# giesselmann/STRique

Hardware: AMD Instinct MI355X
Metric: reads/s for STRique 'count' on 50 kb r9.4 signals (higher is better)
Workload: dtype f32

## Files before the change

### strique_amd/csrc/lut_kernels.h

```cpp
#pragma once
#include <hip/hip_runtime.h>
#include <stdint.h>
#include "align_kernels.h"

#define STRQ_LUT_MAX_K 158
#define STRQ_LUT_LOCAL_HARD 64
#define STRQ_TABLE_SLOT_FLOATS(k) ((size_t)(k) * 256)

namespace strq {

struct LutJob {
    const float* level_val;
    const float* cls_val;
    float* table;
    uint8_t* table3;
    int32_t* band_lo;
    int32_t k, pad_;
};
struct LutInfo { int32_t total, n_hard, need, packed; };
struct HardEntry { int32_t job, k, level, index; };

int launch_lut_build(hipStream_t stream, const LutJob* jobs, LutInfo* info, int n_jobs, int max_k,
                     HardEntry* hard, int* hard_count, int hard_cap, const AlignParams& p);
int launch_lut_patch(hipStream_t stream, const LutJob* jobs, const HardEntry* hard, const float* vals, int n);

}
```

### strique_amd/csrc/lut_kernels.hip

```cpp
#include <hip/hip_runtime.h>
#include <stdint.h>
#include "lut_kernels.h"

namespace strq {

#define STRQ_HARD_ULPS 64

static __device__ __forceinline__ float cell_score_dev(const AlignParams& p, float h, float v, bool* hard)
{
    const float d = h > v ? h - v : v - h;
    const double y = pow((double)d, 1.2);
    const uint64_t bits = __builtin_bit_cast(uint64_t, y);
    const int64_t low = (int64_t)(bits & 0x1FFFFFFFull) - 0x10000000ll;
    bool hd = (low >= -STRQ_HARD_ULPS && low <= STRQ_HARD_ULPS);
    const float x = (float)y;
    const float s = p.dist_offset - x;
    if (hd) {
        const uint32_t xb = __builtin_bit_cast(uint32_t, x);
        const float x2 = __builtin_bit_cast(float, (double)x < y ? xb + 1u : (xb ? xb - 1u : 0u));
        const float s2 = p.dist_offset - x2;
        if (!(s > p.dist_min) && !(s2 > p.dist_min)) hd = false;
    }
    *hard = hd;
    return s > p.dist_min ? s : p.dist_min;
}

__global__ void __launch_bounds__(256)
lut_build_kernel(const LutJob* __restrict__ jobs, LutInfo* __restrict__ info, HardEntry* __restrict__ hard,
                 int* __restrict__ hard_count, int hard_cap, AlignParams p)
{
    __shared__ float v[256];
    __shared__ float cls[STRQ_LUT_MAX_K];
    __shared__ int lo[STRQ_LUT_MAX_K], hi[STRQ_LUT_MAX_K + 1];
    __shared__ int width, n_local, plat_lo, plat_hi, rebuild, unpackable;
    __shared__ unsigned char dup[STRQ_LUT_MAX_K];
    __shared__ unsigned short local_hard[STRQ_LUT_LOCAL_HARD][2];
    const LutJob jb = jobs[blockIdx.x];
    const int q = threadIdx.x, lane = q & 63, wave = q >> 6;
    v[q] = jb.level_val[q];
    for (int k = q; k < jb.k; k += 256) cls[k] = jb.cls_val[k];
    if (q == 0) { width = 0; n_local = 0; plat_lo = 255; plat_hi = 0; rebuild = 0; unpackable = 0; }
    __syncthreads();
    {
        const float v0 = v[0], v255 = v[255], vq = v[q];
        if (__builtin_bit_cast(uint32_t, vq) != __builtin_bit_cast(uint32_t, v0)) atomicMin(&plat_lo, q - 1);
        if (__builtin_bit_cast(uint32_t, vq) != __builtin_bit_cast(uint32_t, v255)) atomicMax(&plat_hi, q + 1);
        if (q > 0 && !(v[q - 1] <= vq)) rebuild = 1;
    }
    __syncthreads();
    if (rebuild) { if (q == 0) { info[blockIdx.x].total = 0; info[blockIdx.x].need = 0; info[blockIdx.x].packed = 0; info[blockIdx.x].n_hard = -1; } return; }
    const int plat_lo_r = plat_lo, plat_hi_r = plat_hi < plat_lo ? plat_lo : plat_hi;
    auto in_band = [&](int lv, float c) { bool hd; return cell_score_dev(p, v[lv], c, &hd) > p.dist_min; };
    for (int k = q; k < jb.k; k += 256) {
        const float c = cls[k];
        int a = 0, b = 256;
        while (a < b) { const int m = (a + b) >> 1; if (v[m] < c) a = m + 1; else b = m; }
        int best = a < 256 ? a : 255;
        if (a > 0 && a < 256) { const float dl = c - v[a - 1], dr = v[a] - c; if (dl <= dr) best = a - 1; }
        int l = 256, h = -1;
        bool hd_best;
        const bool best_in = cell_score_dev(p, v[best], c, &hd_best) > p.dist_min;
        if (hd_best) rebuild = 1;
        if (best_in) {
            int x = 0, y = best;
            while (x < y) { const int m = (x + y) >> 1; if (in_band(m, c)) y = m; else x = m + 1; }
            l = x;
            x = best; y = 255;
            while (x < y) { const int m = (x + y + 1) >> 1; if (in_band(m, c)) x = m; else y = m - 1; }
            h = x;
        }
        const bool none = h < l;
        const int el = none ? 0 : (l <= plat_lo_r ? plat_lo_r : l - 1);
        const int er = none ? 0 : (h >= plat_hi_r ? plat_hi_r : h + 1);
        lo[k] = el | (er << 8) | ((!none && l <= plat_lo_r) ? 0 : 1 << 16) | ((!none && h >= plat_hi_r) ? 0 : 1 << 17);
        hi[k] = er - el + 1;
        atomicMax(&width, er - el + 1);
    }
    __syncthreads();
    for (int k = q; k < jb.k; k += 256) {
        int first = k;
        const uint32_t bits = __builtin_bit_cast(uint32_t, cls[k]);
        for (int j = 0; j < k; ++j) if (__builtin_bit_cast(uint32_t, cls[j]) == bits) { first = j; break; }
        dup[k] = (unsigned char)first;
    }
    __syncthreads();
    if (q == 0) {
        int off = 0;
        for (int k = 0; k < jb.k; ++k) {
            if (dup[k] == k) { const int w = hi[k]; hi[k] = off; off += w; }
            else hi[k] = hi[dup[k]];
        }
        hi[jb.k] = off;
    }
    __syncthreads();
    const int* roff = hi;
    for (int k = wave; k < jb.k; k += 4) {
        const int d = lo[k], el = d & 255, er = (d >> 8) & 255;
        const float c = cls[k];
        if (dup[k] != k) {
            if (lane == 0) jb.band_lo[k] = (int32_t)((uint32_t)el | ((uint32_t)(er - el) << 8) | ((uint32_t)roff[k] << 16));
            continue;
        }
        for (int lv = el + lane; lv <= er; lv += 64) {
            bool hd;
            const float s = cell_score_dev(p, v[lv], c, &hd);
            jb.table[roff[k] + lv - el] = s;
            {
                const float r = s * 1048576.0f;
                const uint32_t u = r >= 0.0f && r < 16777216.0f ? (uint32_t)r : 0u;
                if (!((float)u == r) || !(r < 16777216.0f) || __builtin_bit_cast(uint32_t, r) == 0x80000000u) unpackable = 1;
                const int e = roff[k] + lv - el, total = roff[jb.k];
                reinterpret_cast<uint16_t*>(jb.table3)[e] = (uint16_t)(u >> 8);
                jb.table3[((2 * total + 3) & ~3) + e] = (uint8_t)u;
            }
            if (hd) {
                if ((lv == el && (d & (1 << 16))) || (lv == er && (d & (1 << 17)))) rebuild = 1;
                else {
                    const int slot = atomicAdd(&n_local, 1);
                    if (slot < STRQ_LUT_LOCAL_HARD) { local_hard[slot][0] = (unsigned short)k; local_hard[slot][1] = (unsigned short)lv; }
                }
            }
        }
        if (lane == 0) jb.band_lo[k] = (int32_t)((uint32_t)el | ((uint32_t)(er - el) << 8) | ((uint32_t)roff[k] << 16));
    }
    __syncthreads();
    if (q == 0) {
        int nh = n_local;
        if (nh > STRQ_LUT_LOCAL_HARD || rebuild) nh = -1;
        info[blockIdx.x].total = roff[jb.k];
        info[blockIdx.x].need = width;
        info[blockIdx.x].packed = (nh == 0 && !unpackable) ? 1 : 0;
        info[blockIdx.x].n_hard = nh;
        for (int i = 0; i < nh; ++i) {
            const int k = local_hard[i][0], lv = local_hard[i][1];
            const int slot = atomicAdd(hard_count, 1);
            if (slot < hard_cap) {
                HardEntry e;
                e.job = blockIdx.x; e.k = k; e.level = lv;
                e.index = roff[k] + (lv - (lo[k] & 255));
                hard[slot] = e;
            }
        }
    }
}

__global__ void lut_patch_kernel(const LutJob* __restrict__ jobs, const HardEntry* __restrict__ hard,
                                 const float* __restrict__ vals, int n)
{
    const int i = blockIdx.x * blockDim.x + threadIdx.x;
    if (i < n) jobs[hard[i].job].table[hard[i].index] = vals[i];
}

int launch_lut_build(hipStream_t stream, const LutJob* jobs, LutInfo* info, int n_jobs, int max_k,
                     HardEntry* hard, int* hard_count, int hard_cap, const AlignParams& p)
{
    if (max_k > STRQ_LUT_MAX_K) return 2;
    hipLaunchKernelGGL(lut_build_kernel, dim3(n_jobs), dim3(256), 0, stream, jobs, info, hard, hard_count, hard_cap, p);
    return hipGetLastError() == hipSuccess ? 0 : 1;
}

int launch_lut_patch(hipStream_t stream, const LutJob* jobs, const HardEntry* hard, const float* vals, int n)
{
    if (n <= 0) return 0;
    hipLaunchKernelGGL(lut_patch_kernel, dim3((n + 255) / 256), dim3(256), 0, stream, jobs, hard, vals, n);
    return hipGetLastError() == hipSuccess ? 0 : 1;
}

}
```

### strique_amd/csrc/screen_kernels.h

```cpp
#pragma once
#include <hip/hip_runtime.h>
#include <stdint.h>
#include "align_kernels.h"

#define STRQ_SCREEN_R 14
#define STRQ_SCREEN_S 6
#define STRQ_SCREEN_SEG 4
#define STRQ_SCREEN_CHUNK_COLS 128
#define STRQ_SCREEN_MAX_WINDOWS 4
#define STRQ_SCREEN2_CPL 5
#define STRQ_SCREEN2_LPF 29
#define STRQ_SCREEN2_LANE_B 32

namespace strq {

struct ScreenParams {
    int32_t sc;
    int32_t hh, v;
    int32_t cadd;
    int32_t slack;
    int32_t merge_gap;
    int32_t max_cand;
    int32_t margin;
};

struct ScreenTask {
    const uint8_t* levels;
    const float* table;
    const int32_t* band_lo;
    int32_t* out;
    int32_t tsize;
    int32_t n, m, k, col_off;
    int32_t n_chunks;
    int32_t lane_last;
};

struct Screen2Task {
    const uint8_t* levels;
    const float* table[2];
    const int32_t* band_lo[2];
    int32_t* out[2];
    int32_t tsize[2], k[2];
    int32_t n, col_off, n_chunks;
};

struct ScreenWindows {
    int32_t n_win;
    int32_t lo[STRQ_SCREEN_MAX_WINDOWS], hi[STRQ_SCREEN_MAX_WINDOWS];
    float lower_bound;
    float upper_bound;
    int32_t n_cand;
};

int screen_plan(const AlignParams& p, int samples, int max_n, ScreenParams* sp);
static inline bool screen_flank_ok(int m) { return m >= 2 * STRQ_SCREEN_R && m <= 64 * STRQ_SCREEN_R; }
size_t screen_lds_bytes(int tsize);
int launch_screen(hipStream_t stream, const ScreenTask* tasks, int n_groups, int* queue, const ScreenParams& sp,
                  size_t lds_bytes, int tables_per_cu, int n_cu);
int screen2_plan(const AlignParams& p, int samples, int max_n, int merge, ScreenParams* sp);
static inline bool screen2_flank_ok(int m, int k) { return k >= 1 && k <= STRQ_SCREEN2_LPF * STRQ_SCREEN2_CPL && m == k * STRQ_SCREEN_S; }
size_t screen2_lds_bytes(int tsize_a, int tsize_b);
int screen2_lanes_rows(int need_a, int need_b);
bool screen2_lanes_fit(int rows);
size_t screen2_lanes_lds_bytes(int rows);
int launch_screen2(hipStream_t stream, const Screen2Task* tasks, int n_groups, int* queue, const ScreenParams& sp,
                   size_t lds_bytes, int groups_per_cu, int n_cu, int merge, int lanes_rows);
int launch_screen_windows(hipStream_t stream, const ScreenTask* tasks, int n_groups, const ScreenParams& sp,
                          const int32_t* bound_scaled, ScreenWindows* out, const int32_t* list = nullptr, const int32_t* theta_list = nullptr);

}
```

### strique_amd/csrc/screen_kernels.hip

```cpp
#include "strq_opt.h"
#include <hip/hip_runtime.h>
#include <stdint.h>
#include <stdlib.h>
#include <cmath>
#include "screen_kernels.h"
#include "screen_lds_layout.h"

namespace strq {

namespace {

constexpr int R = STRQ_SCREEN_R, S = STRQ_SCREEN_S, SEG = STRQ_SCREEN_SEG;
constexpr int G = 2, C = 3;
static_assert(R == 14 && S == 6, "class expansion below is written for 14 rows per lane, 6 samples per class");

__device__ __forceinline__ int dpp_shr1(int v, int fill)
{
    return __builtin_amdgcn_update_dpp(fill, v, 0x138, 0xF, 0xF, false);
}
__device__ __forceinline__ int dpp_shr1_open(int v)
{
    return __builtin_amdgcn_mov_dpp(v, 0x138, 0xF, 0xF, true);
}
__device__ __forceinline__ int med3i(int a, int lo, int hi)
{
    int r;
    asm("v_med3_i32 %0, %1, %2, %3" : "=v"(r) : "v"(a), "v"(lo), "v"(hi));
    return r;
}
#define STRQ_SCREEN_BIAS 0x00800000
#ifndef STRQ_SCREEN_WPE
#define STRQ_SCREEN_WPE 6
#endif
__device__ __forceinline__ int max3i(int a, int b, int c)
{
    int r;
    asm("v_max3_f32 %0, %1, %2, %3" : "=v"(r) : "v"(a), "v"(b), "v"(c));
    return r;
}
__device__ __forceinline__ int add_uniform(int v, int u)
{
    int r;
    asm("v_add_u32 %0, %2, %1" : "=v"(r) : "v"(v), "s"(u));
    return r;
}
__device__ __forceinline__ int sel_mask(int if0, int if1, uint64_t mask)
{
    int r;
    asm("v_cndmask_b32_e64 %0, %1, %2, %3" : "=v"(r) : "v"(if0), "v"(if1), "s"(mask));
    return r;
}

struct LaneConst { int lo2[C], hi2[C], off[C]; };

struct Screen {
    const char* lds;
    const LaneConst& lc;
    const uint64_t (&pm)[3];
    const int lane, n, hh;
    int T[R], SbotA, upS, potB, cmax;
    int qq;
    int scA[C], scB[C];

    __device__ __forceinline__ void fetch(int q2, int (&sc)[C])
    {
#pragma unroll
        for (int c = 0; c < C; ++c)
            sc[c] = *reinterpret_cast<const uint16_t*>(lds + med3i(q2, lc.lo2[c], lc.hi2[c]) + lc.off[c]);
    }
    __device__ __forceinline__ void advance(int qsrc, int snext, int& qn, int (&nA)[C], int (&nB)[C])
    {
        qn = __builtin_amdgcn_update_dpp(__builtin_amdgcn_readlane(qsrc, snext), qq, 0x138, 0xF, 0xF, false);
        fetch(qn & 0xffff, nA);
        fetch((int)((unsigned)qn >> 16), nB);
    }
    __device__ __forceinline__ void prime(int qcur)
    {
        qq = 0;
        int qn, nA[C], nB[C];
        advance(qcur, 0, qn, nA, nB);
        qq = qn;
#pragma unroll
        for (int c = 0; c < C; ++c) { scA[c] = nA[c]; scB[c] = nB[c]; }
    }
    __device__ __forceinline__ void expand(const int (&sc)[C], int (&rs)[R])
    {
#pragma unroll
        for (int r = 0; r < R; r += G) {
            const int base = r / S, x = (r % S) / G;
            int v;
            if (x == 0 || base + 1 >= C) v = sc[base < C ? base : C - 1];
            else v = sel_mask(sc[base], sc[base + 1], pm[x]);
#pragma unroll
            for (int g = 0; g < G && r + g < R; ++g) rs[r + g] = v;
        }
    }

    template <bool PRED>
    __device__ __forceinline__ void step(int t, int qsrc, int snext)
    {
        const int qn = __builtin_amdgcn_update_dpp(__builtin_amdgcn_readlane(qsrc, snext), qq, 0x138, 0xF, 0xF, false);
        const int potA = potB + hh, potBn = potA + hh;
        const int upA = dpp_shr1(SbotA, potA);
        const int upB = dpp_shr1(T[R - 1], potBn);
        int rsA[R], rsB[R];
        expand(scA, rsA);
        expand(scB, rsB);
        fetch(qn & 0xffff, scA);
        fetch((int)((unsigned)qn >> 16), scB);
        bool act = true, okB = true;
        if constexpr (PRED) { const int jB = 2 * (t - lane), jA = jB - 1; act = (jA >= 1) && (jA <= n); okB = jB <= n; }
        if (act) {
            int ta_prev = upA, ta_prev2 = upS, tb_prev2 = upB;
#pragma unroll
            for (int r = 0; r < R; ++r) {
                const int diagA = r == 0 ? upS : T[r - 1];
                const int ta = max3i(diagA + rsA[r], T[r], ta_prev);
                if (r > 0) {
                    const int tb = max3i(ta_prev2 + rsB[r - 1], ta_prev, tb_prev2);
                    T[r - 1] = tb; tb_prev2 = tb;
                }
                ta_prev2 = ta_prev; ta_prev = ta;
            }
            const int tb = max3i(ta_prev2 + rsB[R - 1], ta_prev, tb_prev2);
            T[R - 1] = tb;
            SbotA = ta_prev;
            upS = upB;
            const int cA = ta_prev - potA + STRQ_SCREEN_BIAS, cB = okB ? tb - potBn + STRQ_SCREEN_BIAS : cA;
            cmax = max3i(cmax, cA, cB);
        }
        potB = potBn;
        qq = qn;
    }
};

__device__ __forceinline__ int load_chunk(const ScreenTask& tk, int chunk, int lane)
{
    const int idx = (chunk * 64 + lane) * 2;
    int a = 0, b = 0;
    if (idx < tk.n) a = tk.levels[idx];
    if (idx + 1 < tk.n) b = tk.levels[idx + 1];
    return (a * 2) | ((b * 2) << 16);
}

}

size_t screen_lds_bytes(int tsize)
{
    return (size_t)((tsize + 1) & ~1) * 2 + 4;
}

__global__ void __attribute__((amdgpu_flat_work_group_size(64 * STRQ_SCREEN_SEG, 64 * STRQ_SCREEN_SEG), amdgpu_waves_per_eu(STRQ_SCREEN_WPE, STRQ_SCREEN_WPE)))
align_screen_kernel(const ScreenTask* __restrict__ tasks, int n_groups, int* __restrict__ queue, ScreenParams sp)
{
    extern __shared__ uint32_t lds_all[];
    __shared__ int next_group;
    const int lane = threadIdx.x & 63, wave = threadIdx.x >> 6;
    const char* ldsb = reinterpret_cast<const char*>(lds_all);
    for (;;) {
        __syncthreads();
        if (threadIdx.x == 0) next_group = atomicAdd(queue, 1);
        __syncthreads();
        const int gi = __builtin_amdgcn_readfirstlane(next_group);
        if (gi >= n_groups) break;
        const ScreenTask& t0 = tasks[(size_t)gi * SEG];
        const int ts = t0.tsize, zero_idx = (ts + 1) & ~1;
        {
            uint16_t* dst = reinterpret_cast<uint16_t*>(lds_all);
            const float scf = (float)sp.sc;
            for (int i = threadIdx.x; i < ts; i += 64 * SEG) dst[i] = (uint16_t)((int)ceilf(t0.table[i] * scf) + sp.cadd);
            if (threadIdx.x == 0) { dst[zero_idx] = 0; dst[zero_idx + 1] = 0; }
        }
        __syncthreads();
        const ScreenTask& tk = tasks[(size_t)gi * SEG + wave];
        if (tk.n <= 0) continue;

        LaneConst lc; uint64_t pm[3];
        {
            const int row0 = lane * R, kbase = row0 / S, phase = row0 % S;
#pragma unroll
            for (int c = 0; c < C; ++c) {
                const int k = kbase + c;
                if (k < tk.k) {
                    const uint32_t d = (uint32_t)tk.band_lo[k];
                    const int lo = (int)(d & 255u), w1 = (int)((d >> 8) & 255u), off = (int)(d >> 16);
                    lc.lo2[c] = lo * 2; lc.hi2[c] = (lo + w1) * 2;
                    lc.off[c] = (off - lo) * 2;
                } else {
                    lc.lo2[c] = 0; lc.hi2[c] = 0; lc.off[c] = zero_idx * 2;
                }
            }
            pm[0] = 0;
#pragma unroll
            for (int x = 1; x < 3; ++x) {
                const uint64_t b = __ballot(phase >= S - x * G);
                const uint32_t lo = __builtin_amdgcn_readfirstlane((int)(uint32_t)b), hi = __builtin_amdgcn_readfirstlane((int)(uint32_t)(b >> 32));
                pm[x] = ((uint64_t)hi << 32) | lo;
            }
        }
        const int lM = (tk.m - 1) / R;
        Screen f{ldsb, lc, pm, lane, tk.n, sp.hh};
        {
#pragma unroll
            for (int r = 0; r < R; ++r) f.T[r] = STRQ_SCREEN_BIAS;
            f.SbotA = STRQ_SCREEN_BIAS; f.upS = STRQ_SCREEN_BIAS;
            f.potB = STRQ_SCREEN_BIAS - 2 * lane * sp.hh;
            f.cmax = STRQ_SCREEN_BIAS;
        }
        const int nsteps = (tk.n + 1) / 2 + 63;
        int qcur = load_chunk(tk, 0, lane);
        f.prime(qcur);
        for (int t0s = 0; t0s < nsteps; t0s += 64) {
            const int qnext = load_chunk(tk, t0s / 64 + 1, lane);
            const bool full = (t0s >= 63) && (2 * (t0s + 64) <= tk.n);
            const int send = nsteps - t0s < 64 ? nsteps - t0s : 64;
            if (full) {
                for (int s = 0; s < 63; ++s) f.template step<false>(t0s + s + 1, qcur, s + 1);
                f.template step<false>(t0s + 64, qnext, 0);
            } else {
                for (int s = 0; s < send; ++s) {
                    const int qsrc = s == 63 ? qnext : qcur, snext = (s + 1) & 63;
                    f.template step<true>(t0s + s + 1, qsrc, snext);
                }
            }
            const int cm = __builtin_amdgcn_readlane(f.cmax, lM) - STRQ_SCREEN_BIAS;
            if (lane == 0) tk.out[t0s / 64] = cm;
            f.cmax = STRQ_SCREEN_BIAS;
            qcur = qnext;
        }
    }
}

namespace {

constexpr int CPL = STRQ_SCREEN2_CPL, LPF = STRQ_SCREEN2_LPF, LB = STRQ_SCREEN2_LANE_B;

struct Lane2Const { int lo2[CPL], hi2[CPL], off[CPL]; };

template <int RPC, int CMG>
struct Screen2 {
    static constexpr int R2 = RPC * CPL;
    static_assert(CMG == 1 || CMG == 2 || CMG == 4, "groups must divide the 64 steps of a chunk");
    const char* lds;
    const Lane2Const& lc;
    const uint64_t top_mask;
    const int lane, n, hh;
    int T[R2], SbotA, upS, potB, cmax;
    int gpot, gmax;
    int qq;
    int scA[CPL], scB[CPL];

    __device__ __forceinline__ int score(int q2, int c) const
    {
        return *reinterpret_cast<const uint16_t*>(lds + med3i(q2, lc.lo2[c], lc.hi2[c]) + lc.off[c]);
    }
    __device__ __forceinline__ void prime(int qcur)
    {
        qq = __builtin_amdgcn_update_dpp(__builtin_amdgcn_readlane(qcur, 0), 0, 0x138, 0xF, 0xF, false);
#pragma unroll
        for (int c = 0; c < CPL; ++c) { scA[c] = score(qq & 0xffff, c); scB[c] = score((int)((unsigned)qq >> 16), c); }
    }

    template <bool PRED>
    __device__ __forceinline__ void step(int t, int qsrc, int snext, bool gfirst = true, bool glast = true)
    {
        const int qn = __builtin_amdgcn_update_dpp(__builtin_amdgcn_readlane(qsrc, snext), qq, 0x138, 0xF, 0xF, false);
        const int qa = qn & 0xffff, qb = (int)((unsigned)qn >> 16);
        const int potA = add_uniform(potB, hh), potBn = add_uniform(potA, hh);
        const int upA = sel_mask(dpp_shr1_open(SbotA), potA, top_mask);
        const int upB = sel_mask(dpp_shr1_open(T[R2 - 1]), potBn, top_mask);
        constexpr bool GROUPED = !PRED && CMG > 1;
        if (GROUPED && gfirst) gpot = potA;
        bool act = true, okB = true;
        if constexpr (PRED) { const int jB = 2 * (t - lane), jA = jB - 1; act = (jA >= 1) && (jA <= n); okB = jB <= n; }
        int ta_prev = upA, ta_prev2 = upS;
        int tb_prev2 = upB;
#pragma unroll
        for (int c = 0; c < CPL; ++c) {
            if (act) {
#pragma unroll
                for (int r = RPC * c; r < RPC * c + RPC; ++r) {
                    const int diagA = r == 0 ? upS : T[r - 1];
                    const int ta = max3i(diagA + scA[c], T[r], ta_prev);
                    if (r > 0) {
                        const int tb = max3i(ta_prev2 + scB[(r - 1) / RPC], ta_prev, tb_prev2);
                        T[r - 1] = tb; tb_prev2 = tb;
                    }
                    ta_prev2 = ta_prev; ta_prev = ta;
                }
                if (c == CPL - 1) {
                    const int tb = max3i(ta_prev2 + scB[c], ta_prev, tb_prev2);
                    T[R2 - 1] = tb;
                    SbotA = ta_prev;
                    upS = upB;
                    if constexpr (GROUPED) {
                        if (glast) { const int d = tb - gpot; gmax = d > gmax ? d : gmax; }
                    } else {
                        const int cA = ta_prev - potA + STRQ_SCREEN_BIAS, cB = okB ? tb - potBn + STRQ_SCREEN_BIAS : cA;
                        cmax = max3i(cmax, cA, cB);
                    }
                }
            }
            scA[c] = score(qa, c);
            if (c > 0) scB[c - 1] = score(qb, c - 1);
            if (c == CPL - 1) scB[c] = score(qb, c);
        }
        potB = potBn;
        qq = qn;
    }
};

template <int SHIFT>
__device__ __forceinline__ int load_chunk2(const Screen2Task& tk, int chunk, int lane)
{
    const int idx = (chunk * 64 + lane) * 2;
    int a = 0, b = 0;
    if (idx < tk.n) a = tk.levels[idx];
    if (idx + 1 < tk.n) b = tk.levels[idx + 1];
    return (a << SHIFT) | (b << (SHIFT + 16));
}

template <int RPC, int CMG, bool LANES>
__device__ __forceinline__ void screen2_body(const Screen2Task* __restrict__ tasks, int n_groups, int* __restrict__ queue, const ScreenParams& sp, int lds_rows)
{
    constexpr int R2 = RPC * CPL, MERGE = S / RPC;
    constexpr int QSHIFT = LANES ? screen_lanes::ROW_SHIFT : 1;
    static_assert(CPL == screen_lanes::CPL, "screen_lds_layout.h stacks the lane's five classes");
    extern __shared__ uint32_t lds_all[];
    __shared__ int next_group;
    const int lane = threadIdx.x & 63, wave = threadIdx.x >> 6;
    const char* ldsb = reinterpret_cast<const char*>(lds_all);
    const int f = lane >= LB ? 1 : 0, lf = lane - f * LB;
    for (;;) {
        __syncthreads();
        if (threadIdx.x == 0) next_group = atomicAdd(queue, 1);
        __syncthreads();
        const int gi = __builtin_amdgcn_readfirstlane(next_group);
        if (gi >= n_groups) break;
        const Screen2Task& t0 = tasks[(size_t)gi * SEG];
        const float scf = (float)sp.sc;
        Lane2Const lc;
        if constexpr (LANES) {
            uint32_t desc[CPL];
            int nc = 0, rowbase[CPL];
#pragma unroll
            for (int c = 0; c < CPL; ++c) {
                const int k = lf * CPL + c;
                const bool in = lf < LPF && k < t0.k[f];
                desc[c] = in ? (uint32_t)t0.band_lo[f][k] : 0u;
                nc += in ? 1 : 0;
            }
            screen_lanes::row_bases(desc, nc, rowbase);
            char* dst = reinterpret_cast<char*>(lds_all);
            if (wave == 0) *reinterpret_cast<uint16_t*>(dst + screen_lanes::slot(lane)) = 0;
#pragma unroll
            for (int c = 0; c < CPL; ++c) {
                const screen_lanes::ClassAddr a = c < nc ? screen_lanes::class_addr(lane, rowbase[c], desc[c]) : screen_lanes::padding_addr(lane);
                lc.lo2[c] = a.lo2; lc.hi2[c] = a.hi2; lc.off[c] = a.off;
                if (c < nc) {
                    const float* src = t0.table[f] + screen_lanes::desc_off(desc[c]);
                    const int w1 = screen_lanes::desc_w1(desc[c]);
                    for (int i = (wave - rowbase[c]) & (SEG - 1); i <= w1; i += SEG)
                        if (rowbase[c] + i < lds_rows)
                            *reinterpret_cast<uint16_t*>(dst + screen_lanes::entry_address(lane, rowbase[c], i)) = (uint16_t)(MERGE * ((int)ceilf(src[i] * scf) + sp.cadd));
                }
            }
        }
        [[maybe_unused]] int base[2], zero_idx[2];
        base[0] = 0; zero_idx[0] = (t0.tsize[0] + 1) & ~1;
        base[1] = zero_idx[0] + 2; zero_idx[1] = base[1] + ((t0.tsize[1] + 1) & ~1);
        if constexpr (!LANES) {
            uint16_t* dst = reinterpret_cast<uint16_t*>(lds_all);
#pragma unroll
            for (int ff = 0; ff < 2; ++ff) {
                for (int i = threadIdx.x; i < t0.tsize[ff]; i += 64 * SEG) dst[base[ff] + i] = (uint16_t)(MERGE * ((int)ceilf(t0.table[ff][i] * scf) + sp.cadd));
                if (threadIdx.x == 0) { dst[zero_idx[ff]] = 0; dst[zero_idx[ff] + 1] = 0; }
            }
        }
        __syncthreads();
        const Screen2Task& tk = tasks[(size_t)gi * SEG + wave];
        if (tk.n <= 0) continue;

        if constexpr (!LANES) {
#pragma unroll
            for (int c = 0; c < CPL; ++c) {
                const int k = lf * CPL + c;
                if (lf < LPF && k < tk.k[f]) {
                    const uint32_t d = (uint32_t)tk.band_lo[f][k];
                    const int lo = (int)(d & 255u), w1 = (int)((d >> 8) & 255u), off = (int)(d >> 16);
                    lc.lo2[c] = lo * 2; lc.hi2[c] = (lo + w1) * 2;
                    lc.off[c] = (base[f] + off - lo) * 2;
                } else {
                    lc.lo2[c] = 0; lc.hi2[c] = 0; lc.off[c] = zero_idx[f] * 2;
                }
            }
        }
        const uint64_t top_mask = 1ull | (1ull << LB);
        const int lMa = (tk.k[0] - 1) / CPL, lMb = LB + (tk.k[1] - 1) / CPL;
        Screen2<RPC, CMG> s2{ldsb, lc, top_mask, lane, tk.n, sp.hh};
        {
#pragma unroll
            for (int r = 0; r < R2; ++r) s2.T[r] = STRQ_SCREEN_BIAS;
            s2.SbotA = STRQ_SCREEN_BIAS; s2.upS = STRQ_SCREEN_BIAS;
            s2.potB = STRQ_SCREEN_BIAS - 2 * lane * sp.hh;
            s2.cmax = STRQ_SCREEN_BIAS; s2.gpot = 0; s2.gmax = 0;
        }
        const int nsteps = (tk.n + 1) / 2 + 63;
        int qcur = load_chunk2<QSHIFT>(tk, 0, lane);
        s2.prime(qcur);
        for (int t0s = 0; t0s < nsteps; t0s += 64) {
            const int qnext = load_chunk2<QSHIFT>(tk, t0s / 64 + 1, lane);
            const bool full = (t0s >= 63) && (2 * (t0s + 64) <= tk.n);
            const int send = nsteps - t0s < 64 ? nsteps - t0s : 64;
            if (full) {
                constexpr int U = CMG > 2 ? CMG : 2;
                s2.gmax = 0;
#pragma unroll 1
                for (int s = 0; s < 64 - U; s += U) {
#pragma unroll
                    for (int u = 0; u < U; ++u) s2.template step<false>(0, qcur, s + u + 1, u % CMG == 0, u % CMG == CMG - 1);
                }
#pragma unroll
                for (int u = 0; u < U - 1; ++u) s2.template step<false>(0, qcur, 64 - U + u + 1, u % CMG == 0, u % CMG == CMG - 1);
                s2.template step<false>(0, qnext, 0, CMG == 1, true);
                if constexpr (CMG > 1) s2.cmax = s2.gmax + STRQ_SCREEN_BIAS;
            } else {
                for (int s = 0; s < send; ++s) {
                    const int qsrc = s == 63 ? qnext : qcur, snext = (s + 1) & 63;
                    s2.template step<true>(t0s + s + 1, qsrc, snext);
                }
            }
            const int cma = __builtin_amdgcn_readlane(s2.cmax, lMa) - STRQ_SCREEN_BIAS;
            const int cmb = __builtin_amdgcn_readlane(s2.cmax, lMb) - STRQ_SCREEN_BIAS;
            if (lane == 0) { tk.out[0][t0s / 64] = cma; tk.out[1][t0s / 64] = cmb; }
            s2.cmax = STRQ_SCREEN_BIAS;
            qcur = qnext;
        }
    }
}

}

size_t screen2_lds_bytes(int tsize_a, int tsize_b)
{
    return (size_t)(((tsize_a + 1) & ~1) + 2 + ((tsize_b + 1) & ~1) + 2) * 2;
}

int screen2_lanes_rows(int need_a, int need_b) { return screen_lanes::rows_bound(need_a, need_b); }
bool screen2_lanes_fit(int rows) { return screen_lanes::fits(rows); }
size_t screen2_lanes_lds_bytes(int rows) { return screen_lanes::bytes(rows); }

#ifndef STRQ_SCREEN3_CMG
#define STRQ_SCREEN3_CMG 2
#endif
#define STRQ_SCREEN2_ATTR(WPE_) __attribute__((amdgpu_flat_work_group_size(64 * STRQ_SCREEN_SEG, 64 * STRQ_SCREEN_SEG), amdgpu_waves_per_eu(WPE_, WPE_)))
#define STRQ_SCREEN2_ARGS const Screen2Task* __restrict__ tasks, int n_groups, int* __restrict__ queue, ScreenParams sp, int lds_rows
__global__ void STRQ_SCREEN2_ATTR(6) align_screen3_kernel(STRQ_SCREEN2_ARGS) { screen2_body<2, STRQ_SCREEN3_CMG, true>(tasks, n_groups, queue, sp, lds_rows); }
__global__ void STRQ_SCREEN2_ATTR(4) align_screen1_kernel(STRQ_SCREEN2_ARGS) { screen2_body<6, 1, true>(tasks, n_groups, queue, sp, lds_rows); }
__global__ void STRQ_SCREEN2_ATTR(6) align_screen3_rows_kernel(STRQ_SCREEN2_ARGS) { screen2_body<2, STRQ_SCREEN3_CMG, false>(tasks, n_groups, queue, sp, lds_rows); }
__global__ void STRQ_SCREEN2_ATTR(4) align_screen1_rows_kernel(STRQ_SCREEN2_ARGS) { screen2_body<6, 1, false>(tasks, n_groups, queue, sp, lds_rows); }
#undef STRQ_SCREEN2_ARGS

__global__ void __launch_bounds__(256)
screen_windows_kernel(const ScreenTask* __restrict__ tasks, int n_groups, ScreenParams sp,
                      const int32_t* __restrict__ bound_scaled, ScreenWindows* __restrict__ out,
                      const int32_t* __restrict__ list, const int32_t* __restrict__ theta_list)
{
    const int lane = threadIdx.x & 63;
    const int idx = blockIdx.x * (blockDim.x >> 6) + (threadIdx.x >> 6);
    if (idx >= n_groups) return;
    const int g = list ? list[idx] : idx;
    const ScreenTask* tg = tasks + (size_t)g * SEG;
    const int m = tg[0].m, lM = tg[0].lane_last;
    const int shift = -m * sp.v;
    int vmax = 0;
    for (int w = 0; w < SEG; ++w) {
        if (tg[w].n <= 0) continue;
        for (int c = lane; c < tg[w].n_chunks; c += 64) { const int v = tg[w].out[c]; vmax = v > vmax ? v : vmax; }
    }
#pragma unroll
    for (int d = 32; d >= 1; d >>= 1) { const int o = __shfl_xor(vmax, d, 64); vmax = o > vmax ? o : vmax; }
    ScreenWindows r;
    r.n_win = 0; r.n_cand = 0;
    for (int k = 0; k < STRQ_SCREEN_MAX_WINDOWS; ++k) { r.lo[k] = 0; r.hi[k] = 0; }
    const int drop = (sp.margin > 0 ? sp.margin : m) + 2 * sp.slack;
    int theta = theta_list ? theta_list[idx] : vmax - drop;
    if (!theta_list && sp.max_cand > 0) {
        auto count_at = [&](int t) {
            int n = 0;
            for (int w = 0; w < SEG; ++w) {
                if (tg[w].n <= 0) continue;
                for (int c = lane; c < tg[w].n_chunks; c += 64) n += tg[w].out[c] >= t;
            }
#pragma unroll
            for (int d = 32; d >= 1; d >>= 1) n += __shfl_xor(n, d, 64);
            return n;
        };
        if (count_at(theta) > sp.max_cand) {
            int lo = theta, hi = vmax;
            while (hi - lo > 1) {
                const int mid = lo + (hi - lo) / 2;
                if (count_at(mid) > sp.max_cand) lo = mid; else hi = mid;
            }
            theta = hi;
        }
    }
    r.upper_bound = (float)(vmax + shift + sp.slack) / (float)sp.sc;
    auto scan = [&](int th, bool store) -> int {
        int nw = 0, last_hi = -(1 << 30), ncand = 0;
        for (int w = 0; w < SEG; ++w) {
            if (tg[w].n <= 0) continue;
            for (int c0 = 0; c0 < tg[w].n_chunks; c0 += 64) {
                const int c1 = c0 + lane;
                const bool cand = c1 < tg[w].n_chunks && tg[w].out[c1] >= th;
                uint64_t mask = __ballot(cand);
                while (mask) {
                    const int bit = __builtin_ctzll(mask); mask &= mask - 1;
                    const int c = c0 + bit;
                    ++ncand;
                    int lo = 128 * c - 2 * lM + 1, hi = 128 * c - 2 * lM + 128;
                    if (lo < 1) lo = 1;
                    if (hi > tg[w].n) hi = tg[w].n;
                    if (hi < lo) continue;
                    lo += tg[w].col_off; hi += tg[w].col_off;
                    if (nw > 0 && lo <= last_hi + sp.merge_gap) {
                        if (hi > last_hi) last_hi = hi;
                        if (store) {
                            const int k = nw <= STRQ_SCREEN_MAX_WINDOWS ? nw - 1 : STRQ_SCREEN_MAX_WINDOWS - 1;
                            if (hi > r.hi[k]) r.hi[k] = hi;
                            if (lo < r.lo[k]) r.lo[k] = lo;
                        }
                    } else {
                        ++nw; last_hi = hi;
                        if (store) {
                            if (nw <= STRQ_SCREEN_MAX_WINDOWS) { r.lo[nw - 1] = lo; r.hi[nw - 1] = hi; }
                            else if (hi > r.hi[STRQ_SCREEN_MAX_WINDOWS - 1]) r.hi[STRQ_SCREEN_MAX_WINDOWS - 1] = hi;
                        }
                    }
                }
            }
        }
        if (store) r.n_cand = ncand;
        return nw;
    };
    if (!theta_list && sp.max_cand > 0 && scan(theta, false) > STRQ_SCREEN_MAX_WINDOWS) {
        int lo = theta, hi = vmax;
        while (hi - lo > 1) {
            const int mid = lo + (hi - lo) / 2;
            if (scan(mid, false) > STRQ_SCREEN_MAX_WINDOWS) lo = mid; else hi = mid;
        }
        theta = hi;
    }
    {
        const double lb = (double)(theta + shift + sp.slack) / (double)sp.sc;
        float lbf = (float)lb;
        if ((double)lbf < lb) {
            int32_t bits = __float_as_int(lbf);
            bits = lbf > 0.0f ? bits + 1 : (lbf < 0.0f ? bits - 1 : 1);
            lbf = __int_as_float(bits);
        }
        r.lower_bound = lbf;
    }
    const bool ok = theta + shift > 0 && theta + shift > bound_scaled[g];
    if (ok) {
        int nw = scan(theta, true);
        if (nw > STRQ_SCREEN_MAX_WINDOWS) nw = STRQ_SCREEN_MAX_WINDOWS;
        for (int a = 1; a < nw; ++a)
            for (int b = a; b > 0 && r.lo[b] < r.lo[b - 1]; --b) {
                const int tl = r.lo[b], th = r.hi[b]; r.lo[b] = r.lo[b - 1]; r.hi[b] = r.hi[b - 1]; r.lo[b - 1] = tl; r.hi[b - 1] = th;
            }
        int kept = nw > 0 ? 1 : 0;
        for (int a = 1; a < nw; ++a) {
            if (r.lo[a] <= r.hi[kept - 1] + 1) { if (r.hi[a] > r.hi[kept - 1]) r.hi[kept - 1] = r.hi[a]; }
            else { r.lo[kept] = r.lo[a]; r.hi[kept] = r.hi[a]; ++kept; }
        }
        for (int a = kept; a < STRQ_SCREEN_MAX_WINDOWS; ++a) { r.lo[a] = 0; r.hi[a] = 0; }
        r.n_win = kept;
    }
    if (lane == 0) out[idx] = r;
}

int screen_plan(const AlignParams& p, int samples, int max_n, ScreenParams* sp)
{
    if (strq::opt("STRQ_NO_SCREEN")) return 0;
    if (samples != S) return 0;
    if (!(p.open_h == p.ext_h && p.open_v == p.ext_v)) return 0;
    if (!(p.dist_min >= 0.0f) || !(p.ext_h < 0.0f) || !(p.ext_v < 0.0f) || !(p.dist_offset > 0.0f) || !(p.dist_min <= p.dist_offset)) return 0;
    for (int sc = 1024; sc >= 16; sc >>= 1) {
        const double hh = -(double)p.ext_h * sc, v = -(double)p.ext_v * sc, smax = std::ceil((double)p.dist_offset * sc);
        if (hh != (double)(long)hh || v != (double)(long)v) continue;
        if (hh < 1 || smax + v + hh > 65000.0) continue;
        const double top = 64.0 * R * (smax + v) + ((double)max_n + 256.0) * hh + smax + v + hh + (double)STRQ_SCREEN_BIAS;
        if (top > 2.0e9) continue;
        sp->sc = sc; sp->hh = (int)hh; sp->v = (int)v; sp->cadd = (int)(hh + v);
        {
            const double rows = 64.0 * R, maxval = rows * (double)p.dist_offset;
            double p2 = 1.0; while (p2 < maxval) p2 *= 2.0;
            const double adds = rows * (1.0 + (double)p.dist_offset / -(double)p.ext_h);
            const double e = adds * p2 / 16777216.0;
            if (!(e < 1.0e4)) continue;
            sp->slack = ((int)std::ceil(e) + 1) * sc;
        }
        sp->merge_gap = 3072; sp->margin = 0; sp->max_cand = 0;
        return 1;
    }
    return 0;
}

int screen2_plan(const AlignParams& p, int samples, int max_n, int merge, ScreenParams* sp)
{
    if (merge != 1 && merge != 3) return 0;
    if (!screen_plan(p, samples, max_n, sp)) return 0;
    while (sp->sc >= 16) {
        const double smax = std::ceil((double)p.dist_offset * sp->sc);
        if ((double)merge * (smax + sp->cadd) <= 65000.0) return 1;
        if ((sp->hh & 1) || (sp->v & 1)) return 0;
        sp->slack = (sp->slack / sp->sc) * (sp->sc / 2);
        sp->sc /= 2; sp->hh /= 2; sp->v /= 2; sp->cadd = sp->hh + sp->v;
    }
    return 0;
}

int launch_screen2(hipStream_t stream, const Screen2Task* tasks, int n_groups, int* queue, const ScreenParams& sp,
                   size_t lds_bytes, int groups_per_cu, int n_cu, int merge, int lanes_rows)
{
    if (n_groups <= 0) return 0;
    if (merge != 3 && merge != 1) return 2;
    const bool lanes = lanes_rows > 0;
    if (lanes && (!screen_lanes::fits(lanes_rows) || lds_bytes < screen_lanes::bytes(lanes_rows))) return 2;
    auto kern = merge == 3 ? (lanes ? align_screen3_kernel : align_screen3_rows_kernel) : (lanes ? align_screen1_kernel : align_screen1_rows_kernel);
    if (merge == 1 && groups_per_cu > 4) groups_per_cu = 4;
    if (groups_per_cu > 6) groups_per_cu = 6;
    (void)hipFuncSetAttribute((const void*)kern, hipFuncAttributeMaxDynamicSharedMemorySize, (int)lds_bytes);
    hipLaunchKernelGGL(kern, dim3(groups_per_cu * n_cu), dim3(64 * SEG), lds_bytes, stream, tasks, n_groups, queue, sp, lanes_rows);
    return hipGetLastError() == hipSuccess ? 0 : 1;
}

int launch_screen(hipStream_t stream, const ScreenTask* tasks, int n_groups, int* queue, const ScreenParams& sp,
                  size_t lds_bytes, int tables_per_cu, int n_cu)
{
    if (n_groups <= 0) return 0;
    (void)hipFuncSetAttribute((const void*)align_screen_kernel, hipFuncAttributeMaxDynamicSharedMemorySize, (int)lds_bytes);
    hipLaunchKernelGGL(align_screen_kernel, dim3(tables_per_cu * n_cu), dim3(64 * SEG), lds_bytes, stream, tasks, n_groups, queue, sp);
    return hipGetLastError() == hipSuccess ? 0 : 1;
}

int launch_screen_windows(hipStream_t stream, const ScreenTask* tasks, int n_groups, const ScreenParams& sp,
                          const int32_t* bound_scaled, ScreenWindows* out, const int32_t* list, const int32_t* theta_list)
{
    if (n_groups <= 0) return 0;
    hipLaunchKernelGGL(screen_windows_kernel, dim3((n_groups + 3) / 4), dim3(256), 0, stream, tasks, n_groups, sp, bound_scaled, out, list, theta_list);
    return hipGetLastError() == hipSuccess ? 0 : 1;
}

}
```

### strique_amd/csrc/strq_align_api.hip

```cpp
#include <hip/hip_runtime.h>
#include <algorithm>
#include <cmath>
#include <climits>
#include <cstring>
#include <cstdlib>
#include <time.h>
#include <unistd.h>
#include <map>
#include <mutex>
#include <string>
#include <tuple>
#include <numeric>
#include <vector>
#include "../../include/strique_hip.h"
#include "strq_ctx.h"
#include "align_kernels.h"
#include "lut_kernels.h"
#include "align_generic.h"

using namespace strq;

#define STRQ_DBG(...) do { if (strq::opt("STRQ_DEBUG")) { fprintf(stderr, "[strq] " __VA_ARGS__); fprintf(stderr, "\n"); fflush(stderr); } } while (0)

namespace strq {

static thread_local const strq_ctx* t_cur_ctx = nullptr;
static std::mutex g_opt_mu;
static std::map<std::string, std::string> g_opts;
CtxScope::CtxScope(const strq_ctx* c) : prev(t_cur_ctx) { t_cur_ctx = c; }
CtxScope::~CtxScope() { t_cur_ctx = prev; }
const char* opt(const char* key)
{
    static thread_local std::string ring[8];
    static thread_local unsigned ring_pos = 0;
    auto keep = [&](const std::string& v) -> const char* {
        if (v.empty()) return nullptr;
        std::string& slot = ring[ring_pos++ & 7u];
        slot = v;
        return slot.c_str();
    };
    if (t_cur_ctx) {
        std::lock_guard<std::mutex> lk(t_cur_ctx->options_mu);
        auto it = t_cur_ctx->options.find(key);
        if (it != t_cur_ctx->options.end()) return keep(it->second);
    }
    {
        std::lock_guard<std::mutex> lk(g_opt_mu);
        auto it = g_opts.find(key);
        if (it != g_opts.end()) return keep(it->second);
    }
    return getenv(key);
}

float host_cell_score(const AlignParams& p, float h, float v)
{
    const float d = h > v ? h - v : v - h;
    const float s = p.dist_offset - (float)std::pow((double)d, 1.2);
    return s > p.dist_min ? s : p.dist_min;
}

void host_col0(const AlignParams& p, int m, float* out)
{
    const float NINF = -3.4028234663852886e38f / 2;
    out[0] = 0.0f;
    float vprev = NINF, sprev = 0.0f;
    for (int i = 1; i <= m; ++i) {
        const float ext = vprev + p.ext_v, opn = sprev + p.open_v;
        const float v = ext >= opn ? ext : opn;
        out[i] = v; vprev = v; sprev = v;
    }
}

struct BatchIn {
    int64_t n_align, n_reads;
    const uint8_t* levels; const int64_t* read_off; const float* level_val;
    const int32_t* align_read; const float* flank; const int64_t* flank_off; int32_t samples;
};
struct BatchOut { float* score; int64_t* j_end; int64_t* j0; int32_t* rec; };


static const int hard_cap = 1 << 16;
static const int trace_wpb = 8;

struct Piece { int col_off, n; size_t ck; };

static int cut(int n, int segs, int ov, Piece* out)
{
    int use = segs;
    while (use > 1 && (ov <= 0 || (long)n < (long)(use + 1) * ov)) --use;
    const long len = use > 1 ? ((long)n + (long)(use - 1) * ov + use - 1) / use : n;
    long o = 0;
    for (int k = 0; k < segs; ++k) {
        if (k >= use) { out[k].col_off = 0; out[k].n = 0; continue; }
        const long start = k == 0 ? 0 : o - ov;
        long end = k == use - 1 ? n : start + len; if (end > n) end = n;
        out[k].col_off = (int)start; out[k].n = (int)(end - start);
        o = end;
    }
    return use;
}

static int packed_dwords(int entries) { return (((2 * entries + 3) & ~3) + entries + 3) / 4; }

struct Launch { int R, NS, tables, first, count, first_task, first_up, lds_floats, packed, segs; bool known_last_row; };

struct CorePlan {
    CorePlan(strq_ctx* c_, const AlignCoreIn& in_, AlignCoreOut& out_) : c(c_), in(in_), out(out_), nb(in_.nb), S(in_.samples), st(c_->stream) {}
    strq_ctx* c;
    const AlignCoreIn& in;
    AlignCoreOut& out;
    const int nb, S;
    const hipStream_t st;

    bool collapsed = false, allow_pack = false, ov_fixed = false, scr_forced = false, mode_fine = false, mode_coarse = false;
    int seg_want = 0, max_tables = 8, max_waves = 16, ov_cap = 8192;
    std::map<std::pair<int, int>, int> ov_of_m;

    std::vector<size_t> cls_off, col0_off, bnd_off;
    std::vector<int> J0, NJ;
    std::vector<int> job_align, job_k0, job_k;
    std::vector<size_t> tab_off, desc_off;
    int nj = 0, max_k = 0;
    std::vector<float> h_cls;
    std::vector<LutJob> jobs;
    std::vector<LutInfo> info;
    std::vector<int> tab_total;

    std::vector<ScreenWindows> wins;
    bool screen2_ran = false;
    std::vector<int> g2_of;
    ScreenTask* d_st2 = nullptr;
    int32_t* d_bound2 = nullptr;
    ScreenParams sp2{};
    double coarse_cols = 0, coarse_all = 0;

    std::vector<char> packed;
    std::vector<int> overlap, segs_of;
    std::vector<Launch> launches;
    int n_up = 0, max_ns = 1, r2_cap = 0, qi = STRQ_QUEUE_FIRST;
    size_t n_tasks = 0, safe0 = 0, r2_0 = 0;
    std::vector<Piece> pieces, safe;
    std::vector<float> min_score;
    std::vector<char> two_round;
    bool any_two_round = false;
    std::vector<size_t> ck_up;
    std::vector<AlignTask> tasks;
    AlignTask *d_tasks = nullptr, *d_heads = nullptr;
    AlignResult *d_seg = nullptr, *d_res = nullptr, *d_seg_safe = nullptr;
    int32_t* d_pick = nullptr;
    float* d_min_score = nullptr;
    int *d_redo = nullptr, *d_redo_count = nullptr;
};

static int overlap_for(CorePlan& p, int m, int ov_worst, int redo_weight = 1)
{
    strq_ctx* c = p.c;
    if (p.ov_fixed || c->score_fracs.size() < 64 || c->mean_n <= 0) return std::min(ov_worst, p.ov_cap);
    auto it = p.ov_of_m.find(std::make_pair(m, redo_weight));
    if (it != p.ov_of_m.end()) return it->second;
    const std::vector<float>& f = c->score_fracs;
    double best_cost = 0; int best_ov = std::min(ov_worst, p.ov_cap);
    for (int ov = 1024; ; ov += 512) {
        if (ov > ov_worst) ov = ov_worst;
        const float need = align_segment_min_score(c->ap, m, ov) / ((float)m * c->ap.dist_offset) + 0.01f;
        const double redo = (double)(std::lower_bound(f.begin(), f.end(), need) - f.begin()) / (double)f.size();
        const double cost = 3.0 * ov / c->mean_n + redo_weight * redo * (1.0 + 3.0 * ov_worst / c->mean_n);
        if (best_cost == 0 || cost < best_cost) { best_cost = cost; best_ov = ov; }
        if (ov >= ov_worst) break;
    }
    p.ov_of_m[std::make_pair(m, redo_weight)] = best_ov;
    STRQ_DBG("overlap for %d-row flanks: %d columns (worst case %d; previous sub-batch: median score fraction %.3f, mean read %.0f samples)", m, best_ov, ov_worst, f[f.size() / 2], c->mean_n);
    return best_ov;
}

static int tables_for(const CorePlan& p, int dwords, int segs)
{
    int t = std::min(p.max_tables, (160 * 1024 - 64) / (std::max(dwords, 1) * 4));
    if (segs > 1) t = std::min(t, p.max_waves / segs);
    return t;
}

static void pause_after_fail(int& pause, int& fail)
{
    pause = std::min(256, 8 << std::min(fail, 5));
    ++fail;
}

static int upload_inputs(CorePlan& p)
{
    strq_ctx* c = p.c; const AlignCoreIn& in = p.in; AlignCoreOut& out = p.out;
    const int nb = p.nb, S = p.S;
    hipStream_t st = p.st;
    size_t cls_tot = 0, col0_tot = 0, rec_tot = 0, tab_tot = 0, bnd_floats = 0, desc_tot = 0;
    p.cls_off.assign(nb, 0); p.col0_off.assign(nb, 0); p.bnd_off.assign(nb, 0);
    std::map<const float*, size_t> cls_of_flank; std::map<int, size_t> col0_of_m;
    std::vector<int> cls_first, col0_first;
    out.rec_off.assign(nb, 0);
    p.J0.assign(nb, 0); p.NJ.assign(nb, 0);
    for (int i = 0; i < nb; ++i) {
        auto fc = cls_of_flank.find(in.flank[i]);
        if (fc == cls_of_flank.end()) { fc = cls_of_flank.emplace(in.flank[i], cls_tot).first; cls_tot += in.k[i]; cls_first.push_back(i); }
        p.cls_off[i] = fc->second;
        auto f0 = col0_of_m.find(in.m[i]);
        if (f0 == col0_of_m.end()) { f0 = col0_of_m.emplace(in.m[i], col0_tot).first; col0_tot += in.m[i] + 1; col0_first.push_back(i); }
        p.col0_off[i] = f0->second;
        p.J0[i] = (int)p.job_align.size();
        p.NJ[i] = in.k[i] > STRQ_LUT_MAX_K ? in.NS[i] : 1;
        for (int sidx = 0; sidx < p.NJ[i]; ++sidx) {
            int k0 = 0, kn = in.k[i];
            if (p.NJ[i] > 1) {
                const int row0 = sidx * 64 * in.R[i], rows = std::min(64 * in.R[i], in.m[i] - row0);
                k0 = row0 / S; kn = (row0 + rows - 1) / S - k0 + 1;
            }
            p.job_align.push_back(i); p.job_k0.push_back(k0); p.job_k.push_back(kn);
            p.desc_off.push_back(desc_tot); desc_tot += kn;
            p.tab_off.push_back(tab_tot); tab_tot += STRQ_TABLE_SLOT_FLOATS(kn);
            p.max_k = std::max(p.max_k, kn);
        }
        out.rec_off[i] = rec_tot; rec_tot += in.m[i];
        p.bnd_off[i] = bnd_floats; if (in.NS[i] > 1) bnd_floats += (size_t)(in.NS[i] - 1) * 2 * ((size_t)in.n[i] + 2);
    }
    const int nj = p.nj = (int)p.job_align.size();
    out.rec_total = rec_tot;
    p.h_cls.assign(cls_tot, 0.0f);
    std::vector<float> h_col0(col0_tot);
    for (int i : cls_first) {
        const float* f = in.flank[i];
        for (int kk = 0; kk < in.k[i]; ++kk) p.h_cls[p.cls_off[i] + kk] = f[(size_t)kk * S];
    }
    for (int i : col0_first) host_col0(c->ap, in.m[i], &h_col0[p.col0_off[i]]);
    STRQ_HIP(c, c->flank_cls.reserve(cls_tot * 4));
    STRQ_HIP(c, c->col0.reserve(col0_tot * 4));
    STRQ_HIP(c, c->band_lo.reserve(desc_tot * 4));
    STRQ_HIP(c, c->tables.reserve(tab_tot * 4));
    STRQ_HIP(c, c->tables3.reserve(tab_tot * 3 + (size_t)nj * 8 + 64));
    STRQ_HIP(c, c->bnd.reserve(bnd_floats * 4 + 256));
    STRQ_HIP(c, c->rec.reserve(rec_tot * 4 + 256));
    STRQ_HIP(c, c->lutinfo.reserve((size_t)nj * (sizeof(LutJob) + sizeof(LutInfo))));
    STRQ_HIP(c, c->hard.reserve((size_t)hard_cap * (sizeof(HardEntry) + 4) + 64));
    STRQ_HIP(c, c->queue.reserve(STRQ_QUEUE_BYTES));
    STRQ_HIP(c, hipMemcpyAsync(c->flank_cls.p, p.h_cls.data(), cls_tot * 4, hipMemcpyHostToDevice, st));
    STRQ_HIP(c, hipMemcpyAsync(c->col0.p, h_col0.data(), col0_tot * 4, hipMemcpyHostToDevice, st));
    STRQ_HIP(c, hipMemsetAsync(c->queue.p, 0, STRQ_QUEUE_BYTES, st));
    return STRQ_OK;
}

struct TableBuild {
    int nj = 0, max_k = 0;
    std::vector<LutJob>* jobs = nullptr;
    const float* d_level_val = nullptr;
    std::vector<int> job_read;
    std::vector<const float*> job_cls;
    std::function<int()> after_tables;
    std::vector<LutInfo>* info = nullptr;
    std::vector<LutInfo>* reported = nullptr;
    std::vector<HardEntry>* handed = nullptr;
    int hard_count = 0;
};

static int run_table_build(strq_ctx* c, hipStream_t st, TableBuild& b)
{
    const int nj = b.nj;
    std::vector<LutJob>& jobs = *b.jobs;
    std::vector<LutInfo>& info = *b.info;
    LutJob* d_jobs = c->lutinfo.as<LutJob>();
    LutInfo* d_info = reinterpret_cast<LutInfo*>(d_jobs + nj);
    STRQ_HIP(c, hipMemcpyAsync(d_jobs, jobs.data(), (size_t)nj * sizeof(LutJob), hipMemcpyHostToDevice, st));
    HardEntry* d_hard = c->hard.as<HardEntry>();
    float* d_hard_vals = reinterpret_cast<float*>(d_hard + hard_cap);
    int* d_hard_count = c->queue.as<int>();
    STRQ_HIP(c, hipEventRecord(c->ev[0], st));
    if (launch_lut_build(st, d_jobs, d_info, nj, b.max_k, d_hard, d_hard_count, hard_cap, c->ap)) { c->err = "lut launch failed"; return STRQ_ERR_DEVICE; }
    STRQ_HIP(c, hipEventRecord(c->ev[1], st));
    if (b.after_tables) { const int arc = b.after_tables(); if (arc) return arc; }
    info.resize(nj);
    int hard_count = 0;
    STRQ_HIP(c, hipMemcpyAsync(info.data(), d_info, (size_t)nj * sizeof(LutInfo), hipMemcpyDeviceToHost, st));
    STRQ_HIP(c, hipMemcpyAsync(&hard_count, d_hard_count, 4, hipMemcpyDeviceToHost, st));
    STRQ_HIP(c, hipStreamSynchronize(st));
    if (b.reported) *b.reported = info;
    STRQ_DBG("lut done jobs=%d hard=%d floats0=%d", nj, hard_count, info[0].total);
    if (strq::opt("STRQ_DEBUG")) { int hist[9] = {0}; for (int i = 0; i < nj; ++i) hist[std::min(8, info[i].need / 8)]++; STRQ_DBG("band need histogram (x8 levels): %d %d %d %d %d %d %d %d %d", hist[0], hist[1], hist[2], hist[3], hist[4], hist[5], hist[6], hist[7], hist[8]); }
    if (strq::opt("STRQ_DEBUG")) { long tot = 0; int mx = 0; for (int i = 0; i < nj; ++i) { tot += info[i].total; mx = std::max(mx, info[i].total); } STRQ_DBG("table floats: mean %.0f max %d (k=%d)", (double)tot / nj, mx, jobs[0].k); }
    if (hard_count > hard_cap) { c->err = "too many borderline table entries"; return STRQ_ERR_DEVICE; }
    bool any_rebuild = false;
    for (int j = 0; j < nj; ++j) any_rebuild |= info[j].n_hard < 0;
    auto level_vals_of = [&](int read, float* dst) -> int {
        STRQ_HIP(c, hipMemcpy(dst, b.d_level_val + (size_t)read * 256, 256 * 4, hipMemcpyDeviceToHost));
        return STRQ_OK;
    };
    if (hard_count > 0) {
        std::vector<HardEntry> he(hard_count); std::vector<float> hv(hard_count);
        STRQ_HIP(c, hipMemcpy(he.data(), d_hard, (size_t)hard_count * sizeof(HardEntry), hipMemcpyDeviceToHost));
        float lv[256]; int last_read = -1;
        for (int i = 0; i < hard_count; ++i) {
            const int rd = b.job_read[he[i].job];
            if (rd != last_read) { const int rc = level_vals_of(rd, lv); if (rc) return rc; last_read = rd; }
            hv[i] = host_cell_score(c->ap, lv[he[i].level], b.job_cls[he[i].job][he[i].k]);
        }
        STRQ_HIP(c, hipMemcpyAsync(d_hard_vals, hv.data(), (size_t)hard_count * 4, hipMemcpyHostToDevice, st));
        if (launch_lut_patch(st, d_jobs, d_hard, d_hard_vals, hard_count)) { c->err = "patch launch failed"; return STRQ_ERR_DEVICE; }
        STRQ_HIP(c, hipStreamSynchronize(st));
        if (b.handed) *b.handed = he;
    } else if (b.handed) b.handed->clear();
    if (any_rebuild) for (int j = 0; j < nj; ++j) if (info[j].n_hard < 0) {
        const int kk = jobs[j].k;
        std::vector<float> tab((size_t)kk * 256); std::vector<int32_t> blo(kk);
        float lv[256];
        { const int rc = level_vals_of(b.job_read[j], lv); if (rc) return rc; }
        for (int x = 0; x < kk; ++x) {
            float* row = &tab[(size_t)x * 256];
            for (int q = 0; q < 256; ++q) row[q] = host_cell_score(c->ap, lv[q], b.job_cls[j][x]);
            blo[x] = (int32_t)((255u << 8) | ((uint32_t)(x * 256) << 16));
        }
        STRQ_HIP(c, hipMemcpy(jobs[j].table, tab.data(), tab.size() * 4, hipMemcpyHostToDevice));
        STRQ_HIP(c, hipMemcpy(jobs[j].band_lo, blo.data(), (size_t)kk * 4, hipMemcpyHostToDevice));
        info[j].total = kk * 256; info[j].need = 256;
    }
    b.hard_count = hard_count;
    return STRQ_OK;
}

static uint8_t* table3_slot(strq_ctx* c, size_t tab_off, int j)
{
    const size_t o = tab_off * 3 + (size_t)j * 8;
    return c->tables3.as<uint8_t>() + o - o % 4;
}

static int build_tables(CorePlan& p)
{
    strq_ctx* c = p.c; const AlignCoreIn& in = p.in;
    const int nb = p.nb, nj = p.nj;
    std::vector<LutJob>& jobs = p.jobs;
    jobs.resize(nj);
    TableBuild b;
    b.nj = nj; b.max_k = p.max_k; b.jobs = &jobs; b.d_level_val = in.d_level_val; b.after_tables = in.after_tables; b.info = &p.info;
    b.job_read.resize(nj); b.job_cls.resize(nj);
    for (int j = 0; j < nj; ++j) {
        const int i = p.job_align[j];
        jobs[j].level_val = in.d_level_val + (size_t)in.read[i] * 256;
        jobs[j].cls_val = c->flank_cls.as<float>() + p.cls_off[i] + p.job_k0[j];
        jobs[j].table = c->tables.as<float>() + p.tab_off[j];
        jobs[j].table3 = table3_slot(c, p.tab_off[j], j);
        jobs[j].band_lo = c->band_lo.as<int32_t>() + p.desc_off[j];
        jobs[j].k = p.job_k[j]; jobs[j].pad_ = 0;
        b.job_read[j] = in.read[i];
        b.job_cls[j] = &p.h_cls[p.cls_off[i] + p.job_k0[j]];
    }
    const int rc = run_table_build(c, p.st, b);
    if (rc) return rc;
    p.tab_total.assign(nb, 0);
    for (int j = 0; j < nj; ++j) p.tab_total[p.job_align[j]] = std::max(p.tab_total[p.job_align[j]], p.info[j].total);
    p.out.n_hard = b.hard_count;
    return STRQ_OK;
}

static void read_switches(CorePlan& p)
{
    const strq_ctx* c = p.c;
    p.collapsed = p.S == 6 && c->ap.open_h == c->ap.ext_h && c->ap.open_v == c->ap.ext_v;
    if (const char* e = strq::opt("STRQ_SEG")) { const int v = atoi(e); if (v >= 1 && v <= 4) p.seg_want = v; }
    if (const char* e = strq::opt("STRQ_TABLES")) { const int v = atoi(e); if (v >= 1 && v <= 8) p.max_tables = v; }
    if (const char* e = strq::opt("STRQ_MAX_WAVES")) { const int v = atoi(e); if (v >= 4 && v <= 16) p.max_waves = v; }
    p.allow_pack = p.collapsed && !strq::opt("STRQ_NO_PACK");
    if (const char* e = strq::opt("STRQ_OVERLAP")) { const int v = atoi(e); p.ov_cap = v > 0 ? v : (1 << 30); p.ov_fixed = true; }
    p.scr_forced = strq::opt("STRQ_SCREEN_ALWAYS") != nullptr;
    const char* mode_opt = strq::opt("STRQ_SCREEN_MODE");
    p.mode_fine = mode_opt && std::strcmp(mode_opt, "fine") == 0;
    p.mode_coarse = mode_opt && std::strcmp(mode_opt, "coarse") == 0;
}


struct ScreenJob {
    int flanks = 1;
    std::vector<int> al;
    std::vector<ScreenTask> views;
    std::vector<Screen2Task> t2;
    std::vector<int32_t> bound;
    std::vector<size_t> out_off;
    size_t out_words = 0, lds_bytes = 0;
    int lanes_rows = 0;
    double steps = 0;
};

struct ScreenRules {
    int merge;
    int groups_per_cu;
    const char* lds_err;
    bool below_bound_free;
    bool count_untaken;
    bool judge;
    double max_cols;
    int* pause; int* fail;
};

static void screen_tasks(CorePlan& p, const ScreenParams& sp, ScreenJob& j)
{
    constexpr int SSEG = STRQ_SCREEN_SEG;
    const AlignCoreIn& in = p.in;
    const int F = j.flanks, ng = (int)j.al.size() / F;
    if (F == 2) j.t2.resize((size_t)ng * SSEG);
    j.views.resize(j.al.size() * SSEG);
    j.bound.resize(j.al.size());
    j.out_off.assign(j.al.size() * SSEG, 0);
    for (int g = 0; g < ng; ++g) {
        const int* a = &j.al[(size_t)g * F];
        const int n = in.n[a[0]];
        const int m_big = F == 2 ? std::max(in.m[a[0]], in.m[a[1]]) : in.m[a[0]];
        const int ov_worst = align_segment_overlap(p.c->ap, m_big), ov_s = overlap_for(p, m_big, ov_worst, 16);
        Piece pc[SSEG];
        const int used = cut(n, SSEG, ov_s, pc);
        j.lds_bytes = std::max(j.lds_bytes, F == 2 ? screen2_lds_bytes(p.info[p.J0[a[0]]].total, p.info[p.J0[a[1]]].total) : screen_lds_bytes(p.info[p.J0[a[0]]].total));
        if (F == 2) j.lanes_rows = std::max(j.lanes_rows, screen2_lanes_rows(p.info[p.J0[a[0]]].need, p.info[p.J0[a[1]]].need));
        for (int f = 0; f < F; ++f)
            j.bound[(size_t)g * F + f] = used <= 1 ? INT32_MIN / 2 : (ov_s >= ov_worst ? 0 : (int32_t)std::ceil((double)align_segment_min_score(p.c->ap, in.m[a[f]], ov_s) * sp.sc));
        for (int w = 0; w < SSEG; ++w) {
            Screen2Task t; std::memset(&t, 0, sizeof(t));
            t.levels = in.d_levels + in.read_off[in.read[a[0]]] + pc[w].col_off;
            t.n = pc[w].n; t.col_off = pc[w].col_off;
            t.n_chunks = pc[w].n > 0 ? (align_num_steps(pc[w].n) + 63) / 64 : 0;
            for (int f = 0; f < F; ++f) {
                const LutJob& job = p.jobs[p.J0[a[f]]];
                t.table[f] = job.table; t.band_lo[f] = job.band_lo; t.tsize[f] = p.info[p.J0[a[f]]].total; t.k[f] = in.k[a[f]];
                ScreenTask v; std::memset(&v, 0, sizeof(v));
                v.n = pc[w].n; v.m = in.m[a[f]]; v.k = in.k[a[f]]; v.col_off = pc[w].col_off; v.n_chunks = t.n_chunks;
                if (F == 2) v.lane_last = f * STRQ_SCREEN2_LANE_B + (in.k[a[f]] - 1) / STRQ_SCREEN2_CPL;
                else { v.levels = t.levels; v.table = t.table[0]; v.band_lo = t.band_lo[0]; v.tsize = t.tsize[0]; v.lane_last = (v.m - 1) / STRQ_SCREEN_R; }
                j.out_off[((size_t)g * F + f) * SSEG + w] = j.out_words; j.out_words += (size_t)t.n_chunks;
                j.views[((size_t)g * F + f) * SSEG + w] = v;
            }
            if (pc[w].n > 0) j.steps += align_num_steps(pc[w].n);
            if (F == 2) j.t2[(size_t)g * SSEG + w] = t;
        }
    }
}

static int run_screen(CorePlan& p, ScreenJob& j, const ScreenParams& sp, const ScreenRules& r)
{
    constexpr int SSEG = STRQ_SCREEN_SEG;
    strq_ctx* c = p.c; const AlignCoreIn& in = p.in;
    hipStream_t st = p.st;
    const int nv = (int)j.al.size();
    int lanes_rows = 0;
    if (j.flanks == 2) {
        const char* e = strq::opt("STRQ_SCREEN_LDS");
        if (!(e && std::strcmp(e, "rows") == 0) && screen2_lanes_fit(j.lanes_rows)) { lanes_rows = j.lanes_rows; j.lds_bytes = screen2_lanes_lds_bytes(lanes_rows); }
    }
    if (j.lds_bytes > 160 * 1024 - 64) { c->err = r.lds_err; return STRQ_ERR_UNSUPPORTED; }
    const int groups = std::max(1, std::min(r.groups_per_cu, (int)((160 * 1024 - 64) / j.lds_bytes)));
    auto aligned = [](size_t bytes) { return (bytes + 255) & ~(size_t)255; };
    const size_t t2_bytes = aligned(j.t2.size() * sizeof(Screen2Task)), task_bytes = aligned(j.views.size() * sizeof(ScreenTask));
    const size_t bound_bytes = aligned((size_t)nv * 4), win_bytes = aligned((size_t)nv * sizeof(ScreenWindows));
    STRQ_HIP(c, c->screen.reserve(t2_bytes + task_bytes + bound_bytes + win_bytes + j.out_words * 4 + 256));
    char* base = c->screen.as<char>();
    Screen2Task* d_t2 = reinterpret_cast<Screen2Task*>(base);
    ScreenTask* d_st = reinterpret_cast<ScreenTask*>(base + t2_bytes);
    int32_t* d_bound = reinterpret_cast<int32_t*>(base + t2_bytes + task_bytes);
    ScreenWindows* d_win = reinterpret_cast<ScreenWindows*>(base + t2_bytes + task_bytes + bound_bytes);
    int32_t* d_out = reinterpret_cast<int32_t*>(base + t2_bytes + task_bytes + bound_bytes + win_bytes);
    for (size_t x = 0; x < j.views.size(); ++x) j.views[x].out = d_out + j.out_off[x];
    if (j.flanks == 2)
        for (int v = 0; v < nv; ++v) for (int w = 0; w < SSEG; ++w) j.t2[(size_t)(v / 2) * SSEG + w].out[v % 2] = j.views[(size_t)v * SSEG + w].out;
    if (j.flanks == 2) STRQ_HIP(c, hipMemcpyAsync(d_t2, j.t2.data(), j.t2.size() * sizeof(Screen2Task), hipMemcpyHostToDevice, st));
    STRQ_HIP(c, hipMemcpyAsync(d_st, j.views.data(), j.views.size() * sizeof(ScreenTask), hipMemcpyHostToDevice, st));
    STRQ_HIP(c, hipMemcpyAsync(d_bound, j.bound.data(), (size_t)nv * 4, hipMemcpyHostToDevice, st));
    STRQ_HIP(c, hipEventRecord(c->ev[5], st));
    int* queue = c->queue.as<int>() + STRQ_QUEUE_FIRST - 1;
    if (j.flanks == 2) {
        if (launch_screen2(st, d_t2, nv / 2, queue, sp, j.lds_bytes, groups, c->n_cu, r.merge, lanes_rows)) { c->err = "coarse screen launch failed"; return STRQ_ERR_DEVICE; }
    } else {
        if (launch_screen(st, d_st, nv, queue, sp, j.lds_bytes, groups, c->n_cu)) { c->err = "screen launch failed"; return STRQ_ERR_DEVICE; }
    }
    STRQ_HIP(c, hipEventRecord(c->ev[6], st));
    if (launch_screen_windows(st, d_st, nv, sp, d_bound, d_win)) { c->err = "screen windows launch failed"; return STRQ_ERR_DEVICE; }
    std::vector<ScreenWindows> hw((size_t)nv);
    STRQ_HIP(c, hipMemcpyAsync(hw.data(), d_win, hw.size() * sizeof(ScreenWindows), hipMemcpyDeviceToHost, st));
    STRQ_HIP(c, hipStreamSynchronize(st));
    c->screen_ran = true; c->screen_mode_last = r.merge > 1 ? 2 : 1; c->coarse_merge_last = r.merge;
    c->screen_lds_last = j.flanks == 2 ? (lanes_rows > 0 ? 1 : 2) : 0;
    if (const char* path = strq::opt("STRQ_SCREEN_DUMP")) {
        std::vector<int32_t> ho(j.out_words);
        STRQ_HIP(c, hipMemcpy(ho.data(), d_out, j.out_words * 4, hipMemcpyDeviceToHost));
        if (FILE* fp = fopen(path, "wb")) {
            const int32_t hdr[8] = {nv, sp.sc, sp.hh, sp.v, j.flanks, SSEG, sp.slack, r.merge};
            fwrite(hdr, 4, 8, fp);
            for (int v = 0; v < nv; ++v) {
                const int32_t gh[4] = {j.al[v], j.al[v], j.bound[v], j.views[(size_t)v * SSEG].lane_last};
                fwrite(gh, 4, 4, fp);
                for (int w = 0; w < SSEG; ++w) {
                    const ScreenTask& t = j.views[(size_t)v * SSEG + w];
                    const int32_t th[4] = {t.col_off, t.n, t.m, t.n_chunks};
                    fwrite(th, 4, 4, fp);
                    fwrite(ho.data() + (t.out - d_out), 4, (size_t)t.n_chunks, fp);
                }
                fwrite(&hw[(size_t)v], sizeof(ScreenWindows), 1, fp);
            }
            fclose(fp);
        }
    }
    if (const char* e = strq::opt("STRQ_SCREEN_TEST_RAISE")) {
        const float up = (float)atof(e);
        for (auto& w : hw) w.lower_bound += up;
    }
    int windowed = 0, heavy = 0, below_bound = 0; double cols = 0, all = 0;
    for (int v = 0; v < nv; ++v) {
        const int al = j.al[v];
        const ScreenWindows& w = hw[(size_t)v];
        c->screen_stats[1] += 1; c->screen_stats[7] += w.n_cand;
        double mine = in.n[al];
        if (w.n_win > 0) {
            p.wins[al] = w; c->screen_stats[2] += 1; ++windowed; mine = 0;
            for (int k = 0; k < w.n_win; ++k) { c->screen_stats[4] += w.hi[k] - w.lo[k] + 1; mine += w.hi[k] - w.lo[k] + 1 + 4096; }
        } else {
            c->screen_stats[3] += 1;
            if (w.n_cand == 0) { ++below_bound; if (r.below_bound_free) mine = 0; }
        }
        all += in.n[al]; cols += mine; heavy += mine > 4 * 32768.0;
    }
    if (r.count_untaken) c->screen_stats[3] += p.nb - nv;
    c->screen_stats[5] += j.steps; c->screen_stats[6] = sp.sc;
    if (j.flanks == 2) {
        p.screen2_ran = true;
        p.d_st2 = d_st; p.d_bound2 = d_bound; p.sp2 = sp;
        for (int v = 0; v < nv; ++v) p.g2_of[j.al[v]] = v;
        p.coarse_cols = cols; p.coarse_all = all;
    }
    if (r.judge && nv >= 64) {
        if (below_bound * 10 > nv && !p.ov_fixed) c->score_fracs.clear();
        else if (windowed < 0.9 * (nv - (p.ov_fixed ? 0 : below_bound)) || cols > r.max_cols * all || (long)heavy * 100 > 2L * nv) pause_after_fail(*r.pause, *r.fail);
        else *r.fail = 0;
    }
    STRQ_DBG("screen (%d flanks per wave, merge %d): %d alignments, scale %d, margin %.0f, %d groups per CU, LDS %zu bytes: %d with windows (%d below the cold-start bound), %.2f %% of the columns, %d heavy -> pause %d",
             j.flanks, r.merge, nv, sp.sc, (double)sp.margin / sp.sc, groups, j.lds_bytes, windowed, below_bound, 100.0 * cols / std::max(1.0, all), heavy, *r.pause);
    return STRQ_OK;
}

static int screen_two_flank(CorePlan& p, int merge, int max_n)
{
    strq_ctx* c = p.c; const AlignCoreIn& in = p.in;
    const int nb = p.nb;
    ScreenParams sp;
    if (!screen2_plan(c->ap, p.S, max_n, merge, &sp)) return STRQ_OK;
    const bool fine_rules = merge == 1;
    int min_n = fine_rules ? 65536 : 28672, groups = 6;
    if (const char* e = strq::opt("STRQ_SCREEN_MIN_N")) min_n = atoi(e);
    if (const char* e = strq::opt("STRQ_SCREEN2_GROUPS")) { const int v = atoi(e); if (v >= 1 && v <= 8) groups = v; }
    std::map<int, std::vector<int>> by_read;
    for (int i = 0; i < nb; ++i)
        if (in.NS[i] == 1 && p.NJ[i] == 1 && in.n[i] >= min_n && screen2_flank_ok(in.m[i], in.k[i])) by_read[in.read[i]].push_back(i);
    std::vector<std::pair<int, int>> pairs;
    for (auto& kv : by_read) {
        const std::vector<int>& v = kv.second;
        if (v.size() == 2) { pairs.emplace_back(v[0], v[1]); continue; }
        for (size_t x = 0; x + 1 < v.size(); ++x)
            if (!(v[x] & 1) && v[x + 1] == v[x] + 1) { pairs.emplace_back(v[x], v[x + 1]); ++x; }
    }
    std::stable_sort(pairs.begin(), pairs.end(), [&](const std::pair<int, int>& x, const std::pair<int, int>& y) { return in.n[x.first] > in.n[y.first]; });
    const int ngr = (int)pairs.size();
    if (ngr == 0 || 2 * ngr < (nb * 9) / 10) return STRQ_OK;
    sp.margin = (int32_t)std::lround((double)c->coarse_margin * (merge == 3 ? 1.3 : 1.0) * sp.sc);
    if (const char* e = strq::opt("STRQ_SCREEN2_MARGIN")) sp.margin = (int32_t)std::lround(atof(e) * sp.sc);
    sp.max_cand = 8;
    if (const char* e = strq::opt("STRQ_SCREEN2_MAX_CAND")) sp.max_cand = atoi(e);
    if (fine_rules) { sp.margin = 0; sp.max_cand = 0; }
    ScreenJob j;
    j.flanks = 2;
    for (const auto& pr : pairs) { j.al.push_back(pr.first); j.al.push_back(pr.second); }
    screen_tasks(p, sp, j);
    ScreenRules r;
    r.merge = merge; r.groups_per_cu = groups;
    r.lds_err = "score tables do not fit LDS (coarse screen)";
    r.below_bound_free = !p.ov_fixed; r.count_untaken = true;
    if (fine_rules) { r.judge = !p.scr_forced; r.max_cols = 0.15; r.pause = &c->screen_pause; r.fail = &c->screen_fail; }
    else { r.judge = !p.mode_coarse && !p.scr_forced; r.max_cols = 0.30; r.pause = &c->coarse_pause; r.fail = &c->coarse_fail; }
    return run_screen(p, j, sp, r);
}

static int screen_one_flank(CorePlan& p, const ScreenParams& sp)
{
    strq_ctx* c = p.c; const AlignCoreIn& in = p.in;
    int min_n = 65536;
    if (const char* e = strq::opt("STRQ_SCREEN_MIN_N")) min_n = atoi(e);
    std::vector<int> sel;
    for (int i = 0; i < p.nb; ++i)
        if (in.NS[i] == 1 && p.NJ[i] == 1 && in.n[i] >= min_n && screen_flank_ok(in.m[i]) && in.k[i] * p.S == in.m[i]) sel.push_back(i);
    std::stable_sort(sel.begin(), sel.end(), [&](int x, int y) { return in.n[x] > in.n[y]; });
    if (sel.empty()) return STRQ_OK;
    ScreenJob j;
    j.al = sel;
    screen_tasks(p, sp, j);
    ScreenRules r;
    r.merge = 0; r.groups_per_cu = 6;
    r.lds_err = "score table does not fit LDS (screen)";
    r.below_bound_free = false; r.count_untaken = false;
    r.judge = true; r.max_cols = 0.10; r.pause = &c->screen_pause; r.fail = &c->screen_fail;
    return run_screen(p, j, sp, r);
}

static int run_screens(CorePlan& p)
{
    strq_ctx* c = p.c; const AlignCoreIn& in = p.in;
    const int nb = p.nb;
    p.wins.resize(nb);
    c->screen_ran = false;
    STRQ_HIP(c, hipEventRecord(c->ev[2], p.st));
    int max_n = 0;
    for (int i = 0; i < nb; ++i) max_n = std::max(max_n, in.n[i]);
    c->screen_mode_last = 0;
    const int coarse_merge = 3;
    p.g2_of.assign(nb, -1);
    for (int attempt = 0; attempt < 2 && !p.screen2_ran; ++attempt) {
        int merge = coarse_merge;
        if (attempt == 0) {
            if (!p.collapsed || p.mode_fine || strq::opt("STRQ_NO_SCREEN")) continue;
            if (c->coarse_pause > 0 && !p.mode_coarse && !p.scr_forced) { --c->coarse_pause; continue; }
        } else {
            if (!p.collapsed || strq::opt("STRQ_NO_SCREEN") || (c->screen_pause > 0 && !p.scr_forced)) continue;
            merge = 1;
        }
        const int rc = screen_two_flank(p, merge, max_n);
        if (rc) return rc;
    }
    if (p.screen2_ran) return STRQ_OK;
    if (p.collapsed && c->screen_pause > 0 && !p.scr_forced) {
        --c->screen_pause; c->screen_stats[3] += nb;
        return STRQ_OK;
    }
    ScreenParams sp;
    if (p.collapsed && screen_plan(c->ap, p.S, max_n, &sp)) return screen_one_flank(p, sp);
    return STRQ_OK;
}

static int plan_launches(CorePlan& p)
{
    strq_ctx* c = p.c; const AlignCoreIn& in = p.in; AlignCoreOut& out = p.out;
    const int nb = p.nb;
    std::vector<ScreenWindows>& wins = p.wins;
    static const double rate[5][2] = {{0, 0}, {1.017, 0.941}, {0.79, 0.862}, {0.85, 0.85}, {0.69, 0.80}};
    p.packed.assign(nb, 0); p.overlap.assign(nb, 0); p.segs_of.assign(nb, 1);
    std::vector<char> segmentable(nb, 0);
    const bool force_pack = strq::opt("STRQ_PACK") != nullptr;
    int class_count[5] = {0, 0, 0, 0, 0};
    for (int i = 0; i < nb; ++i) {
        segmentable[i] = p.collapsed && in.NS[i] == 1;
        p.overlap[i] = segmentable[i] ? align_segment_overlap(c->ap, in.m[i]) : 0;
        const bool can_pack = p.allow_pack && in.NS[i] == 1 && p.info[p.J0[i]].packed && p.info[p.J0[i]].n_hard == 0;
        int best_s = 1, best_p = can_pack ? 1 : 0;
        if (segmentable[i]) {
            const double l = overlap_for(p, in.m[i], p.overlap[i]);
            double best_cost = 0;
            for (int sgs : {1, 2, 3, 4}) {
                if (p.seg_want ? sgs != p.seg_want : sgs == 3) continue;
                if (sgs > 1 && !p.seg_want && (l <= 0 || in.n[i] < (sgs + 1) * l)) continue;
                for (int pk = 0; pk < 2; ++pk) {
                    if ((pk && !can_pack) || (force_pack && can_pack && !pk)) continue;
                    const double cost = (in.n[i] + (sgs - 1) * l) * rate[sgs][pk];
                    if (best_cost == 0 || cost < best_cost) { best_cost = cost; best_s = sgs; best_p = pk; }
                }
            }
        }
        if (wins[i].n_win > 0) {
            ScreenWindows& w = wins[i];
            while (w.n_win < STRQ_SCREEN_MAX_WINDOWS) {
                int widest = 0;
                for (int k2 = 1; k2 < w.n_win; ++k2) if (w.hi[k2] - w.lo[k2] > w.hi[widest] - w.lo[widest]) widest = k2;
                if (w.hi[widest] - w.lo[widest] < 16384) break;
                const int mid = w.lo[widest] + (w.hi[widest] - w.lo[widest]) / 2;
                for (int k2 = w.n_win; k2 > widest + 1; --k2) { w.lo[k2] = w.lo[k2 - 1]; w.hi[k2] = w.hi[k2 - 1]; }
                w.lo[widest + 1] = mid + 1; w.hi[widest + 1] = w.hi[widest]; w.hi[widest] = mid;
                ++w.n_win;
            }
            const int nw = w.n_win;
            best_s = p.seg_want >= nw ? p.seg_want : (nw <= 2 ? nw : 4); best_p = 0;
        }
        p.segs_of[i] = best_s; p.packed[i] = (char)best_p;
        ++class_count[best_s];
    }
    std::vector<int>& segs_of = p.segs_of;
    if (!p.seg_want && !c->screen_ran) {
        int few = 2 * c->n_cu;
        if (const char* e = strq::opt("STRQ_CLASS_MIN")) few = atoi(e);
        if (class_count[4] && class_count[4] < few) { for (int i = 0; i < nb; ++i) if (segs_of[i] == 4) { segs_of[i] = 2; if (wins[i].n_win > 2) wins[i].n_win = 0; } class_count[2] += class_count[4]; class_count[4] = 0; }
        if (class_count[2] && class_count[2] < few && class_count[1]) { for (int i = 0; i < nb; ++i) if (segs_of[i] == 2) { segs_of[i] = 1; if (wins[i].n_win > 1) wins[i].n_win = 0; } class_count[1] += class_count[2]; class_count[2] = 0; }
    }
    std::map<std::tuple<int, int, int, int, int>, std::vector<int>> groups;
    for (int i = 0; i < nb; ++i) {
        const int w = tables_for(p, p.packed[i] ? packed_dwords(p.tab_total[i]) : p.tab_total[i], segs_of[i]);
        if (w < 1) { c->err = "score table does not fit LDS"; return STRQ_ERR_UNSUPPORTED; }
        groups[std::make_tuple(in.R[i], in.NS[i], -segs_of[i], -w, p.packed[i] ? 0 : 1)].push_back(i);
    }
    const int min_rounds = 4;
    for (auto it = groups.begin(); it != groups.end();) {
        auto nx = std::next(it);
        const int w = -std::get<3>(it->first);
        const bool same_kind = nx != groups.end() && std::get<0>(nx->first) == std::get<0>(it->first) && std::get<1>(nx->first) == std::get<1>(it->first)
                               && std::get<2>(nx->first) == std::get<2>(it->first)
                               && !(std::get<4>(it->first) == 1 && std::get<4>(nx->first) == 0);
        if (same_kind && (long)it->second.size() < (long)min_rounds * w * c->n_cu) {
            nx->second.insert(nx->second.end(), it->second.begin(), it->second.end());
            it = groups.erase(it);
        } else ++it;
    }
    out.order.clear(); out.order.reserve(nb);
    for (auto& g : groups) {
        auto& v = g.second;
        auto work = [&](int x) {
            if (wins[x].n_win <= 0) return (long)in.n[x];
            long w = 0;
            for (int k = 0; k < wins[x].n_win; ++k) w += wins[x].hi[k] - wins[x].lo[k] + 1 + 4096;
            return w;
        };
        std::stable_sort(v.begin(), v.end(), [&](int x, int y) { return work(x) > work(y); });
        const int NS = std::get<1>(g.first);
        const int pk = std::get<4>(g.first) == 0;
        int lds_floats = 0;
        for (int i : v) lds_floats = std::max(lds_floats, pk ? packed_dwords(p.tab_total[i]) : p.tab_total[i]);
        const int segs = -std::get<2>(g.first);
        const int tables = std::min(-std::get<3>(g.first), tables_for(p, lds_floats, segs));
        if (tables < 1) { c->err = "score table does not fit LDS"; return STRQ_ERR_UNSUPPORTED; }
        bool known = std::get<0>(g.first) == 14;
        for (int i : v) known = known && in.m[i] == 870;
        p.launches.push_back({std::get<0>(g.first), NS, tables, (int)out.order.size(), (int)v.size(), (int)p.n_tasks, 0, lds_floats, pk, segs, known});
        out.order.insert(out.order.end(), v.begin(), v.end());
        p.n_tasks += (size_t)v.size() * segs;
        if (NS > 1) p.n_up += (int)v.size() * (NS - 1);
    }
    { size_t up = p.n_tasks; for (auto& L : p.launches) if (L.NS > 1) { L.first_up = (int)up; up += (size_t)L.count * (L.NS - 1); } }
    return STRQ_OK;
}

static int cut_pieces(CorePlan& p)
{
    strq_ctx* c = p.c; const AlignCoreIn& in = p.in; const AlignCoreOut& out = p.out;
    const int nb = p.nb;
    const size_t n_tasks = p.n_tasks;
    p.safe0 = n_tasks + p.n_up + (size_t)nb;
    p.pieces.resize(n_tasks); p.safe.resize(n_tasks);
    p.min_score.assign(nb, -INFINITY);
    p.two_round.assign(p.launches.size(), 0);
    p.ck_up.assign(nb, 0);
    size_t ck_floats = 0;
    for (size_t li = 0; li < p.launches.size(); ++li) {
        auto& L = p.launches[li];
        for (int x = 0; x < L.count; ++x) {
            const int pos = L.first + x, i = out.order[pos];
            const int n = in.n[i], R = in.R[i], ov = p.overlap[i];
            const size_t per_ckpt = (size_t)STRQ_CKPT_FIELDS(R) * 64;
            Piece* pf = &p.pieces[(size_t)L.first_task + (size_t)x * L.segs];
            Piece* ps = &p.safe[(size_t)L.first_task + (size_t)x * L.segs];
            cut(n, L.segs, ov, ps);
            const int ov_fast = overlap_for(p, in.m[i], ov);
            if (p.wins[i].n_win > 0) {
                const ScreenWindows& w = p.wins[i];
                const int ov_w = std::min(ov > 0 ? ov : (1 << 30), align_overlap_for_score(c->ap, in.m[i], w.lower_bound));
                for (int k = 0; k < L.segs; ++k) {
                    if (k < w.n_win) { const int start = std::max(0, w.lo[k] - 1 - ov_w); pf[k].col_off = start; pf[k].n = w.hi[k] - start; }
                    else { pf[k].col_off = 0; pf[k].n = 0; }
                }
                p.min_score[pos] = std::max(w.lower_bound, align_segment_min_score(c->ap, in.m[i], ov_w));
                p.two_round[li] = 1;
            } else if (L.segs > 1 && ov_fast < ov && cut(n, L.segs, ov_fast, pf) > 1) {
                p.min_score[pos] = align_segment_min_score(c->ap, in.m[i], ov_fast);
                p.two_round[li] = 1;
            } else {
                for (int k = 0; k < L.segs; ++k) pf[k] = ps[k];
            }
            for (int k = 0; k < L.segs; ++k) {
                pf[k].ck = ps[k].ck = ck_floats;
                ck_floats += (size_t)align_num_ckpts(std::max(pf[k].n, ps[k].n)) * per_ckpt;
            }
            if (L.NS > 1) { p.ck_up[i] = ck_floats; ck_floats += (size_t)(L.NS - 1) * align_num_ckpts(n) * per_ckpt; }
        }
    }
    for (char t : p.two_round) p.any_two_round |= t != 0;
    const size_t n_all_tasks = p.safe0 + (p.any_two_round ? n_tasks : 0);
    STRQ_HIP(c, c->ckpt.reserve(ck_floats * 4 + 256));
    p.r2_cap = p.screen2_ran ? std::max(1024, std::min(nb, 8192)) : 0;
    p.r2_0 = n_all_tasks;
    STRQ_HIP(c, c->tasks.reserve((n_all_tasks + (size_t)p.r2_cap * 4) * sizeof(AlignTask)));
    STRQ_HIP(c, c->results.reserve((2 * n_tasks + nb) * sizeof(AlignResult) + (size_t)nb * 12 + p.launches.size() * 4 + 256));
    p.tasks.resize(n_all_tasks);
    p.d_tasks = c->tasks.as<AlignTask>();
    p.d_heads = p.d_tasks + n_tasks + p.n_up;
    p.d_seg = c->results.as<AlignResult>();
    p.d_res = p.d_seg + n_tasks;
    p.d_seg_safe = p.d_res + nb;
    p.d_pick = reinterpret_cast<int32_t*>(p.d_seg_safe + n_tasks);
    p.d_min_score = reinterpret_cast<float*>(p.d_pick + nb);
    p.d_redo = reinterpret_cast<int*>(p.d_min_score + nb);
    p.d_redo_count = p.d_redo + nb;
    return STRQ_OK;
}

static int write_tasks(CorePlan& p)
{
    strq_ctx* c = p.c; const AlignCoreIn& in = p.in; AlignCoreOut& out = p.out;
    const int nb = p.nb, S = p.S;
    hipStream_t st = p.st;
    const size_t n_tasks = p.n_tasks, n_up = p.n_up, safe0 = p.safe0;
    std::vector<AlignTask>& tasks = p.tasks;
    for (auto& L : p.launches) {
        for (int x = 0; x < L.count; ++x) {
            const int pos = L.first + x, i = out.order[pos];
            const int R = in.R[i], M = in.m[i];
            AlignTask base; std::memset(&base, 0, sizeof(base));
            base.levels = in.d_levels + in.read_off[in.read[i]];
            base.rec = c->rec.as<int32_t>() + out.rec_off[i];
            base.n = in.n[i]; base.n_full = in.n[i]; base.m_total = M;
            auto strip = [&](int row0, int rows, size_t ck, int sidx) {
                AlignTask t = base;
                const int j = p.NJ[i] > 1 ? p.J0[i] + sidx : p.J0[i];
                const int k0 = row0 / S, k1 = (row0 + rows - 1) / S;
                t.row0 = row0; t.m = rows; t.k = k1 - k0 + 1; t.tsize = p.info[j].total;
                t.table = p.jobs[j].table; t.table3 = p.jobs[j].table3; t.band_lo = p.jobs[j].band_lo + (k0 - p.job_k0[j]);
                t.col0 = c->col0.as<float>() + p.col0_off[i] + row0;
                t.ckpt = c->ckpt.as<float>() + ck;
                return t;
            };
            tasks[n_tasks + n_up + pos] = strip(0, M, 0, 0);
            if (L.NS == 1) {
                for (int k = 0; k < L.segs; ++k) {
                    const size_t ti = (size_t)L.first_task + (size_t)x * L.segs + k;
                    AlignTask t = strip(0, M, p.pieces[ti].ck, 0);
                    t.levels += p.pieces[ti].col_off; t.n = p.pieces[ti].n; t.col_off = p.pieces[ti].col_off;
                    tasks[ti] = t;
                    if (p.any_two_round) {
                        AlignTask u = strip(0, M, p.safe[ti].ck, 0);
                        u.levels += p.safe[ti].col_off; u.n = p.safe[ti].n; u.col_off = p.safe[ti].col_off;
                        tasks[safe0 + ti] = u;
                    }
                }
            } else {
                const int rows_s = 64 * R;
                const size_t ck_strip = (size_t)align_num_ckpts(in.n[i]) * STRQ_CKPT_FIELDS(R) * 64;
                float* bnd = c->bnd.as<float>() + p.bnd_off[i];
                const size_t bnd_stride = 2 * ((size_t)in.n[i] + 2);
                for (int sidx = 0; sidx < L.NS; ++sidx) {
                    const bool last = sidx == L.NS - 1;
                    const int row0 = sidx * rows_s, rows = last ? M - row0 : rows_s;
                    const size_t slot = last ? (size_t)L.first_task + x : (size_t)L.first_up + (size_t)sidx * L.count + x;
                    AlignTask t = strip(row0, rows, last ? p.pieces[(size_t)L.first_task + x].ck : p.ck_up[i] + (size_t)sidx * ck_strip, sidx);
                    if (sidx > 0) { t.bnd_in = bnd + (size_t)(sidx - 1) * bnd_stride; t.up = p.d_tasks + L.first_up + (size_t)(sidx - 1) * L.count + x; }
                    if (!last) t.bnd_out = bnd + (size_t)sidx * bnd_stride;
                    tasks[slot] = t;
                    if (last && p.any_two_round) tasks[safe0 + slot] = t;
                }
            }
        }
    }
    STRQ_HIP(c, hipMemcpyAsync(p.d_tasks, tasks.data(), tasks.size() * sizeof(AlignTask), hipMemcpyHostToDevice, st));
    STRQ_HIP(c, hipMemsetAsync(p.d_seg, 0, (2 * n_tasks + nb) * sizeof(AlignResult), st));
    if (p.any_two_round) {
        STRQ_HIP(c, hipMemcpyAsync(p.d_min_score, p.min_score.data(), (size_t)nb * 4, hipMemcpyHostToDevice, st));
        STRQ_HIP(c, hipMemsetAsync(p.d_redo_count, 0, p.launches.size() * 4, st));
    }
    size_t scratch_words = 0;
    for (auto& L : p.launches) scratch_words = std::max(scratch_words, align_trace_scratch_words_per_wave(L.R));
    STRQ_HIP(c, c->scratch.reserve(scratch_words * 8 * (size_t)c->n_cu * trace_wpb));
    out.n_launches = 0; out.wave_steps = 0; out.columns = 0;
    for (size_t t = 0; t < n_tasks + n_up; ++t) if (tasks[t].n > 0) { out.wave_steps += align_num_steps(tasks[t].n); out.columns += tasks[t].n; }
    if (!p.launches.empty()) {
        const Launch& L = p.launches.back(); out.segs = L.segs; out.tables = L.tables; out.packed = L.packed; out.rows_per_lane = L.R;
        const int i = out.order[L.first];
        out.overlap_worst = p.overlap[i]; out.overlap_first = L.segs > 1 ? overlap_for(p, in.m[i], p.overlap[i]) : 0;
        const bool seg_kernel = L.NS == 1 && p.collapsed;
        const int32_t g[8] = {L.segs, L.tables, seg_kernel ? align_segments_wpe(L.segs, L.tables) : 0, L.R, L.packed, out.overlap_first, out.overlap_worst, (int32_t)p.launches.size()};
        std::memcpy(c->geometry, g, sizeof(g));
    }
    return STRQ_OK;
}
// ... 299 lines not shown
    float ms;
    STRQ_HIP(c, hipEventElapsedTime(&ms, c->ev[0], c->ev[1])); *t_lut += ms;
    STRQ_HIP(c, hipEventElapsedTime(&ms, c->ev[2], c->ev[3])); *t_fwd += ms + c->aborted_fwd_ms;
    c->screen_stats[0] += c->aborted_screen_ms;
    c->aborted_fwd_ms = c->aborted_screen_ms = 0;
    STRQ_HIP(c, hipEventElapsedTime(&ms, c->ev[3], c->ev[4])); *t_tr += ms;
    if (c->screen_ran) { STRQ_HIP(c, hipEventElapsedTime(&ms, c->ev[5], c->ev[6])); c->screen_stats[0] += ms; }
    return STRQ_OK;
}

size_t align_workspace_bytes(int n, int m, int R, int NS)
{
    size_t b = (size_t)NS * (align_num_ckpts(n) + align_num_ckpts(n) / 4 + 300) * STRQ_CKPT_FIELDS(R) * 64 * 4;
    if (NS > 1) b += (size_t)(NS - 1) * ((size_t)n + 2) * 8;
    (void)m;
    return b;
}

int align_validate_flank(strq_ctx* c, const float* f, int64_t mm, int samples, int* k_out, int* R_out, int* NS_out)
{
    if (mm < 1 || samples < 1 || mm % samples != 0) { c->err = "flank length must be a positive multiple of `samples`"; return STRQ_ERR_UNSUPPORTED; }
    for (int64_t i = 0; i < mm; ++i)
        if (std::memcmp(&f[i], &f[i - i % samples], 4) != 0) { c->err = "flank is not made of runs of `samples` equal values"; return STRQ_ERR_UNSUPPORTED; }
    const int S = align_effective_samples(samples);
    int R = 0, NS = 0;
    if (mm > (1 << 20) || !align_plan((int)mm, S, &R, &NS)) { c->err = "flank shape not covered by the compiled kernels"; return STRQ_ERR_UNSUPPORTED; }
    if (S == 6 && mm / S > STRQ_LUT_MAX_K && NS == 1) { R = 12; NS = (int)((mm + 64 * 12 - 1) / (64 * 12)); }
    *k_out = (int)(mm / S); *R_out = R; *NS_out = NS;
    return STRQ_OK;
}

static int run_align_batch(strq_ctx* c, const BatchIn& in, const BatchOut& out)
{
    const int S = align_effective_samples(in.samples);
    const int64_t NA = in.n_align;
    std::fill(c->timing, c->timing + 8, 0.0f);
    for (double& v : c->screen_stats) v = 0;
    if (NA == 0) return STRQ_OK;
    std::vector<int> m(NA), k(NA), R(NA), n(NA), NS(NA);
    for (int64_t a = 0; a < NA; ++a) {
        const int64_t mm = in.flank_off[a + 1] - in.flank_off[a];
        const int rd = in.align_read[a];
        if (rd < 0 || rd >= in.n_reads) { c->err = "align_read out of range"; return STRQ_ERR_ARG; }
        const int64_t nn = in.read_off[rd + 1] - in.read_off[rd];
        if (nn < 0 || nn > (int64_t)1 << 30) { c->err = "bad read length"; return STRQ_ERR_ARG; }
        const int rc = align_validate_flank(c, in.flank + in.flank_off[a], mm, in.samples, &k[a], &R[a], &NS[a]);
        if (rc) return rc;
        m[a] = (int)mm; n[a] = (int)nn;
    }
    hipStream_t st = c->stream;
    c->second_round[0] = 0; c->second_round[1] = NA; c->look2_served = 0;
    STRQ_HIP(c, c->redo_total.reserve(64));
    STRQ_HIP(c, hipMemsetAsync(c->redo_total.p, 0, 64, st));
    const int64_t tot_levels = in.read_off[in.n_reads];
    STRQ_HIP(c, c->levels.reserve((size_t)tot_levels + 64));
    STRQ_HIP(c, c->level_val.reserve((size_t)in.n_reads * 256 * 4));
    STRQ_HIP(c, hipMemcpyAsync(c->levels.p, in.levels, (size_t)tot_levels, hipMemcpyHostToDevice, st));
    STRQ_HIP(c, hipMemcpyAsync(c->level_val.p, in.level_val, (size_t)in.n_reads * 256 * 4, hipMemcpyHostToDevice, st));
    int64_t a0 = 0;
    float t_lut = 0, t_fwd = 0, t_tr = 0, n_hard = 0, n_launch = 0;
    std::fill(c->counters, c->counters + 8, 0.0);
    while (a0 < NA) {
        int64_t a1 = a0; size_t ck_bytes = 0;
        while (a1 < NA) {
            const size_t need = align_workspace_bytes(n[a1], m[a1], R[a1], NS[a1]);
            if (a1 > a0 && ck_bytes + need > c->max_ws_bytes) break;
            ck_bytes += need; ++a1;
        }
        const int nb = (int)(a1 - a0);
        AlignCoreIn ci; AlignCoreOut co;
        ci.nb = nb; ci.samples = S; ci.d_levels = c->levels.as<uint8_t>(); ci.read_off = in.read_off;
        ci.d_level_val = c->level_val.as<float>();
        std::vector<const float*> fl(nb);
        for (int i = 0; i < nb; ++i) fl[i] = in.flank + in.flank_off[a0 + i];
        ci.read = in.align_read + a0; ci.n = &n[a0]; ci.m = &m[a0]; ci.k = &k[a0]; ci.R = &R[a0]; ci.NS = &NS[a0]; ci.flank = fl.data();
        int rc = align_core(c, ci, co);
        if (rc) return rc;
        std::vector<AlignResult> res(nb);
        std::vector<int32_t> h_rec(co.rec_total);
        STRQ_HIP(c, hipMemcpyAsync(res.data(), co.d_results, (size_t)nb * sizeof(AlignResult), hipMemcpyDeviceToHost, st));
        if (out.rec) STRQ_HIP(c, hipMemcpyAsync(h_rec.data(), co.d_rec, co.rec_total * 4, hipMemcpyDeviceToHost, st));
        STRQ_HIP(c, hipStreamSynchronize(st));
        for (int pos = 0; pos < nb; ++pos) {
            const int i = co.order[pos]; const int64_t a = a0 + i;
            if (out.score) out.score[a] = res[pos].best;
            if (out.j_end) out.j_end[a] = res[pos].j_end;
            if (out.j0) out.j0[a] = res[pos].j0;
            if (out.rec) std::memcpy(out.rec + in.flank_off[a], &h_rec[co.rec_off[i]], (size_t)m[a] * 4);
        }
        rc = align_core_times(c, &t_lut, &t_fwd, &t_tr);
        if (rc) return rc;
        n_hard += co.n_hard; n_launch += co.n_launches;
        c->counters[0] += co.wave_steps; c->counters[1] += co.columns; c->counters[2] += nb;
        c->counters[3] = co.segs; c->counters[4] = co.tables; c->counters[5] = co.packed; c->counters[6] = co.rows_per_lane;
        a0 = a1;
    }
    c->timing[0] = t_lut; c->timing[1] = t_fwd; c->timing[2] = t_tr; c->timing[3] = t_lut + t_fwd + t_tr; c->timing[4] = n_hard; c->timing[7] = n_launch;
    {
        unsigned int redo = 0;
        STRQ_HIP(c, hipMemcpy(&redo, c->redo_total.p, 4, hipMemcpyDeviceToHost));
        c->second_round[0] = (int64_t)redo - c->look2_served;
    }
    return STRQ_OK;
}

}

extern "C" {

int strq_abi_version(void) { return 13; }

int strq_set_option(strq_ctx* c, const char* key, const char* value)
{
    if (!key || std::strncmp(key, "STRQ_", 5) != 0) { if (c) c->err = "option keys start with STRQ_"; return STRQ_ERR_ARG; }
    if (c) { std::lock_guard<std::mutex> lk(c->options_mu); if (value) c->options[key] = value; else c->options.erase(key); return STRQ_OK; }
    std::lock_guard<std::mutex> lk(g_opt_mu);
    if (value) g_opts[key] = value; else g_opts.erase(key);
    return STRQ_OK;
}

int strq_get_option(const strq_ctx* c, const char* key, char* out, int32_t cap)
{
    if (!key || !out || cap < 1) return STRQ_ERR_ARG;
    CtxScope scope(c);
    const char* v = opt(key);
    out[0] = 0;
    if (!v) return STRQ_OK;
    std::strncpy(out, v, (size_t)cap - 1); out[cap - 1] = 0;
    return STRQ_OK;
}

int strq_ctx_create(int device_id, strq_ctx** out)
{
    if (!out) return STRQ_ERR_ARG;
    *out = nullptr;
    int ndev = 0;
    if (hipGetDeviceCount(&ndev) != hipSuccess || ndev <= 0 || device_id < 0 || device_id >= ndev) return STRQ_ERR_DEVICE;
    if (hipSetDevice(device_id) != hipSuccess) return STRQ_ERR_DEVICE;
    strq_ctx* c = new strq_ctx();
    c->device = device_id;
    hipDeviceProp_t prop;
    if (hipGetDeviceProperties(&prop, device_id) != hipSuccess) { delete c; return STRQ_ERR_DEVICE; }
    c->n_cu = prop.multiProcessorCount;
    if (hipStreamCreateWithFlags(&c->stream, hipStreamNonBlocking) != hipSuccess) { delete c; return STRQ_ERR_DEVICE; }
    for (auto& e : c->ev) if (hipEventCreate(&e) != hipSuccess) { delete c; return STRQ_ERR_DEVICE; }
    *out = c;
    return STRQ_OK;
}

void strq_ctx_destroy(strq_ctx* c)
{
    if (!c) return;
    (void)hipSetDevice(c->device);
    if (c->stream) (void)hipStreamSynchronize(c->stream);
    detect_state_free(c);
    for (HostModel* m : c->models) delete m;
    for (auto& e : c->ev) if (e) (void)hipEventDestroy(e);
    if (c->ev_fork) (void)hipEventDestroy(c->ev_fork);
    if (c->side_join) (void)hipEventDestroy(c->side_join);
    if (c->side_stream) (void)hipStreamDestroy(c->side_stream);
    if (c->stream) (void)hipStreamDestroy(c->stream);
    delete c;
}

int strq_debug_live_allocations(int64_t out[2])
{
    if (!out) return STRQ_ERR_ARG;
    out[0] = live_allocations[0].load(); out[1] = live_allocations[1].load();
    return STRQ_OK;
}

const char* strq_last_error(const strq_ctx* c) { return c ? c->err.c_str() : "null context"; }

int strq_set_align_params(strq_ctx* c, const float p[6])
{
    if (!c || !p) return STRQ_ERR_ARG;
    c->ap = AlignParams{p[0], p[1], p[2], p[3], p[4], p[5]};
    return STRQ_OK;
}
int strq_get_align_params(const strq_ctx* c, float p[6])
{
    if (!c || !p) return STRQ_ERR_ARG;
    p[0] = c->ap.open_h; p[1] = c->ap.ext_h; p[2] = c->ap.open_v; p[3] = c->ap.ext_v;
    p[4] = c->ap.dist_offset; p[5] = c->ap.dist_min;
    return STRQ_OK;
}

int strq_device_synchronize(strq_ctx* c)
{
    if (!c) return STRQ_ERR_ARG;
    STRQ_HIP(c, hipSetDevice(c->device));
    STRQ_HIP(c, hipDeviceSynchronize());
    return STRQ_OK;
}

int strq_last_timing(const strq_ctx* c, float ms[8])
{
    if (!c || !ms) return STRQ_ERR_ARG;
    std::memcpy(ms, c->timing, sizeof(c->timing));
    return STRQ_OK;
}

int strq_last_counters(const strq_ctx* c, double out[8])
{
    if (!c || !out) return STRQ_ERR_ARG;
    std::memcpy(out, c->counters, sizeof(c->counters));
    return STRQ_OK;
}

int strq_debug_screen_plan(const float params[6], int32_t samples, int32_t max_n, int32_t out[6])
{
    if (!params || !out) return 0;
    const AlignParams p{params[0], params[1], params[2], params[3], params[4], params[5]};
    ScreenParams sp;
    if (!screen_plan(p, samples, max_n, &sp)) return 0;
    out[0] = sp.sc; out[1] = sp.hh; out[2] = sp.v; out[3] = sp.cadd; out[4] = sp.slack; out[5] = sp.merge_gap;
    return 1;
}

int strq_debug_score_tables(strq_ctx* c, int32_t n_jobs, const float* level_val, const float* cls_val, const int64_t* cls_off,
                            int32_t* info_out, int32_t* band_lo, float* table, uint8_t* planes,
                            int32_t* handed, int32_t handed_cap, int32_t* n_handed)
{
    strq::CtxScope scope_(c);
    if (!c) return STRQ_ERR_ARG;
    if (n_jobs < 1 || n_jobs > 4096 || !level_val || !cls_val || !cls_off || !info_out || !band_lo || !table || !planes || !n_handed ||
        handed_cap < 0 || (handed_cap > 0 && !handed) || cls_off[0] != 0) { c->err = "bad argument"; return STRQ_ERR_ARG; }
    int max_k = 0;
    for (int j = 0; j < n_jobs; ++j) {
        const int64_t k = cls_off[j + 1] - cls_off[j];
        if (k < 1 || k > STRQ_LUT_MAX_K) { c->err = "a score table has 1 to 158 classes"; return STRQ_ERR_ARG; }
        max_k = std::max(max_k, (int)k);
    }
    STRQ_HIP(c, hipSetDevice(c->device));
    hipStream_t st = c->stream;
    const size_t cls_tot = (size_t)cls_off[n_jobs], tab_tot = STRQ_TABLE_SLOT_FLOATS(cls_tot);
    STRQ_HIP(c, c->level_val.reserve((size_t)n_jobs * 256 * 4));
    STRQ_HIP(c, c->flank_cls.reserve(cls_tot * 4));
    STRQ_HIP(c, c->band_lo.reserve(cls_tot * 4));
    STRQ_HIP(c, c->tables.reserve(tab_tot * 4));
    STRQ_HIP(c, c->tables3.reserve(tab_tot * 3 + (size_t)n_jobs * 8 + 64));
    STRQ_HIP(c, c->lutinfo.reserve((size_t)n_jobs * (sizeof(LutJob) + sizeof(LutInfo))));
    STRQ_HIP(c, c->hard.reserve((size_t)hard_cap * (sizeof(HardEntry) + 4) + 64));
    STRQ_HIP(c, c->queue.reserve(STRQ_QUEUE_BYTES));
    STRQ_HIP(c, hipMemcpyAsync(c->level_val.p, level_val, (size_t)n_jobs * 256 * 4, hipMemcpyHostToDevice, st));
    STRQ_HIP(c, hipMemcpyAsync(c->flank_cls.p, cls_val, cls_tot * 4, hipMemcpyHostToDevice, st));
    STRQ_HIP(c, hipMemsetAsync(c->queue.p, 0, STRQ_QUEUE_BYTES, st));
    STRQ_HIP(c, hipMemsetAsync(c->tables3.p, 0, tab_tot * 3 + (size_t)n_jobs * 8, st));
    std::vector<LutJob> jobs(n_jobs);
    std::vector<LutInfo> info, reported;
    std::vector<HardEntry> he;
    TableBuild b;
    b.nj = n_jobs; b.max_k = max_k; b.jobs = &jobs; b.d_level_val = c->level_val.as<float>(); b.info = &info; b.reported = &reported; b.handed = &he;
    b.job_read.resize(n_jobs); b.job_cls.resize(n_jobs);
    for (int j = 0; j < n_jobs; ++j) {
        const size_t tab_off = STRQ_TABLE_SLOT_FLOATS(cls_off[j]);
        jobs[j].level_val = c->level_val.as<float>() + (size_t)j * 256;
        jobs[j].cls_val = c->flank_cls.as<float>() + cls_off[j];
        jobs[j].table = c->tables.as<float>() + tab_off;
        jobs[j].table3 = table3_slot(c, tab_off, j);
        jobs[j].band_lo = c->band_lo.as<int32_t>() + cls_off[j];
        jobs[j].k = (int32_t)(cls_off[j + 1] - cls_off[j]); jobs[j].pad_ = 0;
        b.job_read[j] = j;
        b.job_cls[j] = cls_val + cls_off[j];
    }
    const int rc = run_table_build(c, st, b);
    if (rc) return rc;
    for (int j = 0; j < n_jobs; ++j) {
        info_out[5 * j] = reported[j].total; info_out[5 * j + 1] = reported[j].need; info_out[5 * j + 2] = reported[j].packed;
        info_out[5 * j + 3] = reported[j].n_hard; info_out[5 * j + 4] = info[j].total;
    }
    STRQ_HIP(c, hipMemcpy(band_lo, c->band_lo.p, cls_tot * 4, hipMemcpyDeviceToHost));
    STRQ_HIP(c, hipMemcpy(table, c->tables.p, tab_tot * 4, hipMemcpyDeviceToHost));
    for (int j = 0; j < n_jobs; ++j)
        STRQ_HIP(c, hipMemcpy(planes + (size_t)cls_off[j] * 768 + (size_t)j * 8, jobs[j].table3, (size_t)jobs[j].k * 768 + 8, hipMemcpyDeviceToHost));
    *n_handed = (int32_t)he.size();
    for (size_t i = 0; i < he.size() && (int64_t)i < handed_cap; ++i) {
        handed[4 * i] = he[i].job; handed[4 * i + 1] = he[i].k; handed[4 * i + 2] = he[i].level; handed[4 * i + 3] = he[i].index;
    }
    return STRQ_OK;
}

int strq_last_overlap(const strq_ctx* c, double out[4])
{
    if (!c || !out) return STRQ_ERR_ARG;
    for (int i = 0; i < 4; ++i) out[i] = c->overlap[i];
    return STRQ_OK;
}
int strq_last_screen(const strq_ctx* c, double out[8])
{
    if (!c || !out) return STRQ_ERR_ARG;
    for (int i = 0; i < 8; ++i) out[i] = c->screen_stats[i];
    return STRQ_OK;
}

int strq_last_screen_mode(const strq_ctx* c, int32_t out[8])
{
    if (!c || !out) return STRQ_ERR_ARG;
    for (int i = 0; i < 8; ++i) out[i] = 0;
    out[0] = c->screen_mode_last; out[1] = c->coarse_pause; out[2] = c->screen_pause; out[3] = (int32_t)c->coarse_margin;
    out[5] = (int32_t)std::min<int64_t>(c->look2_served, INT32_MAX);
    out[4] = c->screen_mode_last ? c->coarse_merge_last : 0;
    out[6] = c->screen_mode_last ? c->screen_lds_last : 0;
    return STRQ_OK;
}

int strq_last_second_round(const strq_ctx* c, int64_t out[2])
{
    if (!c || !out) return STRQ_ERR_ARG;
    out[0] = c->second_round[0]; out[1] = c->second_round[1];
    return STRQ_OK;
}

int strq_last_viterbi_launches(const strq_ctx* c, int32_t out[4])
{
    if (!c || !out) return STRQ_ERR_ARG;
    std::memcpy(out, c->vit_launches, sizeof(c->vit_launches));
    return STRQ_OK;
}

int strq_last_geometry(const strq_ctx* c, int32_t out[8])
{
    if (!c || !out) return STRQ_ERR_ARG;
    std::memcpy(out, c->geometry, sizeof(c->geometry));
    return STRQ_OK;
}

int strq_align_batch(strq_ctx* c, int64_t n_align, int64_t n_reads, const uint8_t* levels,
                     const int64_t* read_off, const float* level_val, const int32_t* align_read,
                     const float* flank, const int64_t* flank_off, int32_t samples,
                     float* score, int64_t* j_end, int64_t* j0, int32_t* rec)
{
    strq::CtxScope scope_(c);
    if (!c) return STRQ_ERR_ARG;
    if (n_align < 0 || n_reads < 0 || (n_align > 0 && (!levels || !read_off || !level_val || !align_read || !flank || !flank_off)) || samples < 1) {
        c->err = "bad argument"; return STRQ_ERR_ARG;
    }
    STRQ_HIP(c, hipSetDevice(c->device));
    BatchIn in{n_align, n_reads, levels, read_off, level_val, align_read, flank, flank_off, samples};
    BatchOut out{score, j_end, j0, rec};
    return run_align_batch(c, in, out);
}

static int align_overlap_generic(strq_ctx* c, const float* a, int64_t n, const float* b, int64_t m, float* score,
                                 std::vector<int32_t>& rec, int64_t* je, int64_t* j0)
{
    if (n > ((int64_t)1 << 30) || m > ((int64_t)1 << 24) || (double)(n + 1) * (double)(m + 1) > 1.7e10) {
        c->err = "align_overlap: (n + 1) x (m + 1) exceeds the 16 GiB trace limit of the generic path"; return STRQ_ERR_UNSUPPORTED;
    }
    hipStream_t st = c->stream;
    auto encode = [](const float* x, int64_t len, std::vector<float>& vals, std::vector<uint32_t>& code) {
        std::vector<uint32_t> bits((size_t)len);
        std::memcpy(bits.data(), x, (size_t)len * 4);
        std::vector<uint32_t> uniq(bits);
        std::sort(uniq.begin(), uniq.end());
        uniq.erase(std::unique(uniq.begin(), uniq.end()), uniq.end());
        code.resize((size_t)len);
        for (int64_t i = 0; i < len; ++i) code[(size_t)i] = (uint32_t)(std::lower_bound(uniq.begin(), uniq.end(), bits[(size_t)i]) - uniq.begin());
        vals.resize(uniq.size());
        std::memcpy(vals.data(), uniq.data(), uniq.size() * 4);
    };
    std::vector<float> va, vb; std::vector<uint32_t> ca, cb;
    encode(a, n, va, ca); encode(b, m, vb, cb);
    const size_t na = va.size(), nbv = vb.size();
    if ((double)na * (double)nbv > 2.0e9) { c->err = "align_overlap: more than 2e9 distinct (a, b) value pairs"; return STRQ_ERR_UNSUPPORTED; }
    const size_t tab = std::max<size_t>(1, na * nbv);
    const int hard_cap = 1 << 20;
    STRQ_HIP(c, c->gen_codes.reserve(((size_t)n + (size_t)m + na + nbv) * 4 + 64));
    STRQ_HIP(c, c->gen_table.reserve(tab * 4 + 64));
    STRQ_HIP(c, c->gen_bnd.reserve(((size_t)n + 1) * 16 + ((size_t)m + 1) * 4 + 256));
    STRQ_HIP(c, c->gen_trace.reserve(((size_t)n + 1) * ((size_t)m + 1) + 64));
    STRQ_HIP(c, c->gen_hard.reserve((size_t)hard_cap * (sizeof(GenericHard) + 4) + 64));
    STRQ_HIP(c, c->results.reserve(sizeof(AlignResult) + 64));
    STRQ_HIP(c, c->queue.reserve(STRQ_QUEUE_BYTES));
    uint32_t* d_ca = c->gen_codes.as<uint32_t>(); uint32_t* d_cb = d_ca + n;
    float* d_va = reinterpret_cast<float*>(d_cb + m); float* d_vb = d_va + na;
    float* d_tab = c->gen_table.as<float>();
    float* d_bnd = c->gen_bnd.as<float>();
    GenericHard* d_hard = c->gen_hard.as<GenericHard>(); float* d_hvals = reinterpret_cast<float*>(d_hard + hard_cap);
    int* d_count = c->queue.as<int>();
    if (n) STRQ_HIP(c, hipMemcpyAsync(d_ca, ca.data(), (size_t)n * 4, hipMemcpyHostToDevice, st));
    STRQ_HIP(c, hipMemcpyAsync(d_cb, cb.data(), (size_t)m * 4, hipMemcpyHostToDevice, st));
    if (na) STRQ_HIP(c, hipMemcpyAsync(d_va, va.data(), na * 4, hipMemcpyHostToDevice, st));
    STRQ_HIP(c, hipMemcpyAsync(d_vb, vb.data(), nbv * 4, hipMemcpyHostToDevice, st));
    STRQ_HIP(c, hipMemsetAsync(d_count, 0, 4, st));
    int hard_count = 0;
    if (na) {
        if (launch_generic_table(st, d_va, (int)na, d_vb, (int)nbv, d_tab, d_hard, d_count, hard_cap, c->ap)) { c->err = "table launch failed"; return STRQ_ERR_DEVICE; }
        STRQ_HIP(c, hipMemcpyAsync(&hard_count, d_count, 4, hipMemcpyDeviceToHost, st));
        STRQ_HIP(c, hipStreamSynchronize(st));
        if (hard_count > hard_cap) {
            std::vector<float> full(tab);
            for (size_t y = 0; y < nbv; ++y) for (size_t x = 0; x < na; ++x) full[y * na + x] = host_cell_score(c->ap, va[x], vb[y]);
            STRQ_HIP(c, hipMemcpy(d_tab, full.data(), tab * 4, hipMemcpyHostToDevice));
        } else if (hard_count > 0) {
            std::vector<GenericHard> he((size_t)hard_count); std::vector<float> hv((size_t)hard_count);
            STRQ_HIP(c, hipMemcpy(he.data(), d_hard, (size_t)hard_count * sizeof(GenericHard), hipMemcpyDeviceToHost));
            for (int i = 0; i < hard_count; ++i) hv[(size_t)i] = host_cell_score(c->ap, va[(size_t)he[(size_t)i].ia], vb[(size_t)he[(size_t)i].ib]);
            STRQ_HIP(c, hipMemcpyAsync(d_hvals, hv.data(), (size_t)hard_count * 4, hipMemcpyHostToDevice, st));
            if (launch_generic_patch(st, d_tab, (int)na, d_hard, d_hvals, hard_count)) { c->err = "patch launch failed"; return STRQ_ERR_DEVICE; }
        }
    }
    c->timing[4] = (float)hard_count;
    std::vector<float> col0((size_t)m + 1);
    host_col0(c->ap, (int)m, col0.data());
    GenericAlignArgs ga;
    ga.code_a = d_ca; ga.code_b = d_cb; ga.table = d_tab;
    ga.bnd_S[0] = d_bnd; ga.bnd_V[0] = d_bnd + (n + 1); ga.bnd_S[1] = d_bnd + 2 * (n + 1); ga.bnd_V[1] = d_bnd + 3 * (n + 1);
    float* d_col0 = d_bnd + 4 * (n + 1);
    STRQ_HIP(c, hipMemcpyAsync(d_col0, col0.data(), ((size_t)m + 1) * 4, hipMemcpyHostToDevice, st));
    ga.col0 = d_col0; ga.trace = c->gen_trace.as<uint8_t>(); ga.result = c->results.as<AlignResult>();
    ga.p = c->ap; ga.n = (int32_t)n; ga.m = (int32_t)m; ga.na = (int32_t)na; ga.nb = (int32_t)nbv;
    if (launch_generic_align(st, ga)) { c->err = "generic align launch failed"; return STRQ_ERR_DEVICE; }
    AlignResult res;
    std::vector<uint8_t> trace(((size_t)n + 1) * ((size_t)m + 1));
    STRQ_HIP(c, hipMemcpyAsync(&res, ga.result, sizeof(res), hipMemcpyDeviceToHost, st));
    STRQ_HIP(c, hipMemcpyAsync(trace.data(), ga.trace, trace.size(), hipMemcpyDeviceToHost, st));
    STRQ_HIP(c, hipStreamSynchronize(st));
    rec.assign((size_t)m, 0);
    int64_t i = m, j = res.j_end; int state = 0;
    const size_t W = (size_t)n + 1;
    while (i > 0 && j > 0) {
        const uint8_t tr = trace[(size_t)i * W + (size_t)j];
        if (state == 0) {
            const unsigned dsel = tr & 3u;
            if (dsel == 0) { rec[(size_t)i - 1] = (int32_t)(j << 1); --i; --j; }
            else state = (int)dsel;
        } else if (state == 1) { --j; if (!(tr & 4u)) state = 0; }
        else { rec[(size_t)i - 1] = (int32_t)((j << 1) | 1); --i; if (!(tr & 8u)) state = 0; }
    }
    for (; i > 0; --i) rec[(size_t)i - 1] = (int32_t)((j << 1) | 1);
    *score = res.best; *je = res.j_end; *j0 = j;
    return STRQ_OK;
}

int strq_align_overlap(strq_ctx* c, const float* a, int64_t n, const float* b, int64_t m, float* score,
                       uint64_t* a_idx, uint64_t* b_idx, int32_t* rec_out, int64_t* j_end_out, int64_t* j0_out)
{
    strq::CtxScope scope_(c);
    if (!c) return STRQ_ERR_ARG;
    if ((!a && n > 0) || !b || n < 0 || m < 1 || !score) { c->err = "bad argument"; return STRQ_ERR_ARG; }
    STRQ_HIP(c, hipSetDevice(c->device));
    std::fill(c->timing, c->timing + 8, 0.0f);
    std::vector<int32_t> rec((size_t)m);
    int64_t je = 0, j0 = 0;
    std::vector<float> vals(a, a + n);
    std::sort(vals.begin(), vals.end(), [](float x, float y) { return __builtin_bit_cast(uint32_t, x) < __builtin_bit_cast(uint32_t, y); });
    vals.erase(std::unique(vals.begin(), vals.end(), [](float x, float y) { return std::memcmp(&x, &y, 4) == 0; }), vals.end());
    int run = 0;
    { int64_t start = 0;
      for (int64_t i = 1; i <= m; ++i)
          if (i == m || std::memcmp(&b[i], &b[start], 4) != 0) { int len = (int)std::min<int64_t>(i - start, 1 << 20); run = run ? std::__gcd(run, len) : len; start = i; } }
    bool fast = vals.size() <= 256 && run >= 1 && !strq::opt("STRQ_GENERIC_ALIGN");
    for (float v : vals) if (v != v) fast = false;
    if (fast) {
        std::sort(vals.begin(), vals.end());
        for (size_t x = 1; x < vals.size(); ++x) if (vals[x] == vals[x - 1]) fast = false;
        int kk, RR, NN;
        if (fast && align_validate_flank(c, b, m, run, &kk, &RR, &NN) != STRQ_OK) fast = false;
    }
    if (fast) {
        std::vector<uint8_t> lv((size_t)n);
        for (int64_t i = 0; i < n; ++i) lv[(size_t)i] = (uint8_t)(std::lower_bound(vals.begin(), vals.end(), a[i]) - vals.begin());
        std::vector<float> lval(256, INFINITY);
        std::copy(vals.begin(), vals.end(), lval.begin());
        const int64_t roff[2] = {0, n}, foff[2] = {0, m};
        const int32_t ar = 0;
        BatchIn in{1, 1, lv.data(), roff, lval.data(), &ar, b, foff, run};
        BatchOut out{score, &je, &j0, rec.data()};
        const int rc = run_align_batch(c, in, out);
        if (rc) return rc;
    } else {
        const int rc = align_overlap_generic(c, a, n, b, m, score, rec, &je, &j0);
        if (rc) return rc;
    }
    if (rec_out) std::memcpy(rec_out, rec.data(), (size_t)m * 4);
    if (j_end_out) *j_end_out = je;
    if (j0_out) *j0_out = j0;
    if (a_idx || b_idx) {
        if (a_idx) for (int64_t x = 0; x < j0; ++x) a_idx[x] = (uint64_t)x;
        int64_t ai = j0, col = j0;
        for (int64_t kk = 0; kk < m; ++kk) {
            const int64_t j = rec[(size_t)kk] >> 1; const bool vert = rec[(size_t)kk] & 1;
            const int64_t upto = vert ? j : j - 1;
            for (; ai < upto; ++ai, ++col) if (a_idx) a_idx[ai] = (uint64_t)col;
            if (b_idx) b_idx[kk] = (uint64_t)col;
            if (!vert) { if (a_idx) a_idx[ai] = (uint64_t)col; ++ai; }
            ++col;
        }
        for (; ai < n; ++ai, ++col) if (a_idx) a_idx[ai] = (uint64_t)col;
    }
    return STRQ_OK;
}

}
```

### strique_amd/csrc/strq_ctx.h

```cpp
#pragma once
#include <hip/hip_runtime.h>
#include <stdint.h>
#include <string>
#include <vector>
#include <map>
#include <cstdio>
#include <functional>
#include <mutex>
#include <atomic>
#include <utility>
#include "align_kernels.h"
#include "viterbi_kernels.h"
#include "forward_kernels.h"
#include "mod_llr_kernels.h"
#include "variant_kernels.h"
#include "screen_kernels.h"
#include "strq_opt.h"

namespace strq {

inline std::atomic<int64_t> live_allocations[2];

template <bool PINNED> struct OwnedBuf {
    void* p = nullptr;
    size_t cap = 0;
    OwnedBuf() = default;
    OwnedBuf(const OwnedBuf&) = delete;
    OwnedBuf& operator=(const OwnedBuf&) = delete;
    ~OwnedBuf() { release(); }
    hipError_t reserve(size_t bytes)
    {
        if (bytes <= cap) return hipSuccess;
        release();
        const size_t want = bytes + bytes / 8 + (PINNED ? 0 : 256);
        const hipError_t e = PINNED ? hipHostMalloc(&p, want, hipHostMallocDefault) : hipMalloc(&p, want);
        if (e != hipSuccess) { p = nullptr; return e; }
        cap = want; ++live_allocations[PINNED];
        return e;
    }
    void release()
    {
        if (p) { (void)(PINNED ? hipHostFree(p) : hipFree(p)); --live_allocations[PINNED]; }
        p = nullptr; cap = 0;
    }
    void swap(OwnedBuf& o) { std::swap(p, o.p); std::swap(cap, o.cap); }
    template <class T> T* as() const { return reinterpret_cast<T*>(p); }
};
using DevBuf = OwnedBuf<false>;
using PinBuf = OwnedBuf<true>;

#define STRQ_QUEUE_BYTES 65536
#define STRQ_QUEUE_FIRST 8
#define STRQ_QUEUE_SLOTS (STRQ_QUEUE_BYTES / 4)

struct AlignCoreIn {
    int nb = 0, samples = 6;
    const uint8_t* d_levels = nullptr;
    const int64_t* read_off = nullptr;
    const float* d_level_val = nullptr;
    const int32_t* read = nullptr;
    const int* n = nullptr; const int* m = nullptr; const int* k = nullptr; const int* R = nullptr;
    const int* NS = nullptr;
    const float* const* flank = nullptr;
    std::function<int()> after_tables;
};
struct AlignCoreOut {
    std::vector<int> order;
    std::vector<size_t> rec_off;
    size_t rec_total = 0;
    AlignTask* d_tasks = nullptr; AlignResult* d_results = nullptr; int32_t* d_rec = nullptr;
    int n_hard = 0;
    int n_launches = 0;
    double wave_steps = 0, columns = 0;
    int segs = 1, tables = 0, packed = 0, rows_per_lane = 0;
    int overlap_first = 0, overlap_worst = 0;
};

struct HostModel {
    VitModel h;
    const VitModel* dev = nullptr;
    DevBuf blob;
    DevBuf g2_blob;
    int32_t n_states = 0, silent_start = 0, start = 0, end = 0;
    std::vector<int32_t> in_ptr, in_src, emis_kind, count_inc, state_tag;
    std::vector<double> in_logp, emis_a, emis_b, emis_c;
    std::vector<int32_t> edge_csr, chain_csr;
    int32_t fwd_stages = 1;
    std::vector<double> fwd_logp;
    DevBuf fwd_blob;
    const FwdModel* fwd_dev = nullptr;
    DevBuf llr_blob;
    const LlrModel* llr_dev = nullptr;
    int32_t llr_mode = -1;
    DevBuf var_blob;
    const VarModel* var_dev = nullptr;
    int32_t var_mode = -1, var_nb = 0;
    DevBuf tract_blob;
    int32_t n_tracts = 0;
};

}

struct strq_ctx {
    std::map<std::string, std::string> options;
    mutable std::mutex options_mu;
    int device = 0;
    int n_cu = 0;
    hipStream_t stream = nullptr;
    hipStream_t side_stream = nullptr;
    hipEvent_t ev_fork = nullptr, side_join = nullptr;
    hipEvent_t ev[8] = {};
    strq::AlignParams ap{-2.0f, -8.0f, -2.0f, -8.0f, 8.0f, -16.0f};
    std::string err;
    float timing[8] = {};
    double counters[8] = {};
    int32_t geometry[8] = {};
    int32_t vit_launches[4] = {};
    int32_t tract_shape_last = -1;
    int64_t second_round[2] = {};
    strq::DevBuf redo_total;
    int64_t look2_served = 0;
    double screen_stats[8] = {};
    double overlap[4] = {};
    bool screen_ran = false;
    int screen_pause = 0;
    int coarse_pause = 0;
    int coarse_fail = 0, screen_fail = 0;
    float coarse_margin = 384.0f;
    float aborted_fwd_ms = 0, aborted_screen_ms = 0;
    int screen_mode_last = 0;
    int coarse_merge_last = 0;
    int screen_lds_last = 0;
    
    strq::DevBuf levels, level_val, flank_cls, tables, tables3, band_lo, col0, ckpt, rec, tasks, results,
        queue, scratch, lutinfo, hard, misc, vit_x, vit_tasks, vit_bp, vit_path, bnd,
        gen_codes, gen_table, gen_bnd, gen_trace, gen_hard,
        screen,
        ckpt2;
    std::vector<strq::HostModel*> models;
    void* detect = nullptr;
    size_t max_ws_bytes = (size_t)96 << 30;
    std::vector<float> score_fracs; double mean_n = 0;
};

namespace strq {
struct CtxScope { const strq_ctx* prev; explicit CtxScope(const strq_ctx* c); ~CtxScope(); };
int align_core(strq_ctx* c, const AlignCoreIn& in, AlignCoreOut& out);
int align_core_times(strq_ctx* c, float* t_lut, float* t_fwd, float* t_tr);
int align_validate_flank(strq_ctx* c, const float* f, int64_t m, int samples, int* k_out, int* R_out, int* NS_out);
size_t align_workspace_bytes(int n, int m, int R, int NS);
float host_cell_score(const AlignParams& p, float h, float v);
void detect_state_free(strq_ctx* c);
int detect_drain(strq_ctx* c);
int viterbi_launch_status(int vrc);
int forward_model(strq_ctx* c, HostModel* hm);
struct TractPosWindow { VitTask task; const HostModel* hm; int64_t base; int64_t n[3]; };
struct TractPosOut { std::vector<int32_t> status; std::vector<std::vector<int64_t>> pos; };
int tract_positions(strq_ctx* c, const std::vector<TractPosWindow>& w, TractPosOut& out, double* stats);
void host_stats_batch(const double* signals, const int64_t* offsets, int64_t n_reads, bool want_raw, double* out,
                      const double* const* reads = nullptr);
}

#define STRQ_ENTER(ctx)                                                                        \
    if (!(ctx)) return STRQ_ERR_ARG;                                                           \
    strq::CtxScope scope_(ctx);                                                                \
    STRQ_HIP(ctx, hipSetDevice((ctx)->device))

#define STRQ_HIP(ctx, call)                                                                    \
    do {                                                                                       \
        hipError_t e_ = (call);                                                                \
        if (e_ != hipSuccess) {                                                                \
            (ctx)->err = std::string(#call) + ": " + hipGetErrorString(e_);                    \
            return STRQ_ERR_DEVICE;                                                            \
        }                                                                                      \
    } while (0)

namespace strq {
inline int reset_queue_heads(strq_ctx* c, hipStream_t st)
{
    STRQ_HIP(c, c->queue.reserve(1024));
    STRQ_HIP(c, hipMemsetAsync(c->queue.p, 0, 1024, st));
    return STRQ_OK;
}
}
```

### strique_amd/ffi.py

```python
import ctypes
import os

import numpy as np

_HERE = os.path.dirname(os.path.abspath(__file__))
LIB_PATH = os.environ.get("STRQ_LIB") or os.path.join(_HERE, "lib", "libstrique_hip.so")

STRQ_OK, STRQ_ERR_ARG, STRQ_ERR_DEVICE, STRQ_ERR_UNSUPPORTED, STRQ_ERR_NOMEM = 0, 1, 2, 3, 4

SCAN_SYMBOLS = ("strq_scan_batch_reads", "strq_scan_set", "strq_scan_clear", "strq_batch_fetch_scan")

_lib = None


class StriqueHipError(RuntimeError):
    def __init__(self, code, message):
        RuntimeError.__init__(self, "libstrique_hip error %d: %s" % (code, message))
        self.code = code


def _torch_hip_runtime():
    import importlib.util
    try:
        spec = importlib.util.find_spec("torch")
    except (ImportError, ValueError):
        spec = None
    if spec is None or not spec.submodule_search_locations:
        return None
    cand = os.path.join(list(spec.submodule_search_locations)[0], "lib", "libamdhip64.so")
    return cand if os.path.exists(cand) else None


def mapped_hip_runtimes():
    seen = set()
    try:
        for line in open("/proc/self/maps"):
            f = line.split()[-1]
            if "libamdhip64" in os.path.basename(f):
                seen.add(os.path.realpath(f))
    except OSError:
        pass
    return sorted(seen)


def _pin_hip_runtime():
    choice = os.environ.get("STRQ_HIP_RUNTIME", "auto")
    if choice == "system" or mapped_hip_runtimes():
        return None
    path = _torch_hip_runtime() if choice in ("auto", "torch") else choice
    if path is None:
        if choice == "torch":
            raise ImportError("STRQ_HIP_RUNTIME=torch: no torch wheel with a bundled libamdhip64.so found")
        return None
    ctypes.CDLL(path, mode=ctypes.RTLD_GLOBAL)
    return path


def load_library(path=None):
    global _lib
    if _lib is None:
        path = path or LIB_PATH
        if not os.path.exists(path):
            raise ImportError("%s not found: run `python -m strique_amd.build` (hipcc, gfx950) first" % path)
        _pin_hip_runtime()
        lib = ctypes.CDLL(path)
        lib.strq_last_error.restype = ctypes.c_char_p
        lib.strq_last_error.argtypes = [ctypes.c_void_p]
        lib.strq_ctx_destroy.restype = None
        lib.strq_ctx_destroy.argtypes = [ctypes.c_void_p]
        lib.strq_set_option.argtypes = [ctypes.c_void_p, ctypes.c_char_p, ctypes.c_char_p]
        lib.strq_get_option.argtypes = [ctypes.c_void_p, ctypes.c_char_p, ctypes.c_char_p, ctypes.c_int32]
        for name in SCAN_SYMBOLS:
            getattr(lib, name).restype = ctypes.c_int
        _lib = lib
    return _lib


def _ptr(a):
    return None if a is None else a.ctypes.data_as(ctypes.c_void_p)


def _c(a, dtype):
    return np.ascontiguousarray(a, dtype=dtype)


def host_stats(signals, offsets, want_raw=False):
    lib = load_library()
    signals = _c(signals, np.float64); offsets = _c(offsets, np.int64)
    out = np.zeros((len(offsets) - 1, 6), np.float64)
    rc = lib.strq_host_stats(_ptr(signals), _ptr(offsets), ctypes.c_int64(len(offsets) - 1), ctypes.c_int32(1 if want_raw else 0), _ptr(out))
    if rc != STRQ_OK:
        raise StriqueHipError(rc, "strq_host_stats: bad argument")
    return out


def live_allocations():
    out = np.zeros(2, np.int64)
    rc = load_library().strq_debug_live_allocations(_ptr(out))
    if rc != STRQ_OK:
        raise StriqueHipError(rc, "strq_debug_live_allocations: bad argument")
    return int(out[0]), int(out[1])


def _offsets(arrays, dtype):
    off = np.zeros(len(arrays) + 1, np.int64)
    for i, a in enumerate(arrays):
        off[i + 1] = off[i] + len(a)
    flat = np.concatenate([_c(a, dtype).ravel() for a in arrays] + [np.zeros(1, dtype)])
    return flat, off


_IMAGE_ORDER = ("src", "lp", "src2", "lp2", "start_lp", "kind", "hub", "ea", "eb", "ec", "end_src", "end_lp")
VARIANT_IMAGE_SHAPES = {"src": (np.int32, (2, 8, 64)), "lp": (np.float64, (2, 8, 64)), "src2": (np.int32, (3, 2, 4, 64)), "lp2": (np.float64, (3, 2, 4, 64)),
                        "start_lp": (np.float64, (2, 64)), "kind": (np.int32, (2, 64)), "hub": (np.int32, (2, 64)), "ea": (np.float64, (2, 64)),
                        "eb": (np.float64, (2, 64)), "ec": (np.float64, (2, 64)), "end_src": (np.int32, (4, 8)), "end_lp": (np.float64, (4, 8))}
MOD_LLR_IMAGE_SHAPES = dict(VARIANT_IMAGE_SHAPES, src2=(np.int32, (2, 4, 64)), lp2=(np.float64, (2, 4, 64)), start_lp=(np.float64, (2, 2, 64)),
                            end_src=(np.int32, (2, 8)), end_lp=(np.float64, (2, 8)))


def _debug_image(entry, shapes, baked, extra):
    lib = load_library()
    arrs = [_c(baked.in_ptr, np.int32), _c(baked.in_src, np.int32), _c(baked.in_logp, np.float64), _c(baked.emis_kind, np.int32),
            _c(baked.emis_a, np.float64), _c(baked.emis_b, np.float64), _c(baked.emis_c, np.float64),
            None if baked.tag is None else _c(baked.tag, np.int32)]
    brc = ctypes.c_int32(-1); head = np.zeros(10, np.int32); offs = np.zeros(12, np.int64); nbytes = ctypes.c_int64(0)
    image = np.zeros(1 << 16, np.uint8); why = ctypes.create_string_buffer(512)
    rc = getattr(lib, entry)(ctypes.c_int32(baked.n_states), ctypes.c_int32(baked.silent_start), ctypes.c_int32(baked.start), ctypes.c_int32(baked.end),
                             *([_ptr(a) for a in arrs] + extra + [ctypes.byref(brc), _ptr(head), _ptr(offs), _ptr(image), ctypes.c_int64(len(image)),
                                                                ctypes.byref(nbytes), why, ctypes.c_int32(512)]))
    if rc != STRQ_OK:
        raise StriqueHipError(rc, "%s: bad argument" % entry)
    out = {"rc": int(brc.value), "why": why.value.decode()}
    if brc.value:
        return out
    if nbytes.value > len(image):
        raise StriqueHipError(STRQ_ERR_NOMEM, "%s: an image of %d bytes" % (entry, nbytes.value))
    out.update(n_emit=int(head[0]), n_branch=int(head[1]), mode=int(head[2]), deg=int(head[3]), deg2=int(head[4]),
               end_deg=[int(v) for v in head[5:5 + int(head[1])]])
    for name, at in zip(_IMAGE_ORDER, offs):
        dtype, shape = shapes[name]
        count = int(np.prod(shape))
        out[name] = np.frombuffer(image.tobytes(), dtype, count, int(at)).reshape(shape).copy()
    return out


def debug_variant_image(baked, n_alt):
    return _debug_image("strq_debug_variant_image", VARIANT_IMAGE_SHAPES, baked, [ctypes.c_int32(n_alt)])


def debug_mod_llr_image(baked):
    return _debug_image("strq_debug_mod_llr_image", MOD_LLR_IMAGE_SHAPES, baked, [])


VIT_COUNT, VIT_BACKPTR, VIT_MARK, VIT_HUB, VIT_UNIT = range(5)
VIT_SHAPE_CSR, VIT_SHAPE_G2, VIT_SHAPE_SS = 8, 9, 16
VIT_SRC_F64, VIT_SRC_F64_AFFINE, VIT_SRC_I16_AFFINE = 0, 1, 2


def debug_viterbi_plan(baked):
    lib = load_library()
    hints = getattr(baked, 'hint_slot', None) is not None and (np.asarray(baked.hint_slot)[:baked.silent_start] >= 0).all()
    arrs = [_c(baked.in_ptr, np.int32), _c(baked.in_src, np.int32), _c(baked.in_logp, np.float64), _c(baked.emis_kind, np.int32),
            _c(baked.emis_a, np.float64), _c(baked.emis_b, np.float64), _c(baked.emis_c, np.float64), _c(baked.count_inc, np.int32),
            None if baked.tag is None else _c(baked.tag, np.int32),
            _c(baked.hint_slot, np.int32) if hints else None, _c(baked.hint_lane, np.int32) if hints else None]
    out = np.zeros(48, np.int32); why = ctypes.create_string_buffer(256)
    rc = lib.strq_debug_viterbi_plan(ctypes.c_int32(baked.n_states), ctypes.c_int32(baked.silent_start), ctypes.c_int32(baked.start),
                                     ctypes.c_int32(baked.end), *([_ptr(a) for a in arrs] + [_ptr(out), why, ctypes.c_int32(256)]))
    if rc != STRQ_OK:
        raise StriqueHipError(rc, "strq_debug_viterbi_plan: " + why.value.decode())
    shape = int(out[0])
    epl, spl = int(out[10]), int(out[11])
    return {"shape": shape, "row": shape & ~VIT_SHAPE_SS if shape >= 0 else -1, "ss": bool(shape >= 0 and shape & VIT_SHAPE_SS),
            "shapes": [int(v) for v in out[0:5]], "modes": [m for m in range(5) if out[5 + m]], "epl": epl, "spl": spl,
            "e_deg": [int(v) for v in out[12:12 + epl]], "s_deg": [int(v) for v in out[20:20 + spl]], "e_flat": [int(v) for v in out[28:28 + epl]],
            "single_stage": int(out[36]), "silent_counted": int(out[37]), "rec_state": int(out[38]),
            "unit_state": (int(out[39]), int(out[40])), "csr": int(out[41])}


class Context(object):

    def __init__(self, device=0):
        self._lib = load_library()
        self._h = ctypes.c_void_p()
        rc = self._lib.strq_ctx_create(ctypes.c_int(device), ctypes.byref(self._h))
        if rc != STRQ_OK:
            self._h = None
            raise StriqueHipError(rc, "cannot create a context on HIP device %d (no GPU?)" % device)
        self.device = device

    def close(self):
        if getattr(self, "_h", None):
            self._lib.strq_ctx_destroy(self._h)
            self._h = None

    def __del__(self):
        try:
            self.close()
        except Exception:
            pass

    def _check(self, rc):
        if rc != STRQ_OK:
            raise StriqueHipError(rc, self._lib.strq_last_error(self._h).decode())

    def device_synchronize(self):
        self._check(self._lib.strq_device_synchronize(self._h))

    def set_option(self, key, value):
        v = None if value is None else str(value).encode()
        self._check(self._lib.strq_set_option(self._h, key.encode(), v))

    def get_option(self, key):
        buf = ctypes.create_string_buffer(256)
        self._check(self._lib.strq_get_option(self._h, key.encode(), buf, ctypes.c_int32(256)))
        return buf.value.decode()

    def set_align_params(self, open_h, ext_h, open_v, ext_v, dist_offset, dist_min):
        p = np.array([open_h, ext_h, open_v, ext_v, dist_offset, dist_min], dtype=np.float32)
        self._check(self._lib.strq_set_align_params(self._h, _ptr(p)))

    def get_align_params(self):
        p = np.zeros(6, np.float32)
        self._check(self._lib.strq_get_align_params(self._h, _ptr(p)))
        return p

    def align_overlap(self, a, b, want_idx=True):
        a = _c(a, np.float32); b = _c(b, np.float32)
        n, m = len(a), len(b)
        score = ctypes.c_float(); j_end = ctypes.c_int64(); j0 = ctypes.c_int64()
        rec = np.zeros(m, np.int32)
        a_idx = np.zeros(n, np.uint64) if want_idx else None
        b_idx = np.zeros(m, np.uint64) if want_idx else None
        self._check(self._lib.strq_align_overlap(self._h, _ptr(a), ctypes.c_int64(n), _ptr(b), ctypes.c_int64(m),
                                                 ctypes.byref(score), _ptr(a_idx), _ptr(b_idx), _ptr(rec),
                                                 ctypes.byref(j_end), ctypes.byref(j0)))
        return score.value, a_idx, b_idx, rec, j_end.value, j0.value

    def align_batch(self, levels, read_off, level_val, align_read, flank, flank_off, samples=6, want_rec=True):
        levels = _c(levels, np.uint8); read_off = _c(read_off, np.int64); level_val = _c(level_val, np.float32)
        align_read = _c(align_read, np.int32); flank = _c(flank, np.float32); flank_off = _c(flank_off, np.int64)
        na, nr = len(align_read), len(read_off) - 1
        score = np.zeros(na, np.float32); j_end = np.zeros(na, np.int64); j0 = np.zeros(na, np.int64)
        rec = np.zeros(len(flank), np.int32) if want_rec else None
        self._check(self._lib.strq_align_batch(self._h, ctypes.c_int64(na), ctypes.c_int64(nr), _ptr(levels), _ptr(read_off),
                                               _ptr(level_val), _ptr(align_read), _ptr(flank), _ptr(flank_off),
                                               ctypes.c_int32(samples), _ptr(score), _ptr(j_end), _ptr(j0), _ptr(rec)))
        return score, j_end, j0, rec

    def last_timing(self):
        t = np.zeros(8, np.float32)
        self._check(self._lib.strq_last_timing(self._h, _ptr(t)))
        return t

    def last_counters(self):
        t = np.zeros(8, np.float64)
        self._check(self._lib.strq_last_counters(self._h, _ptr(t)))
        return t

    def last_viterbi_launches(self):
        g = np.zeros(4, np.int32)
        self._check(self._lib.strq_last_viterbi_launches(self._h, _ptr(g)))
        return dict(zip(("launches", "register_resident", "lane_layout", "general"), (int(v) for v in g)))

    def last_second_round(self):
        g = np.zeros(2, np.int64)
        self._check(self._lib.strq_last_second_round(self._h, _ptr(g)))
        return int(g[0]), int(g[1])

    def last_screen(self):
        g = np.zeros(8, np.float64)
        self._check(self._lib.strq_last_screen(self._h, _ptr(g)))
        keys = ("ms", "screened", "windowed", "whole_read", "window_columns", "wave_steps", "scale", "candidate_chunks")
        out = dict(zip(keys, (float(v) for v in g)))
        m = np.zeros(8, np.int32)
        self._check(self._lib.strq_last_screen_mode(self._h, _ptr(m)))
        out["mode"] = {0: None, 1: "fine", 2: "coarse"}.get(int(m[0]))
        out["coarse_pause"], out["fine_pause"], out["coarse_margin"], out["merge"] = int(m[1]), int(m[2]), int(m[3]), int(m[4])
        out["second_look"] = int(m[5])
        out["lds_layout"] = {0: None, 1: "lanes", 2: "rows"}.get(int(m[6]))
        return out

    def last_overlap(self):
        g = np.zeros(4, np.float64)
        self._check(self._lib.strq_last_overlap(self._h, _ptr(g)))
        return dict(zip(("viterbi_ms", "under_screen_ms", "under_alignment_stage_ms", "sub_batches"), (float(v) for v in g)))

    def last_geometry(self):
        g = np.zeros(8, np.int32)
        self._check(self._lib.strq_last_geometry(self._h, _ptr(g)))
        keys = ("waves_per_alignment", "tables_per_cu", "wpe", "rows_per_lane", "packed", "overlap_first", "overlap_worst", "launch_groups")
        return dict(zip(keys, (int(v) for v in g)))

    def model_create(self, baked):
        mid = ctypes.c_int32(-1)
        arrs = [_c(baked.in_ptr, np.int32), _c(baked.in_src, np.int32), _c(baked.in_logp, np.float64),
                _c(baked.emis_kind, np.int32), _c(baked.emis_a, np.float64), _c(baked.emis_b, np.float64),
                _c(baked.emis_c, np.float64), _c(baked.count_inc, np.int32), _c(baked.tag, np.int32)]
        hints = getattr(baked, 'hint_slot', None) is not None and (np.asarray(baked.hint_slot)[:baked.silent_start] >= 0).all()
        arrs += [_c(baked.hint_slot, np.int32) if hints else None, _c(baked.hint_lane, np.int32) if hints else None]
        self._check(self._lib.strq_model_create(self._h, ctypes.c_int32(baked.n_states), ctypes.c_int32(baked.silent_start),
                                                ctypes.c_int32(baked.start), ctypes.c_int32(baked.end),
                                                *[_ptr(a) for a in arrs], ctypes.byref(mid)))
        psum = getattr(baked, 'in_logp_sum', None)
        if psum is not None and len(psum) == len(baked.in_logp) and np.all(psum >= baked.in_logp) and not np.array_equal(psum, baked.in_logp):
            self._check(self._lib.strq_model_set_forward_logp(self._h, mid, _ptr(_c(baked.in_logp_sum, np.float64))))
        self.last_positions_rc = self.last_positions_error = None
        if getattr(baked, 'pos_kind', None) is not None:
            rc = self._lib.strq_model_set_positions(self._h, mid, _ptr(_c(baked.pos_kind, np.int32)), _ptr(_c(baked.pos_index, np.int32)))
            self.last_positions_rc = rc
            self.last_positions_error = self._lib.strq_last_error(self._h).decode() if rc == STRQ_ERR_UNSUPPORTED else None
            if rc not in (STRQ_OK, STRQ_ERR_UNSUPPORTED):
                self._check(rc)
        return mid.value

    def viterbi_batch(self, model_id, seqs, want_path=False):
        off = np.zeros(len(seqs) + 1, np.int64)
        for i, s in enumerate(seqs):
            off[i + 1] = off[i] + len(s)
        x = np.concatenate([_c(s, np.float64) for s in seqs]) if len(seqs) else np.zeros(0)
        n = len(seqs)
        logp = np.zeros(n); counted = np.zeros(n, np.int64); status = np.zeros(n, np.int32)
        paths = np.zeros(len(x), np.int32) if want_path else None
        self._check(self._lib.strq_viterbi_batch(self._h, ctypes.c_int32(model_id), ctypes.c_int64(n), _ptr(x), _ptr(off),
                                                 _ptr(logp), _ptr(counted), _ptr(status), _ptr(paths)))
        if want_path:
            paths = [paths[off[i]:off[i + 1]] for i in range(n)]
        return logp, counted, status, paths

    def debug_viterbi_mode(self, model_id, mode, seqs):
        return self._debug_viterbi(model_id, mode, seqs, VIT_SRC_F64, None, False, False)

    def debug_viterbi_sourced(self, model_id, mode, kind, samples, consts, tracts=False):
        consts = _c(consts, np.float64).reshape(-1, 6)
        if len(consts) != len(samples):
            raise ValueError("consts must have one row per window")
        return self._debug_viterbi(model_id, mode, samples, kind, consts, tracts, True)

    def _debug_viterbi(self, model_id, mode, seqs, kind, consts, tracts, sourced):
        n = len(seqs)
        x, x_off = _offsets(seqs, np.int16 if kind == VIT_SRC_I16_AFFINE else np.float64)
        logp = np.zeros(n); counted = np.zeros(n, np.int64); status = np.zeros(n, np.int32); dbg = np.zeros((n, 4), np.uint32)
        launched = np.full(1, -1, np.int32)
        rec = rec_off = None
        if mode in (VIT_HUB, VIT_UNIT):
            rec_off = np.zeros(n + 1, np.int64)
            for i, s in enumerate(seqs):
                rec_off[i + 1] = rec_off[i] + (8 * (len(s) + 1) if mode == VIT_HUB else 8 * len(s))
            rec = np.full(int(rec_off[-1]) + 8, 0xA5, np.uint8)
        tcounts = np.zeros((n, 3), np.int64) if tracts else None
        if not sourced:
            self._check(self._lib.strq_debug_viterbi_mode(self._h, ctypes.c_int32(model_id), ctypes.c_int32(mode), ctypes.c_int64(n), _ptr(x), _ptr(x_off),
                                                          _ptr(logp), _ptr(counted), _ptr(status), _ptr(dbg), _ptr(rec), _ptr(rec_off), _ptr(launched)))
        else:
            self._check(self._lib.strq_debug_viterbi_sourced(self._h, ctypes.c_int32(model_id), ctypes.c_int32(mode), ctypes.c_int32(kind),
                                                             ctypes.c_int32(1 if tracts else 0), ctypes.c_int64(n), _ptr(x), _ptr(x_off), _ptr(consts),
                                                             _ptr(logp), _ptr(counted), _ptr(status), _ptr(dbg), _ptr(rec), _ptr(rec_off), _ptr(tcounts),
                                                             _ptr(launched)))
        records = [None] * n
        if rec is not None:
            for i in range(n):
                raw = rec[int(rec_off[i]):int(rec_off[i + 1])]
                records[i] = raw.view(np.uint64).copy() if mode == VIT_HUB else raw.view(np.uint32).reshape(-1, 2).copy()
        out = {"logp": logp, "counted": counted, "status": status, "dbg": dbg, "records": records, "launched": int(launched[0])}
        if tracts:
            out["tract_counts"] = tcounts
        return out

    def forward_batch(self, model_id, xs, c0=None):
        n = len(xs)
        off = np.zeros(n + 1, np.int64)
        for i, s in enumerate(xs):
            off[i + 1] = off[i] + len(s)
        x = np.concatenate([_c(s, np.float64) for s in xs]) if n else np.zeros(0)
        if len(x) == 0:
            x = np.zeros(1)
        ll = np.zeros(n); mean = np.zeros(n); var = np.zeros(n); status = np.zeros(n, np.int32)
        c0a = None if c0 is None else _c(c0, np.int64)
        if c0a is not None and len(c0a) != n:
            raise ValueError("c0 must have one entry per window")
        self._check(self._lib.strq_forward_batch(self._h, ctypes.c_int32(model_id), ctypes.c_int64(n), _ptr(x), _ptr(off), _ptr(c0a),
                                                 _ptr(ll), _ptr(mean), _ptr(var), _ptr(status)))
        return ll, mean, var, status

    def model_set_tracts(self, model_id, n_tracts, tract_of):
        self._check(self._lib.strq_model_set_tracts(self._h, ctypes.c_int32(model_id), ctypes.c_int32(n_tracts), _ptr(_c(tract_of, np.int32))))

    def viterbi_tracts(self, model_id, xs):
        n = len(xs)
        x, off = _offsets(xs, np.float64)
        logp = np.zeros(n); counts = np.zeros((n, 3), np.int64); status = np.zeros(n, np.int32)
        self._check(self._lib.strq_viterbi_tracts(self._h, ctypes.c_int32(model_id), ctypes.c_int64(n), _ptr(x), _ptr(off),
                                                  _ptr(logp), _ptr(counts), _ptr(status)))
        return logp, counts, status

    def viterbi_tract_positions(self, model_id, xs):
        n = len(xs)
        x, off = _offsets(xs, np.float64)
        logp = np.zeros(n); counts = np.zeros((n, 3), np.int64); status = np.zeros(max(1, n), np.int32)
        pos_off = np.zeros(3 * n + 1, np.int64); pool = np.zeros(max(1, int(off[-1])), np.int64)
        self._check(self._lib.strq_viterbi_tract_positions(self._h, ctypes.c_int32(model_id), ctypes.c_int64(n), _ptr(x), _ptr(off), _ptr(logp), _ptr(counts),
                                                           _ptr(status), _ptr(pos_off), _ptr(pool), ctypes.c_int64(len(pool))))
        return logp, counts, status[:n], [tuple(pool[pos_off[3 * i + j]:pos_off[3 * i + j + 1]].copy() for j in range(3)) for i in range(n)]

    def debug_tract_shape(self):
        shape = ctypes.c_int32(-1)
        self._check(self._lib.strq_debug_tract_shape(self._h, ctypes.byref(shape)))
        return int(shape.value)

    def viterbi(self, model_id, x, want_path=True):
        logp, counted, status, paths = self.viterbi_batch(model_id, [x], want_path)
        return logp[0], int(counted[0]), int(status[0]), (paths[0] if want_path else None)

    def set_pore_stats(self, tail_lo, tail_hi, model_min, model_max):
        self._check(self._lib.strq_set_pore_stats(self._h, ctypes.c_double(tail_lo), ctypes.c_double(tail_hi),
                                                  ctypes.c_double(model_min), ctypes.c_double(model_max)))

    def target_add(self, prefix_ext, suffix_ext, trim_prefix, trim_suffix, samples, model_id, count_bias):
        pe = _c(prefix_ext, np.float32); se = _c(suffix_ext, np.float32)
        tid = ctypes.c_int32(-1)
        self._check(self._lib.strq_target_add(self._h, _ptr(pe), ctypes.c_int64(len(pe)), _ptr(se), ctypes.c_int64(len(se)),
                                              ctypes.c_int32(trim_prefix), ctypes.c_int32(trim_suffix), ctypes.c_int32(samples),
                                              ctypes.c_int32(model_id), ctypes.c_int32(count_bias), ctypes.byref(tid)))
        return tid.value

    def target_set_mod(self, target_id, mod_model_id, mod_min, mod_max):
        self._check(self._lib.strq_target_set_mod(self._h, ctypes.c_int32(target_id), ctypes.c_int32(mod_model_id),
                                                  ctypes.c_double(mod_min), ctypes.c_double(mod_max)))

    def batch_fetch_mod(self):
        off = np.zeros(self._n_batch + 1, np.int64)
        self._check(self._lib.strq_batch_fetch_mod(self._h, None, ctypes.c_int64(0), _ptr(off)))
        pool = np.zeros(max(1, int(off[-1])), np.uint8)
        self._check(self._lib.strq_batch_fetch_mod(self._h, _ptr(pool), ctypes.c_int64(len(pool)), _ptr(off)))
        raw = pool.tobytes()
        return [raw[off[i]:off[i + 1]].decode() for i in range(self._n_batch)]

    def _last(self, entry, keys, floats=("ms",)):
        out = np.zeros(len(keys))
        self._check(getattr(self._lib, "strq_last_" + entry)(self._h, _ptr(out)))
        return {k: float(v) if k in floats else int(v) for k, v in zip(keys, out)}

    def _fetch_records(self, entry, dtype):
        n = getattr(self, '_n_batch', 0)
        out = np.zeros(max(1, n), dtype=dtype)
        self._check(getattr(self._lib, "strq_batch_fetch_" + entry)(self._h, _ptr(out), ctypes.c_int64(n)))
        return out[:n]

    def _switch(self, entry, on, level=None):
        args = [ctypes.c_int32(1 if on else 0)] + ([] if level is None else [ctypes.c_double(level if on else 0.0)])
        self._check(getattr(self._lib, "strq_set_" + entry)(self._h, *args))

    def set_units(self, on):
        self._switch("units", on)

    def batch_fetch_units(self):
        n = getattr(self, '_n_batch', 0)
        off = np.zeros(n + 1, np.int64); dec = np.zeros(max(1, n), np.int32)
        self._check(self._lib.strq_batch_fetch_units(self._h, None, ctypes.c_int64(0), _ptr(off), _ptr(dec)))
        pool = np.zeros(max(1, int(off[-1])), np.int64)
        self._check(self._lib.strq_batch_fetch_units(self._h, _ptr(pool), ctypes.c_int64(len(pool)), _ptr(off), _ptr(dec)))
        return [pool[off[i]:off[i + 1]].copy() if dec[i] else None for i in range(n)]

    def last_units(self):
        return self._last("units", ("ms", "ws_bytes", "windows", "positions"), floats=("ms", "ws_bytes"))

    def set_confidence(self, on):
        self._switch("confidence", on)

    def batch_fetch_confidence(self):
        n = getattr(self, '_n_batch', 0)
        out = np.zeros((max(1, n), 3), np.float64); dec = np.zeros(max(1, n), np.int32)
        self._check(self._lib.strq_batch_fetch_confidence(self._h, _ptr(out), _ptr(dec)))
        return [(float(out[i, 0]), float(out[i, 1]), float(out[i, 2])) if dec[i] else None for i in range(n)]

    def last_confidence(self):
        return self._last("confidence", ("ms", "windows", "no_path", "max_exponent"))

    def set_mod_llr(self, on):
        self._switch("mod_llr", on)

    def batch_fetch_mod_llr(self):
        n = getattr(self, '_n_batch', 0)
        off = np.zeros(n + 1, np.int64)
        self._check(self._lib.strq_batch_fetch_mod_llr(self._h, None, ctypes.c_int64(0), _ptr(off)))
        pool = np.zeros((max(1, int(off[-1])), 2), np.float64)
        self._check(self._lib.strq_batch_fetch_mod_llr(self._h, _ptr(pool), ctypes.c_int64(len(pool)), _ptr(off)))
        return [pool[off[i]:off[i + 1]].copy() if off[i + 1] > off[i] else None for i in range(n)]

    def last_mod_llr(self):
        return self._last("mod_llr", ("ms", "units", "reads", "launches"))

    def target_set_variants(self, target_id, model_id, lo, hi, n_alt, context_units):
        self._check(self._lib.strq_target_set_variants(self._h, ctypes.c_int32(target_id), ctypes.c_int32(model_id), ctypes.c_double(lo), ctypes.c_double(hi),
                                                       ctypes.c_int32(n_alt), ctypes.c_int32(context_units)))

    def set_variants(self, on):
        self._switch("variants", on)

    def batch_fetch_variants(self):
        n = getattr(self, '_n_batch', 0)
        count_v = np.zeros(max(1, n), np.int32); dec = np.zeros(max(1, n), np.int32); off = np.zeros(n + 1, np.int64)
        vt = ctypes.c_int64(0)
        self._check(self._lib.strq_batch_fetch_variants(self._h, _ptr(count_v), _ptr(dec), _ptr(off), None, None, ctypes.c_int64(0),
                                                        None, None, ctypes.c_int64(0), ctypes.byref(vt)))
        npass = int(off[-1])
        branch = np.zeros(max(1, npass), np.int8); end = np.zeros(max(1, npass), np.int64)
        vpool = np.zeros(max(1, vt.value), np.float64); voff = np.zeros(npass + 1, np.int64)
        self._check(self._lib.strq_batch_fetch_variants(self._h, _ptr(count_v), _ptr(dec), _ptr(off), _ptr(branch), _ptr(end), ctypes.c_int64(len(branch)),
                                                        _ptr(vpool), _ptr(voff), ctypes.c_int64(len(vpool)), None))
        out = []
        for i in range(n):
            if not dec[i]:
                out.append(None)
                continue
            a, b = int(off[i]), int(off[i + 1])
            nb = int(voff[a + 1] - voff[a]) if b > a else 0
            V = vpool[voff[a]:voff[b]].reshape(b - a, nb).copy() if b > a else np.zeros((0, 0))
            out.append((int(count_v[i]), branch[a:b].copy(), end[a:b].copy(), V))
        return out

    def last_variants(self):
        return self._last("variants", ("launches", "passages", "ms", "reads"))

    def target_set_anchored(self, target_id, end_model_id, end_bias, start_model_id, start_bias):
        self._check(self._lib.strq_target_set_anchored(self._h, ctypes.c_int32(target_id), ctypes.c_int32(end_model_id), ctypes.c_int32(end_bias),
                                                       ctypes.c_int32(start_model_id), ctypes.c_int32(start_bias)))

    def set_anchored(self, on, min_score=0.0):
        self._switch("anchored", on, min_score)

    def batch_fetch_anchored(self):
        return self._fetch_records("anchored", ANCHORED_DTYPE)

    def last_anchored(self):
        d = self._last("anchored", ("ms", 0, 1, 2, 3, "launches", "register_resident", "lane_layout"))
        return {'ms': d['ms'], 'kinds': tuple(d[k] for k in range(4)), **{k: d[k] for k in ('launches', 'register_resident', 'lane_layout')}}

    def target_set_tracts(self, target_id, model_id, n_tracts=0, bias=()):
        b = np.zeros(3, np.int32)
        b[:len(bias)] = bias
        self._check(self._lib.strq_target_set_tracts(self._h, ctypes.c_int32(target_id), ctypes.c_int32(model_id), ctypes.c_int32(n_tracts), _ptr(b)))

    def set_tracts(self, on):
        self._switch("tracts", on)

    def batch_fetch_tracts(self):
        return self._fetch_records("tracts", TRACTS_DTYPE)

    def last_tracts(self):
        return self._last("tracts", ("ms", "windows", "launches", "failed"))

    def set_tract_positions(self, on):
        self._switch("tract_positions", on)

    def batch_fetch_tract_positions(self):
        n = getattr(self, '_n_batch', 0)
        off = np.zeros(3 * n + 1, np.int64); ps = np.zeros(max(1, n), np.int32)
        self._check(self._lib.strq_batch_fetch_tract_positions(self._h, _ptr(ps), _ptr(off), None, ctypes.c_int64(0)))
        pool = np.zeros(max(1, int(off[-1])), np.int64)
        self._check(self._lib.strq_batch_fetch_tract_positions(self._h, _ptr(ps), _ptr(off), _ptr(pool), ctypes.c_int64(len(pool))))
        return [(int(ps[i]), tuple(pool[off[3 * i + j]:off[3 * i + j + 1]].copy() for j in range(3)) if ps[i] == 0 else None) for i in range(n)]

    def last_tract_positions(self):
        return self._last("tract_positions", ("ms", "windows", "launches", "bp_bytes"), floats=("ms", "bp_bytes"))

    def target_set_flank_mod(self, target_id, which, profile_model_id, flank_len, column_of, groups):
        col = _c(column_of, np.int32)
        g = _c(groups if len(groups) else np.zeros((0, 6)), np.int32).reshape(-1, 6)
        self._check(self._lib.strq_target_set_flank_mod(self._h, ctypes.c_int32(target_id), ctypes.c_int32(which), ctypes.c_int32(profile_model_id),
                                                        ctypes.c_int32(flank_len), _ptr(col), ctypes.c_int32(len(g)), _ptr(g) if len(g) else None))

    def set_flank_mod(self, on):
        self._switch("flank_mod", on)

    def batch_fetch_flank_mod(self):
        n = getattr(self, '_n_batch', 0)
        called = np.zeros(max(1, n), np.int32); off = np.zeros(n + 1, np.int64)
        self._check(self._lib.strq_batch_fetch_flank_mod(self._h, _ptr(called), _ptr(off), None, ctypes.c_int64(0)))
        pool = np.zeros(max(1, int(off[-1])), FLANK_MOD_DTYPE)
        self._check(self._lib.strq_batch_fetch_flank_mod(self._h, _ptr(called), _ptr(off), _ptr(pool), ctypes.c_int64(len(pool))))
        return [pool[int(off[i]):int(off[i + 1])].copy() if called[i] else None for i in range(n)]

# ... 282 lines not shown
```

Measured before the change: 24930.

## Add level-indexed byte LDS image layout for the coarse flank-pair screen

Adds a third LDS layout for the two-flank coarse screen (merge 3). Each lane's class scores are stored as one byte per signal level, over the level range the LUT build now reports, instead of as 16-bit band entries. The kernel rescales levels into byte-row addresses, requantizes scores to a byte scale, and maps chunk maxima back to the original scale. It also allows 8 pieces per group instead of 4. The goal is a smaller LDS footprint and cheaper score lookups, which raises occupancy and parallelism. In exchange there is coarser quantization, some saturation at 255, and extra overlap work from more pieces, all gated by a host-side heuristic.

```diff
diff --git a/strique_amd/csrc/lut_kernels.h b/strique_amd/csrc/lut_kernels.h
--- a/strique_amd/csrc/lut_kernels.h
+++ b/strique_amd/csrc/lut_kernels.h
@@ -17,7 +17,7 @@
     int32_t* band_lo;
     int32_t k, pad_;
 };
-struct LutInfo { int32_t total, n_hard, need, packed; };
+struct LutInfo { int32_t total, n_hard, need, packed, lvl; };
 struct HardEntry { int32_t job, k, level, index; };
 
 int launch_lut_build(hipStream_t stream, const LutJob* jobs, LutInfo* info, int n_jobs, int max_k,
diff --git a/strique_amd/csrc/lut_kernels.hip b/strique_amd/csrc/lut_kernels.hip
--- a/strique_amd/csrc/lut_kernels.hip
+++ b/strique_amd/csrc/lut_kernels.hip
@@ -33,13 +33,14 @@
     __shared__ float cls[STRQ_LUT_MAX_K];
     __shared__ int lo[STRQ_LUT_MAX_K], hi[STRQ_LUT_MAX_K + 1];
     __shared__ int width, n_local, plat_lo, plat_hi, rebuild, unpackable;
+    __shared__ int lvl_lo, lvl_hi;
     __shared__ unsigned char dup[STRQ_LUT_MAX_K];
     __shared__ unsigned short local_hard[STRQ_LUT_LOCAL_HARD][2];
     const LutJob jb = jobs[blockIdx.x];
     const int q = threadIdx.x, lane = q & 63, wave = q >> 6;
     v[q] = jb.level_val[q];
     for (int k = q; k < jb.k; k += 256) cls[k] = jb.cls_val[k];
-    if (q == 0) { width = 0; n_local = 0; plat_lo = 255; plat_hi = 0; rebuild = 0; unpackable = 0; }
+    if (q == 0) { width = 0; n_local = 0; plat_lo = 255; plat_hi = 0; rebuild = 0; unpackable = 0; lvl_lo = 255; lvl_hi = 0; }
     __syncthreads();
     {
         const float v0 = v[0], v255 = v[255], vq = v[q];
@@ -48,7 +49,7 @@
         if (q > 0 && !(v[q - 1] <= vq)) rebuild = 1;
     }
     __syncthreads();
-    if (rebuild) { if (q == 0) { info[blockIdx.x].total = 0; info[blockIdx.x].need = 0; info[blockIdx.x].packed = 0; info[blockIdx.x].n_hard = -1; } return; }
+    if (rebuild) { if (q == 0) { info[blockIdx.x].total = 0; info[blockIdx.x].need = 0; info[blockIdx.x].packed = 0; info[blockIdx.x].n_hard = -1; info[blockIdx.x].lvl = 255 << 8; } return; }
     const int plat_lo_r = plat_lo, plat_hi_r = plat_hi < plat_lo ? plat_lo : plat_hi;
     auto in_band = [&](int lv, float c) { bool hd; return cell_score_dev(p, v[lv], c, &hd) > p.dist_min; };
     for (int k = q; k < jb.k; k += 256) {
@@ -75,6 +76,7 @@
         lo[k] = el | (er << 8) | ((!none && l <= plat_lo_r) ? 0 : 1 << 16) | ((!none && h >= plat_hi_r) ? 0 : 1 << 17);
         hi[k] = er - el + 1;
         atomicMax(&width, er - el + 1);
+        if (!none) { atomicMin(&lvl_lo, el); atomicMax(&lvl_hi, er); }
     }
     __syncthreads();
     for (int k = q; k < jb.k; k += 256) {
@@ -131,6 +133,7 @@
         info[blockIdx.x].need = width;
         info[blockIdx.x].packed = (nh == 0 && !unpackable) ? 1 : 0;
         info[blockIdx.x].n_hard = nh;
+        info[blockIdx.x].lvl = lvl_lo <= lvl_hi ? lvl_lo | (lvl_hi << 8) : 0;
         for (int i = 0; i < nh; ++i) {
             const int k = local_hard[i][0], lv = local_hard[i][1];
             const int slot = atomicAdd(hard_count, 1);
diff --git a/strique_amd/csrc/screen_kernels.h b/strique_amd/csrc/screen_kernels.h
--- a/strique_amd/csrc/screen_kernels.h
+++ b/strique_amd/csrc/screen_kernels.h
@@ -6,6 +6,8 @@
 #define STRQ_SCREEN_R 14
 #define STRQ_SCREEN_S 6
 #define STRQ_SCREEN_SEG 4
+#define STRQ_SCREEN_SEG_LEVELS 8
+#define STRQ_SCREEN_SEG_MAX 8
 #define STRQ_SCREEN_CHUNK_COLS 128
 #define STRQ_SCREEN_MAX_WINDOWS 4
 #define STRQ_SCREEN2_CPL 5
@@ -22,6 +24,8 @@
     int32_t merge_gap;
     int32_t max_cand;
     int32_t margin;
+    int32_t seg;
+    int32_t byte_sc;
 };
 
 struct ScreenTask {
@@ -42,6 +46,7 @@
     int32_t* out[2];
     int32_t tsize[2], k[2];
     int32_t n, col_off, n_chunks;
+    uint32_t lvl;
 };
 
 struct ScreenWindows {
@@ -63,8 +68,17 @@
 int screen2_lanes_rows(int need_a, int need_b);
 bool screen2_lanes_fit(int rows);
 size_t screen2_lanes_lds_bytes(int rows);
+#define STRQ_SCREEN_LDS_LANES 1
+#define STRQ_SCREEN_LDS_ROWS 2
+#define STRQ_SCREEN_LDS_LEVELS 3
+int screen2_levels_plan(const AlignParams& p, int samples, int max_n, int merge, ScreenParams* sp);
+ScreenParams screen2_byte_frame(const ScreenParams& sp);
+uint32_t screen2_levels_range(uint32_t lvl_a, uint32_t lvl_b);
+int screen2_levels_rows(uint32_t range);
+bool screen2_levels_fit(int rows);
+size_t screen2_levels_lds_bytes(int rows);
 int launch_screen2(hipStream_t stream, const Screen2Task* tasks, int n_groups, int* queue, const ScreenParams& sp,
-                   size_t lds_bytes, int groups_per_cu, int n_cu, int merge, int lanes_rows);
+                   size_t lds_bytes, int groups_per_cu, int n_cu, int merge, int layout, int rows);
 int launch_screen_windows(hipStream_t stream, const ScreenTask* tasks, int n_groups, const ScreenParams& sp,
                           const int32_t* bound_scaled, ScreenWindows* out, const int32_t* list = nullptr, const int32_t* theta_list = nullptr);
 
diff --git a/strique_amd/csrc/screen_kernels.hip b/strique_amd/csrc/screen_kernels.hip
--- a/strique_amd/csrc/screen_kernels.hip
+++ b/strique_amd/csrc/screen_kernels.hip
@@ -5,6 +5,7 @@
 #include <cmath>
 #include "screen_kernels.h"
 #include "screen_lds_layout.h"
+#include "screen_levels_layout.h"
 
 namespace strq {
 
@@ -49,6 +50,25 @@
     int r;
     asm("v_cndmask_b32_e64 %0, %1, %2, %3" : "=v"(r) : "v"(if0), "v"(if1), "s"(mask));
     return r;
+}
+
+__device__ __forceinline__ int mad3_lo16(int q, int add)
+{
+    int r;
+    asm("v_mad_u32_u16 %0, %1, 3, %2" : "=v"(r) : "v"(q), "v"(add));
+    return r;
+}
+__device__ __forceinline__ int mad3_hi16(int q, int add)
+{
+    int r;
+    asm("v_mad_u32_u16 %0, %1, 3, %2 op_sel:[1,0,0,0]" : "=v"(r) : "v"(q), "v"(add));
+    return r;
+}
+__device__ __forceinline__ int ceil_scaled(float s, float scf)
+{
+    float c = ceilf(s * scf);
+    if (fmaf(s, scf, -c) > 0.0f) c += 1.0f;
+    return (int)c;
 }
 
 struct LaneConst { int lo2[C], hi2[C], off[C]; };
@@ -237,9 +257,10 @@
 
 struct Lane2Const { int lo2[CPL], hi2[CPL], off[CPL]; };
 
-template <int RPC, int CMG>
+template <int RPC, int CMG, int LAYOUT>
 struct Screen2 {
     static constexpr int R2 = RPC * CPL;
+    static constexpr bool LEVELS = LAYOUT == STRQ_SCREEN_LDS_LEVELS;
     static_assert(CMG == 1 || CMG == 2 || CMG == 4, "groups must divide the 64 steps of a chunk");
     const char* lds;
     const Lane2Const& lc;
@@ -250,22 +271,30 @@
     int qq;
     int scA[CPL], scB[CPL];
 
+    template <bool HI>
+    __device__ __forceinline__ int column(int qpair) const
+    {
+        if constexpr (LEVELS) return HI ? mad3_hi16(qpair, lc.off[0]) : mad3_lo16(qpair, lc.off[0]);
+        else return HI ? (int)((unsigned)qpair >> 16) : (qpair & 0xffff);
+    }
     __device__ __forceinline__ int score(int q2, int c) const
     {
-        return *reinterpret_cast<const uint16_t*>(lds + med3i(q2, lc.lo2[c], lc.hi2[c]) + lc.off[c]);
+        if constexpr (LEVELS) return *reinterpret_cast<const uint8_t*>(lds + q2 + screen_levels::class_offset(c));
+        else return *reinterpret_cast<const uint16_t*>(lds + med3i(q2, lc.lo2[c], lc.hi2[c]) + lc.off[c]);
     }
     __device__ __forceinline__ void prime(int qcur)
     {
         qq = __builtin_amdgcn_update_dpp(__builtin_amdgcn_readlane(qcur, 0), 0, 0x138, 0xF, 0xF, false);
-#pragma unroll
-        for (int c = 0; c < CPL; ++c) { scA[c] = score(qq & 0xffff, c); scB[c] = score((int)((unsigned)qq >> 16), c); }
+        const int qa = column<false>(qq), qb = column<true>(qq);
+#pragma unroll
+        for (int c = 0; c < CPL; ++c) { scA[c] = score(qa, c); scB[c] = score(qb, c); }
     }
 
     template <bool PRED>
     __device__ __forceinline__ void step(int t, int qsrc, int snext, bool gfirst = true, bool glast = true)
     {
         const int qn = __builtin_amdgcn_update_dpp(__builtin_amdgcn_readlane(qsrc, snext), qq, 0x138, 0xF, 0xF, false);
-        const int qa = qn & 0xffff, qb = (int)((unsigned)qn >> 16);
+        const int qa = column<false>(qn), qb = column<true>(qn);
         const int potA = add_uniform(potB, hh), potBn = add_uniform(potA, hh);
         const int upA = sel_mask(dpp_shr1_open(SbotA), potA, top_mask);
         const int upB = sel_mask(dpp_shr1_open(T[R2 - 1]), potBn, top_mask);
@@ -310,21 +339,26 @@
     }
 };
 
-template <int SHIFT>
-__device__ __forceinline__ int load_chunk2(const Screen2Task& tk, int chunk, int lane)
+template <int SHIFT, bool LEVELS>
+__device__ __forceinline__ int load_chunk2(const Screen2Task& tk, int chunk, int lane, int lvl0, int lvl1)
 {
     const int idx = (chunk * 64 + lane) * 2;
     int a = 0, b = 0;
     if (idx < tk.n) a = tk.levels[idx];
     if (idx + 1 < tk.n) b = tk.levels[idx + 1];
-    return (a << SHIFT) | (b << (SHIFT + 16));
-}
-
-template <int RPC, int CMG, bool LANES>
+    if constexpr (LEVELS) return screen_levels::scaled_level(a, lvl0, lvl1) | (screen_levels::scaled_level(b, lvl0, lvl1) << 16);
+    else return (a << SHIFT) | (b << (SHIFT + 16));
+}
+
+template <int RPC, int CMG, int LAYOUT, int SEGW>
 __device__ __forceinline__ void screen2_body(const Screen2Task* __restrict__ tasks, int n_groups, int* __restrict__ queue, const ScreenParams& sp, int lds_rows)
 {
     constexpr int R2 = RPC * CPL, MERGE = S / RPC;
+    constexpr bool LANES = LAYOUT == STRQ_SCREEN_LDS_LANES, LEVELS = LAYOUT == STRQ_SCREEN_LDS_LEVELS;
     constexpr int QSHIFT = LANES ? screen_lanes::ROW_SHIFT : 1;
+    constexpr int UNIT = LEVELS ? MERGE : 1;
+    static_assert(!LEVELS || (MERGE == screen_levels::MERGE && SEGW == screen_levels::SEG && CPL == screen_levels::CPL), "the level image is the coarse screen's");
+    static_assert((SEGW & (SEGW - 1)) == 0, "the prologue deals rows to waves by a mask");
     static_assert(CPL == screen_lanes::CPL, "screen_lds_layout.h stacks the lane's five classes");
     extern __shared__ uint32_t lds_all[];
     __shared__ int next_group;
@@ -337,9 +371,44 @@
         __syncthreads();
         const int gi = __builtin_amdgcn_readfirstlane(next_group);
         if (gi >= n_groups) break;
-        const Screen2Task& t0 = tasks[(size_t)gi * SEG];
-        const float scf = (float)sp.sc;
+        const Screen2Task& t0 = tasks[(size_t)gi * SEGW];
+        const int ksc = LEVELS ? sp.byte_sc : sp.sc;
+        const int khh = LEVELS ? sp.hh * ksc / sp.sc : sp.hh, kcadd = LEVELS ? khh + sp.v * ksc / sp.sc : sp.cadd;
+        const float scf = (float)ksc;
         Lane2Const lc;
+        [[maybe_unused]] int lvl0 = 0, lvl1 = 0;
+        if constexpr (LEVELS) {
+            lvl0 = screen_levels::range_lo(t0.lvl); lvl1 = screen_levels::range_hi(t0.lvl);
+            uint32_t desc[CPL];
+            int nc = 0;
+#pragma unroll
+            for (int c = 0; c < CPL; ++c) {
+                const int k = lf * CPL + c;
+                const bool in = lf < LPF && k < t0.k[f];
+                desc[c] = in ? (uint32_t)t0.band_lo[f][k] : 0u;
+                nc += in ? 1 : 0;
+            }
+            char* dst = reinterpret_cast<char*>(lds_all) + screen_levels::slot(lane);
+            const float* src = t0.table[f];
+            const int rows = lvl1 - lvl0 + 1 < lds_rows ? lvl1 - lvl0 + 1 : lds_rows;
+            for (int r = wave; r < rows; r += SEGW) {
+                int e[CPL];
+#pragma unroll
+                for (int c = 0; c < CPL; ++c) {
+                    e[c] = 0;
+                    if (c < nc) {
+                        const int v = ceil_scaled(src[screen_levels::desc_off(desc[c]) + screen_levels::band_index(desc[c], lvl0 + r)], scf) + kcadd;
+                        e[c] = v < 255 ? v : 255;
+                    }
+                }
+                char* row = dst + r * screen_levels::ROW_BYTES;
+                *reinterpret_cast<uint16_t*>(row + screen_levels::class_offset(0)) = (uint16_t)(e[0] | (e[1] << 8));
+                *reinterpret_cast<uint16_t*>(row + screen_levels::class_offset(2)) = (uint16_t)(e[2] | (e[3] << 8));
+                *reinterpret_cast<uint16_t*>(row + screen_levels::class_offset(4)) = (uint16_t)e[4];
+            }
+#pragma unroll
+            for (int c = 0; c < CPL; ++c) { lc.lo2[c] = 0; lc.hi2[c] = 0; lc.off[c] = screen_levels::slot(lane); }
+        }
         if constexpr (LANES) {
             uint32_t desc[CPL];
             int nc = 0, rowbase[CPL];
@@ -360,28 +429,28 @@
                 if (c < nc) {
                     const float* src = t0.table[f] + screen_lanes::desc_off(desc[c]);
                     const int w1 = screen_lanes::desc_w1(desc[c]);
-                    for (int i = (wave - rowbase[c]) & (SEG - 1); i <= w1; i += SEG)
+                    for (int i = (wave - rowbase[c]) & (SEGW - 1); i <= w1; i += SEGW)
                         if (rowbase[c] + i < lds_rows)
-                            *reinterpret_cast<uint16_t*>(dst + screen_lanes::entry_address(lane, rowbase[c], i)) = (uint16_t)(MERGE * ((int)ceilf(src[i] * scf) + sp.cadd));
+                            *reinterpret_cast<uint16_t*>(dst + screen_lanes::entry_address(lane, rowbase[c], i)) = (uint16_t)(MERGE * (ceil_scaled(src[i], scf) + sp.cadd));
                 }
             }
         }
         [[maybe_unused]] int base[2], zero_idx[2];
         base[0] = 0; zero_idx[0] = (t0.tsize[0] + 1) & ~1;
         base[1] = zero_idx[0] + 2; zero_idx[1] = base[1] + ((t0.tsize[1] + 1) & ~1);
-        if constexpr (!LANES) {
+        if constexpr (!LANES && !LEVELS) {
             uint16_t* dst = reinterpret_cast<uint16_t*>(lds_all);
 #pragma unroll
             for (int ff = 0; ff < 2; ++ff) {
-                for (int i = threadIdx.x; i < t0.tsize[ff]; i += 64 * SEG) dst[base[ff] + i] = (uint16_t)(MERGE * ((int)ceilf(t0.table[ff][i] * scf) + sp.cadd));
+                for (int i = threadIdx.x; i < t0.tsize[ff]; i += 64 * SEGW) dst[base[ff] + i] = (uint16_t)(MERGE * (ceil_scaled(t0.table[ff][i], scf) + sp.cadd));
                 if (threadIdx.x == 0) { dst[zero_idx[ff]] = 0; dst[zero_idx[ff] + 1] = 0; }
             }
         }
         __syncthreads();
-        const Screen2Task& tk = tasks[(size_t)gi * SEG + wave];
+        const Screen2Task& tk = tasks[(size_t)gi * SEGW + wave];
         if (tk.n <= 0) continue;
 
-        if constexpr (!LANES) {
+        if constexpr (!LANES && !LEVELS) {
 #pragma unroll
             for (int c = 0; c < CPL; ++c) {
                 const int k = lf * CPL + c;
@@ -397,19 +466,20 @@
         }
         const uint64_t top_mask = 1ull | (1ull << LB);
         const int lMa = (tk.k[0] - 1) / CPL, lMb = LB + (tk.k[1] - 1) / CPL;
-        Screen2<RPC, CMG> s2{ldsb, lc, top_mask, lane, tk.n, sp.hh};
+        const int hh = khh / UNIT;
+        Screen2<RPC, CMG, LAYOUT> s2{ldsb, lc, top_mask, lane, tk.n, hh};
         {
 #pragma unroll
             for (int r = 0; r < R2; ++r) s2.T[r] = STRQ_SCREEN_BIAS;
             s2.SbotA = STRQ_SCREEN_BIAS; s2.upS = STRQ_SCREEN_BIAS;
-            s2.potB = STRQ_SCREEN_BIAS - 2 * lane * sp.hh;
+            s2.potB = STRQ_SCREEN_BIAS - 2 * lane * hh;
             s2.cmax = STRQ_SCREEN_BIAS; s2.gpot = 0; s2.gmax = 0;
         }
         const int nsteps = (tk.n + 1) / 2 + 63;
-        int qcur = load_chunk2<QSHIFT>(tk, 0, lane);
+        int qcur = load_chunk2<QSHIFT, LEVELS>(tk, 0, lane, lvl0, lvl1);
         s2.prime(qcur);
         for (int t0s = 0; t0s < nsteps; t0s += 64) {
-            const int qnext = load_chunk2<QSHIFT>(tk, t0s / 64 + 1, lane);
+            const int qnext = load_chunk2<QSHIFT, LEVELS>(tk, t0s / 64 + 1, lane, lvl0, lvl1);
             const bool full = (t0s >= 63) && (2 * (t0s + 64) <= tk.n);
             const int send = nsteps - t0s < 64 ? nsteps - t0s : 64;
             if (full) {
@@ -432,7 +502,12 @@
             }
             const int cma = __builtin_amdgcn_readlane(s2.cmax, lMa) - STRQ_SCREEN_BIAS;
             const int cmb = __builtin_amdgcn_readlane(s2.cmax, lMb) - STRQ_SCREEN_BIAS;
-            if (lane == 0) { tk.out[0][t0s / 64] = cma; tk.out[1][t0s / 64] = cmb; }
+            if (lane == 0) {
+                if constexpr (LEVELS) {
+                    tk.out[0][t0s / 64] = (int)(((long long)cma * UNIT * sp.sc + ksc - 1) / ksc);
+                    tk.out[1][t0s / 64] = (int)(((long long)cmb * UNIT * sp.sc + ksc - 1) / ksc);
+                } else { tk.out[0][t0s / 64] = cma; tk.out[1][t0s / 64] = cmb; }
+            }
             s2.cmax = STRQ_SCREEN_BIAS;
             qcur = qnext;
         }
@@ -453,12 +528,14 @@
 #ifndef STRQ_SCREEN3_CMG
 #define STRQ_SCREEN3_CMG 2
 #endif
-#define STRQ_SCREEN2_ATTR(WPE_) __attribute__((amdgpu_flat_work_group_size(64 * STRQ_SCREEN_SEG, 64 * STRQ_SCREEN_SEG), amdgpu_waves_per_eu(WPE_, WPE_)))
+#define STRQ_SCREEN2_ATTR_SEG(WPE_, SEG_) __attribute__((amdgpu_flat_work_group_size(64 * SEG_, 64 * SEG_), amdgpu_waves_per_eu(WPE_, WPE_)))
+#define STRQ_SCREEN2_ATTR(WPE_) STRQ_SCREEN2_ATTR_SEG(WPE_, STRQ_SCREEN_SEG)
 #define STRQ_SCREEN2_ARGS const Screen2Task* __restrict__ tasks, int n_groups, int* __restrict__ queue, ScreenParams sp, int lds_rows
-__global__ void STRQ_SCREEN2_ATTR(6) align_screen3_kernel(STRQ_SCREEN2_ARGS) { screen2_body<2, STRQ_SCREEN3_CMG, true>(tasks, n_groups, queue, sp, lds_rows); }
-__global__ void STRQ_SCREEN2_ATTR(4) align_screen1_kernel(STRQ_SCREEN2_ARGS) { screen2_body<6, 1, true>(tasks, n_groups, queue, sp, lds_rows); }
-__global__ void STRQ_SCREEN2_ATTR(6) align_screen3_rows_kernel(STRQ_SCREEN2_ARGS) { screen2_body<2, STRQ_SCREEN3_CMG, false>(tasks, n_groups, queue, sp, lds_rows); }
-__global__ void STRQ_SCREEN2_ATTR(4) align_screen1_rows_kernel(STRQ_SCREEN2_ARGS) { screen2_body<6, 1, false>(tasks, n_groups, queue, sp, lds_rows); }
+__global__ void STRQ_SCREEN2_ATTR_SEG(6, STRQ_SCREEN_SEG_LEVELS) align_screen3_kernel(STRQ_SCREEN2_ARGS) { screen2_body<2, STRQ_SCREEN3_CMG, STRQ_SCREEN_LDS_LEVELS, STRQ_SCREEN_SEG_LEVELS>(tasks, n_groups, queue, sp, lds_rows); }
+__global__ void STRQ_SCREEN2_ATTR(6) align_screen3_lanes_kernel(STRQ_SCREEN2_ARGS) { screen2_body<2, STRQ_SCREEN3_CMG, STRQ_SCREEN_LDS_LANES, STRQ_SCREEN_SEG>(tasks, n_groups, queue, sp, lds_rows); }
+__global__ void STRQ_SCREEN2_ATTR(4) align_screen1_kernel(STRQ_SCREEN2_ARGS) { screen2_body<6, 1, STRQ_SCREEN_LDS_LANES, STRQ_SCREEN_SEG>(tasks, n_groups, queue, sp, lds_rows); }
+__global__ void STRQ_SCREEN2_ATTR(6) align_screen3_rows_kernel(STRQ_SCREEN2_ARGS) { screen2_body<2, STRQ_SCREEN3_CMG, STRQ_SCREEN_LDS_ROWS, STRQ_SCREEN_SEG>(tasks, n_groups, queue, sp, lds_rows); }
+__global__ void STRQ_SCREEN2_ATTR(4) align_screen1_rows_kernel(STRQ_SCREEN2_ARGS) { screen2_body<6, 1, STRQ_SCREEN_LDS_ROWS, STRQ_SCREEN_SEG>(tasks, n_groups, queue, sp, lds_rows); }
 #undef STRQ_SCREEN2_ARGS
 
 __global__ void __launch_bounds__(256)
@@ -470,6 +547,7 @@
     const int idx = blockIdx.x * (blockDim.x >> 6) + (threadIdx.x >> 6);
     if (idx >= n_groups) return;
     const int g = list ? list[idx] : idx;
+    const int SEG = sp.seg;
     const ScreenTask* tg = tasks + (size_t)g * SEG;
     const int m = tg[0].m, lM = tg[0].lane_last;
     const int shift = -m * sp.v;
@@ -601,7 +679,7 @@
             if (!(e < 1.0e4)) continue;
             sp->slack = ((int)std::ceil(e) + 1) * sc;
         }
-        sp->merge_gap = 3072; sp->margin = 0; sp->max_cand = 0;
+        sp->merge_gap = 3072; sp->margin = 0; sp->max_cand = 0; sp->seg = STRQ_SCREEN_SEG; sp->byte_sc = 0;
         return 1;
     }
     return 0;
@@ -621,18 +699,51 @@
     return 0;
 }
 
+int screen2_levels_plan(const AlignParams& p, int samples, int max_n, int merge, ScreenParams* sp)
+{
+    if (merge != screen_levels::MERGE) return 0;
+    if (!screen2_plan(p, samples, max_n, merge, sp)) return 0;
+    const int bsc = screen_levels::byte_scale((double)p.ext_h, (double)p.ext_v, (double)p.dist_offset);
+    if (bsc <= 0) return 0;
+    const double hhb = -(double)p.ext_h * bsc;
+    if ((double)(max_n + 256) * hhb / screen_levels::MERGE + 64.0 * CPL * 2 * 255.0 + (double)STRQ_SCREEN_BIAS > 2.0e9) return 0;
+    sp->byte_sc = bsc; sp->seg = STRQ_SCREEN_SEG_LEVELS;
+    return 1;
+}
+
+ScreenParams screen2_byte_frame(const ScreenParams& sp)
+{
+    ScreenParams b = sp;
+    const int bsc = sp.byte_sc;
+    b.hh = (int)((long long)sp.hh * bsc / sp.sc); b.v = (int)((long long)sp.v * bsc / sp.sc); b.cadd = b.hh + b.v;
+    b.slack = sp.slack / sp.sc * bsc; b.sc = bsc; b.seg = STRQ_SCREEN_SEG; b.byte_sc = 0;
+    return b;
+}
+
+uint32_t screen2_levels_range(uint32_t lvl_a, uint32_t lvl_b) { return screen_levels::join_ranges(lvl_a, lvl_b); }
+int screen2_levels_rows(uint32_t range) { return screen_levels::rows_of(range); }
+bool screen2_levels_fit(int rows) { return screen_levels::fits(rows); }
+size_t screen2_levels_lds_bytes(int rows) { return screen_levels::bytes(rows); }
+
 int launch_screen2(hipStream_t stream, const Screen2Task* tasks, int n_groups, int* queue, const ScreenParams& sp,
-                   size_t lds_bytes, int groups_per_cu, int n_cu, int merge, int lanes_rows)
+                   size_t lds_bytes, int groups_per_cu, int n_cu, int merge, int layout, int rows)
 {
     if (n_groups <= 0) return 0;
     if (merge != 3 && merge != 1) return 2;
-    const bool lanes = lanes_rows > 0;
-    if (lanes && (!screen_lanes::fits(lanes_rows) || lds_bytes < screen_lanes::bytes(lanes_rows))) return 2;
-    auto kern = merge == 3 ? (lanes ? align_screen3_kernel : align_screen3_rows_kernel) : (lanes ? align_screen1_kernel : align_screen1_rows_kernel);
+    const bool lanes = layout == STRQ_SCREEN_LDS_LANES, levels = layout == STRQ_SCREEN_LDS_LEVELS;
+    if (!lanes && !levels && layout != STRQ_SCREEN_LDS_ROWS) return 2;
+    if (lanes && (!screen_lanes::fits(rows) || lds_bytes < screen_lanes::bytes(rows))) return 2;
+    if (levels) {
+        if (merge != screen_levels::MERGE || !screen_levels::fits(rows) || lds_bytes < screen_levels::bytes(rows) || sp.seg != STRQ_SCREEN_SEG_LEVELS || sp.byte_sc <= 0) return 2;
+        const ScreenParams b = screen2_byte_frame(sp);
+        if (b.hh < screen_levels::MERGE || b.hh % screen_levels::MERGE != 0 || b.cadd > 255 || (long long)b.hh * sp.sc != (long long)sp.hh * b.sc) return 2;
+    }
+    if (!levels && sp.seg != SEG) return 2;
+    auto kern = merge == 3 ? (levels ? align_screen3_kernel : lanes ? align_screen3_lanes_kernel : align_screen3_rows_kernel) : (lanes ? align_screen1_kernel : align_screen1_rows_kernel);
     if (merge == 1 && groups_per_cu > 4) groups_per_cu = 4;
     if (groups_per_cu > 6) groups_per_cu = 6;
     (void)hipFuncSetAttribute((const void*)kern, hipFuncAttributeMaxDynamicSharedMemorySize, (int)lds_bytes);
-    hipLaunchKernelGGL(kern, dim3(groups_per_cu * n_cu), dim3(64 * SEG), lds_bytes, stream, tasks, n_groups, queue, sp, lanes_rows);
+    hipLaunchKernelGGL(kern, dim3(groups_per_cu * n_cu), dim3(64 * sp.seg), lds_bytes, stream, tasks, n_groups, queue, sp, lanes || levels ? rows : 0);
     return hipGetLastError() == hipSuccess ? 0 : 1;
 }
 
diff --git a/strique_amd/csrc/screen_levels_layout.h b/strique_amd/csrc/screen_levels_layout.h
--- /dev/null
+++ b/strique_amd/csrc/screen_levels_layout.h
@@ -0,0 +1,74 @@
+#pragma once
+#include <stddef.h>
+#include <stdint.h>
+
+#if defined(__HIPCC__) || defined(__CUDACC__)
+#define STRQ_LEVELS_HD __host__ __device__ __forceinline__
+#else
+#define STRQ_LEVELS_HD inline
+#endif
+
+namespace strq {
+namespace screen_levels {
+
+constexpr int SUB_BYTES = 128;
+constexpr int SUBS = 3;
+constexpr int ROW_BYTES = SUBS * SUB_BYTES;
+constexpr int Q_SHIFT = 7;
+constexpr int CPL = 5;
+constexpr int MERGE = 3;
+constexpr int SEG = 8;
+static_assert(SUB_BYTES == 1 << Q_SHIFT && 255 * SUB_BYTES < 65536, "a scaled level has to fit the 16-bit half of the level pair");
+
+constexpr int MAX_ROWS = 183;
+constexpr size_t MAX_BYTES = (size_t)MAX_ROWS * ROW_BYTES;
+
+STRQ_LEVELS_HD int desc_lo(uint32_t d) { return (int)(d & 255u); }
+STRQ_LEVELS_HD int desc_w1(uint32_t d) { return (int)((d >> 8) & 255u); }
+STRQ_LEVELS_HD int desc_off(uint32_t d) { return (int)(d >> 16); }
+
+STRQ_LEVELS_HD uint32_t pack_range(int lvl0, int lvl1) { return (uint32_t)lvl0 | ((uint32_t)lvl1 << 8); }
+STRQ_LEVELS_HD int range_lo(uint32_t r) { return (int)(r & 255u); }
+STRQ_LEVELS_HD int range_hi(uint32_t r) { return (int)((r >> 8) & 255u); }
+STRQ_LEVELS_HD uint32_t join_ranges(uint32_t a, uint32_t b)
+{
+    const int lo = range_lo(a) < range_lo(b) ? range_lo(a) : range_lo(b), hi = range_hi(a) > range_hi(b) ? range_hi(a) : range_hi(b);
+    return pack_range(lo, hi < lo ? lo : hi);
+}
+STRQ_LEVELS_HD int rows_of(uint32_t r) { return range_hi(r) - range_lo(r) + 1; }
+
+STRQ_LEVELS_HD int slot(int lane) { return (lane & 31) * 4 + (lane >> 5) * 2; }
+STRQ_LEVELS_HD int class_offset(int c) { return (c >> 1) * SUB_BYTES + (c & 1); }
+
+STRQ_LEVELS_HD int scaled_level(int level, int lvl0, int lvl1)
+{
+    const int l = level < lvl0 ? lvl0 : (level > lvl1 ? lvl1 : level);
+    return (l - lvl0) << Q_SHIFT;
+}
+STRQ_LEVELS_HD int column_address(int scaled, int lane) { return scaled * SUBS + slot(lane); }
+STRQ_LEVELS_HD int address(int lane, int c, int level, int lvl0, int lvl1) { return column_address(scaled_level(level, lvl0, lvl1), lane) + class_offset(c); }
+STRQ_LEVELS_HD int band_index(uint32_t desc, int level)
+{
+    const int lo = desc_lo(desc), w1 = desc_w1(desc);
+    return level < lo ? 0 : (level > lo + w1 ? w1 : level - lo);
+}
+
+STRQ_LEVELS_HD size_t bytes(int rows) { return (size_t)rows * ROW_BYTES; }
+STRQ_LEVELS_HD bool fits(int rows) { return rows >= 1 && rows <= MAX_ROWS; }
+
+inline int byte_scale(double ext_h, double ext_v, double dist_offset)
+{
+    for (int sc = 255; sc >= 1; --sc) {
+        const double hh = -ext_h * sc, v = -ext_v * sc;
+        if (hh != (double)(long)hh || v != (double)(long)v || hh < MERGE) continue;
+        if ((long)hh % MERGE != 0) continue;
+        const double top = dist_offset * sc;
+        const long smax = (long)top + ((double)(long)top < top ? 1 : 0);
+        if ((double)smax + hh + v > 255.0) continue;
+        return sc;
+    }
+    return 0;
+}
+
+}
+}
diff --git a/strique_amd/csrc/strq_align_api.hip b/strique_amd/csrc/strq_align_api.hip
--- a/strique_amd/csrc/strq_align_api.hip
+++ b/strique_amd/csrc/strq_align_api.hip
@@ -315,7 +315,7 @@
         }
         STRQ_HIP(c, hipMemcpy(jobs[j].table, tab.data(), tab.size() * 4, hipMemcpyHostToDevice));
         STRQ_HIP(c, hipMemcpy(jobs[j].band_lo, blo.data(), (size_t)kk * 4, hipMemcpyHostToDevice));
-        info[j].total = kk * 256; info[j].need = 256;
+        info[j].total = kk * 256; info[j].need = 256; info[j].lvl = 255 << 8;
     }
     b.hard_count = hard_count;
     return STRQ_OK;
@@ -380,6 +380,8 @@
     std::vector<size_t> out_off;
     size_t out_words = 0, lds_bytes = 0;
     int lanes_rows = 0;
+    int levels_rows = 0;
+    int layout = 0;
     double steps = 0;
 };
 
@@ -396,7 +398,7 @@
 
 static void screen_tasks(CorePlan& p, const ScreenParams& sp, ScreenJob& j)
 {
-    constexpr int SSEG = STRQ_SCREEN_SEG;
+    const int SSEG = sp.seg;
     const AlignCoreIn& in = p.in;
     const int F = j.flanks, ng = (int)j.al.size() / F;
     if (F == 2) j.t2.resize((size_t)ng * SSEG);
@@ -408,16 +410,18 @@
         const int n = in.n[a[0]];
         const int m_big = F == 2 ? std::max(in.m[a[0]], in.m[a[1]]) : in.m[a[0]];
         const int ov_worst = align_segment_overlap(p.c->ap, m_big), ov_s = overlap_for(p, m_big, ov_worst, 16);
-        Piece pc[SSEG];
+        Piece pc[STRQ_SCREEN_SEG_MAX];
         const int used = cut(n, SSEG, ov_s, pc);
         j.lds_bytes = std::max(j.lds_bytes, F == 2 ? screen2_lds_bytes(p.info[p.J0[a[0]]].total, p.info[p.J0[a[1]]].total) : screen_lds_bytes(p.info[p.J0[a[0]]].total));
         if (F == 2) j.lanes_rows = std::max(j.lanes_rows, screen2_lanes_rows(p.info[p.J0[a[0]]].need, p.info[p.J0[a[1]]].need));
+        const uint32_t lvl = F == 2 ? screen2_levels_range((uint32_t)p.info[p.J0[a[0]]].lvl, (uint32_t)p.info[p.J0[a[1]]].lvl) : 0u;
+        if (F == 2) j.levels_rows = std::max(j.levels_rows, screen2_levels_rows(lvl));
         for (int f = 0; f < F; ++f)
             j.bound[(size_t)g * F + f] = used <= 1 ? INT32_MIN / 2 : (ov_s >= ov_worst ? 0 : (int32_t)std::ceil((double)align_segment_min_score(p.c->ap, in.m[a[f]], ov_s) * sp.sc));
         for (int w = 0; w < SSEG; ++w) {
             Screen2Task t; std::memset(&t, 0, sizeof(t));
             t.levels = in.d_levels + in.read_off[in.read[a[0]]] + pc[w].col_off;
-            t.n = pc[w].n; t.col_off = pc[w].col_off;
+            t.n = pc[w].n; t.col_off = pc[w].col_off; t.lvl = lvl;
             t.n_chunks = pc[w].n > 0 ? (align_num_steps(pc[w].n) + 63) / 64 : 0;
             for (int f = 0; f < F; ++f) {
                 const LutJob& job = p.jobs[p.J0[a[f]]];
@@ -437,14 +441,16 @@
 
 static int run_screen(CorePlan& p, ScreenJob& j, const ScreenParams& sp, const ScreenRules& r)
 {
-    constexpr int SSEG = STRQ_SCREEN_SEG;
+    const int SSEG = sp.seg;
     strq_ctx* c = p.c; const AlignCoreIn& in = p.in;
     hipStream_t st = p.st;
     const int nv = (int)j.al.size();
-    int lanes_rows = 0;
+    int layout = 0, image_rows = 0;
     if (j.flanks == 2) {
         const char* e = strq::opt("STRQ_SCREEN_LDS");
-        if (!(e && std::strcmp(e, "rows") == 0) && screen2_lanes_fit(j.lanes_rows)) { lanes_rows = j.lanes_rows; j.lds_bytes = screen2_lanes_lds_bytes(lanes_rows); }
+        layout = STRQ_SCREEN_LDS_ROWS;
+        if (j.layout == STRQ_SCREEN_LDS_LEVELS) { layout = STRQ_SCREEN_LDS_LEVELS; image_rows = j.levels_rows; j.lds_bytes = screen2_levels_lds_bytes(image_rows); }
+        else if (!(e && std::strcmp(e, "rows") == 0) && screen2_lanes_fit(j.lanes_rows)) { layout = STRQ_SCREEN_LDS_LANES; image_rows = j.lanes_rows; j.lds_bytes = screen2_lanes_lds_bytes(image_rows); }
     }
     if (j.lds_bytes > 160 * 1024 - 64) { c->err = r.lds_err; return STRQ_ERR_UNSUPPORTED; }
     const int groups = std::max(1, std::min(r.groups_per_cu, (int)((160 * 1024 - 64) / j.lds_bytes)));
@@ -467,7 +473,7 @@
     STRQ_HIP(c, hipEventRecord(c->ev[5], st));
     int* queue = c->queue.as<int>() + STRQ_QUEUE_FIRST - 1;
     if (j.flanks == 2) {
-        if (launch_screen2(st, d_t2, nv / 2, queue, sp, j.lds_bytes, groups, c->n_cu, r.merge, lanes_rows)) { c->err = "coarse screen launch failed"; return STRQ_ERR_DEVICE; }
+        if (launch_screen2(st, d_t2, nv / 2, queue, sp, j.lds_bytes, groups, c->n_cu, r.merge, layout, image_rows)) { c->err = "coarse screen launch failed"; return STRQ_ERR_DEVICE; }
     } else {
         if (launch_screen(st, d_st, nv, queue, sp, j.lds_bytes, groups, c->n_cu)) { c->err = "screen launch failed"; return STRQ_ERR_DEVICE; }
     }
@@ -477,7 +483,7 @@
     STRQ_HIP(c, hipMemcpyAsync(hw.data(), d_win, hw.size() * sizeof(ScreenWindows), hipMemcpyDeviceToHost, st));
     STRQ_HIP(c, hipStreamSynchronize(st));
     c->screen_ran = true; c->screen_mode_last = r.merge > 1 ? 2 : 1; c->coarse_merge_last = r.merge;
-    c->screen_lds_last = j.flanks == 2 ? (lanes_rows > 0 ? 1 : 2) : 0;
+    c->screen_lds_last = layout; c->screen_byte_sc_last = layout == STRQ_SCREEN_LDS_LEVELS ? sp.byte_sc : 0;
     if (const char* path = strq::opt("STRQ_SCREEN_DUMP")) {
         std::vector<int32_t> ho(j.out_words);
         STRQ_HIP(c, hipMemcpy(ho.data(), d_out, j.out_words * 4, hipMemcpyDeviceToHost));
@@ -530,8 +536,8 @@
         else if (windowed < 0.9 * (nv - (p.ov_fixed ? 0 : below_bound)) || cols > r.max_cols * all || (long)heavy * 100 > 2L * nv) pause_after_fail(*r.pause, *r.fail);
         else *r.fail = 0;
     }
-    STRQ_DBG("screen (%d flanks per wave, merge %d): %d alignments, scale %d, margin %.0f, %d groups per CU, LDS %zu bytes: %d with windows (%d below the cold-start bound), %.2f %% of the columns, %d heavy -> pause %d",
-             j.flanks, r.merge, nv, sp.sc, (double)sp.margin / sp.sc, groups, j.lds_bytes, windowed, below_bound, 100.0 * cols / std::max(1.0, all), heavy, *r.pause);
+    STRQ_DBG("screen (%d flanks per wave, merge %d, LDS layout %d, %d image rows, %d pieces): %d alignments, scale %d, margin %.0f, %d groups per CU, LDS %zu bytes: %d with windows (%d below the cold-start bound), %.2f %% of the columns, %d heavy -> pause %d",
+             j.flanks, r.merge, layout, image_rows, SSEG, nv, sp.sc, (double)sp.margin / sp.sc, groups, j.lds_bytes, windowed, below_bound, 100.0 * cols / std::max(1.0, all), heavy, *r.pause);
     return STRQ_OK;
 }
 
@@ -558,6 +564,29 @@
     std::stable_sort(pairs.begin(), pairs.end(), [&](const std::pair<int, int>& x, const std::pair<int, int>& y) { return in.n[x.first] > in.n[y.first]; });
     const int ngr = (int)pairs.size();
     if (ngr == 0 || 2 * ngr < (nb * 9) / 10) return STRQ_OK;
+    bool levels = false;
+    if (merge == 3) {
+        const char* e = strq::opt("STRQ_SCREEN_LDS");
+        ScreenParams spb;
+        if (screen2_levels_plan(c->ap, p.S, max_n, merge, &spb)) {
+            levels = !e || std::strcmp(e, "levels") == 0;
+            for (size_t x = 0; levels && x < pairs.size(); ++x)
+                levels = screen2_levels_fit(screen2_levels_rows(screen2_levels_range((uint32_t)p.info[p.J0[pairs[x].first]].lvl, (uint32_t)p.info[p.J0[pairs[x].second]].lvl)));
+            if (levels && !e) {
+                double extra = 0, all = 0; long used = 0;
+                for (const auto& pr : pairs) {
+                    const int m_big = std::max(in.m[pr.first], in.m[pr.second]);
+                    const int ov_s = overlap_for(p, m_big, align_segment_overlap(c->ap, m_big), 16);
+                    Piece pc[STRQ_SCREEN_SEG_MAX];
+                    const int u8 = cut(in.n[pr.first], STRQ_SCREEN_SEG_LEVELS, ov_s, pc), u4 = cut(in.n[pr.first], STRQ_SCREEN_SEG, ov_s, pc);
+                    extra += (double)(u8 - u4) * ov_s; all += in.n[pr.first]; used += u8;
+                }
+                levels = extra <= 0.10 * all && used * 10 >= 9L * STRQ_SCREEN_SEG_LEVELS * (long)pairs.size();
+            }
+            if (levels) sp = spb;
+            else if (strq::opt("STRQ_SCREEN2_BYTE_SCALE")) sp = screen2_byte_frame(spb);
+        }
+    }
     sp.margin = (int32_t)std::lround((double)c->coarse_margin * (merge == 3 ? 1.3 : 1.0) * sp.sc);
     if (const char* e = strq::opt("STRQ_SCREEN2_MARGIN")) sp.margin = (int32_t)std::lround(atof(e) * sp.sc);
     sp.max_cand = 8;
@@ -566,6 +595,7 @@
     ScreenJob j;
     j.flanks = 2;
     for (const auto& pr : pairs) { j.al.push_back(pr.first); j.al.push_back(pr.second); }
+    j.layout = levels ? STRQ_SCREEN_LDS_LEVELS : 0;
     screen_tasks(p, sp, j);
     ScreenRules r;
     r.merge = merge; r.groups_per_cu = groups;
@@ -1471,6 +1501,7 @@
     out[5] = (int32_t)std::min<int64_t>(c->look2_served, INT32_MAX);
     out[4] = c->screen_mode_last ? c->coarse_merge_last : 0;
     out[6] = c->screen_mode_last ? c->screen_lds_last : 0;
+    out[7] = c->screen_mode_last ? c->screen_byte_sc_last : 0;
     return STRQ_OK;
 }
 
diff --git a/strique_amd/csrc/strq_ctx.h b/strique_amd/csrc/strq_ctx.h
--- a/strique_amd/csrc/strq_ctx.h
+++ b/strique_amd/csrc/strq_ctx.h
@@ -130,6 +130,7 @@
     float aborted_fwd_ms = 0, aborted_screen_ms = 0;
     int screen_mode_last = 0;
     int coarse_merge_last = 0;
+    int screen_byte_sc_last = 0;
     int screen_lds_last = 0;
     
     strq::DevBuf levels, level_val, flank_cls, tables, tables3, band_lo, col0, ckpt, rec, tasks, results,
diff --git a/strique_amd/ffi.py b/strique_amd/ffi.py
--- a/strique_amd/ffi.py
+++ b/strique_amd/ffi.py
@@ -278,7 +278,8 @@
         out["mode"] = {0: None, 1: "fine", 2: "coarse"}.get(int(m[0]))
         out["coarse_pause"], out["fine_pause"], out["coarse_margin"], out["merge"] = int(m[1]), int(m[2]), int(m[3]), int(m[4])
         out["second_look"] = int(m[5])
-        out["lds_layout"] = {0: None, 1: "lanes", 2: "rows"}.get(int(m[6]))
+        out["lds_layout"] = {0: None, 1: "lanes", 2: "rows", 3: "levels"}.get(int(m[6]))
+        out["byte_scale"] = int(m[7])
         return out
 
     def last_overlap(self):
```

Result: faster. 26800, median of 6 (+7.5%).
